# set-soft/ComfyUI-FLOAT_Optimized

Hardware: AMD Instinct MI355X
Metric: 512x512 frames/sec end-to-end audio->video @50 ODE steps (higher is better)
Workload: dtype fp16; 1 GPU; configs[1]: 10 s audio + 512x512 portrait in HBM -> 250 frames in pinned host memory; appearance encoder + wav2vec2 audio encoder + FMT sampling (50 Euler evaluations/window, CFG a=2.0 e=1.0) + decode + D2H, through InferenceAgent.infer_device (the product call); nfe=51, frames_per_clip=250, fmt_dtype=fp16, dec_dtype=fp16, decode_batch=32, hip_graph=True, parallelism=replicas x1 (one clip per GPU), stage_overlap=off

## Files before the change

### comfyui-float_optimized_amd/csrc/fmt_api.hip

```cpp
#include <math.h>
#include <stdlib.h>

#include "fmt_gemm.hpp"
#include "fmt_kernels.hpp"
#include "fmt_rb_kernels.hpp"
#include "fmt_big_kernels.hpp"

namespace {

typedef FmtLin Lin;

struct Blk {
  Lin qkv, proj, fc1, fc2;
};

constexpr int kMaxTok = 80;
constexpr int kMaxSteps = 1024;

}

struct float_fmt {
  float_fmt_cfg_t cfg;
  DevicePool pool;
  int D, ntok, Mpad, Kc, Ntot, Kx;
  int Bmax = 1;
  Lin x_embed, t0, t2, c_embed, adaln_all, final_lin;
  std::vector<Blk> blk;
  float* pos = nullptr;
  float* freqs = nullptr;
  u16 *cond16, *sc16, *h16, *hfin16, *qkv16, *att16, *hid16, *xin16, *tsin16, *th16;
  float *ccond, *xres, *xcur, *temb, *vout;
  unsigned long long* sat = nullptr;
  float* slab = nullptr;
  float *wa_c, *we_c, *prev_x, *prev_wa, *prev_we, *x0_c;
  int method = 0;
  FmtTune tune;
  int n_cu = 0;
  struct MegaPlan {
    MegaStage* dev = nullptr;
    int nstage = 0, bc = 0, tried = 0;
    MegaCtx ctx{};
  } mega[5];
  unsigned* mega_sync = nullptr;
  unsigned* mega_err_host = nullptr;
  u16* mega_ws = nullptr;
  float* kbuf = nullptr;
  float* modall = nullptr;
  int Mmod = 0;
  size_t mod_zs = 0;
  struct GraphKey {
    int nfe, bc, we_len, method, nclip;
    int prio;
    float a, r, e;
    bool operator==(const GraphKey& o) const { return memcmp(this, &o, sizeof(GraphKey)) == 0; }
  };
  struct GraphEntry {
    GraphKey key;
    hipGraphExec_t exec;
    uint64_t used;
  };
  std::vector<GraphEntry> graphs;
  uint64_t graph_clock = 0;
  hipStream_t cap_stream = nullptr;
  int cap_prio = 0;
  struct {
    const float *wr, *wa, *we, *noise;
    float* r_d;
    int T, we_len, nfe, include_r, next, n_chunks, B;
    int first = 0, total = 0;
    const float *hist_x = nullptr, *hist_wa = nullptr, *hist_we = nullptr;
    float a, r, e;
    std::vector<float> ts;
    bool active = false;
  } job;
};

namespace {

int round_up(int x, int m) { return (x + m - 1) / m * m; }

int dev_copy2d(float* dst, size_t dpitch, const float* src, size_t spitch, int width, int rows, hipStream_t s) {
  if (width <= 0 || rows <= 0) return FLOAT_OK;
  hipLaunchKernelGGL(fmt_copy_kernel, dim3((unsigned)(((size_t)rows * width + 255) / 256)), dim3(256), 0, s, dst, dpitch, src, spitch, width, rows);
  FH_CHECK_HIP(hipGetLastError());
  return FLOAT_OK;
}
int dev_copy(float* dst, const float* src, size_t n, hipStream_t s) { return dev_copy2d(dst, n, src, n, (int)n, 1, s); }
int dev_zero(float* dst, size_t n, hipStream_t s) { return dev_copy2d(dst, n, nullptr, n, (int)n, 1, s); }


template <class T>
__global__ __launch_bounds__(256) void fmt_pack_w_kernel(typename T::elem* __restrict__ out, const float* __restrict__ w, int N_each,
                                                         int K, int KB, int n0) {
  const size_t idx = (size_t)blockIdx.x * 256 + threadIdx.x;
  const int gpr = KB * 4;
  const int n = (int)(idx / gpr), k0 = (int)(idx % gpr) * 8;
  if (n >= N_each) return;
  typename T::pack8 p;
#pragma unroll
  for (int i = 0; i < 8; ++i) T::set(p, i, k0 + i < K ? w[(size_t)n * K + k0 + i] : 0.f);
  T::store8(out + fmt_pack_off(n0 + n, k0, KB), p);
}

template <class T>
int pack_linear_pool(const FmtTune& tn, DevicePool* pool, const TensorTable& tt, const std::vector<std::string>& names, int N_each,
                     int K, Lin* out) {
  typedef typename T::elem E;
  constexpr size_t esz = sizeof(E) / sizeof(u16);
  const int Kp = round_up(K, 128);
  const int N = N_each * (int)names.size();
  const bool on_host = tn.pack_host;
  std::vector<E> hw;
  if (on_host) hw.assign((size_t)N * Kp, (E)0);
  std::vector<float> hb(N, 0.f);
  int rc;
  if ((rc = pool->alloc(&out->W, (size_t)N * Kp * esz, false))) return rc;
  if ((rc = pool->alloc(&out->b, hb.size(), false))) return rc;
  float* stage = nullptr;
  if (!on_host) FH_CHECK_HIP(hipMalloc(&stage, (size_t)N_each * K * sizeof(float)));
  struct Free {
    float* p;
    ~Free() {
      if (p) (void)hipFree(p);
    }
  } free_stage{stage};
  int n0 = 0;
  for (const std::string& nm : names) {
    const float_tensor_t* w = tt.find(nm + ".weight");
    const float_tensor_t* b = tt.find(nm + ".bias");
    if (!w || !b) {
      fh_set_error("missing checkpoint tensor '%s.weight/.bias'", nm.c_str());
      return FLOAT_E_MISSING;
    }
    if (w->ndim != 2 || w->shape[0] != N_each || w->shape[1] != K || TensorTable::numel(b) != N_each) {
      fh_set_error("tensor '%s.weight' has shape (%lld,%lld), expected (%d,%d)", nm.c_str(), (long long)w->shape[0],
                   (long long)(w->ndim > 1 ? w->shape[1] : 0), N_each, K);
      return FLOAT_E_INVALID;
    }
    if (on_host) {
      for (int n = 0; n < N_each; ++n) {
        const float* src = w->data + (size_t)n * K;
        for (int k = 0; k < K; ++k) hw[fmt_pack_off(n0 + n, k, Kp / 32)] = T::host_from_float(src[k]);
      }
    } else {
      FH_CHECK_HIP(hipMemcpy(stage, w->data, (size_t)N_each * K * sizeof(float), hipMemcpyHostToDevice));
      const size_t packs = (size_t)N_each * (Kp / 8);
      hipLaunchKernelGGL((fmt_pack_w_kernel<T>), dim3((unsigned)((packs + 255) / 256)), dim3(256), 0, nullptr,
                         reinterpret_cast<E*>(out->W), stage, N_each, K, Kp / 32, n0);
      FH_CHECK_HIP(hipGetLastError());
    }
    for (int n = 0; n < N_each; ++n) hb[n0 + n] = b->data[n];
    n0 += N_each;
  }
  if (on_host) FH_CHECK_HIP(hipMemcpy(out->W, hw.data(), hw.size() * sizeof(E), hipMemcpyHostToDevice));
  FH_CHECK_HIP(hipMemcpy(out->b, hb.data(), hb.size() * sizeof(float), hipMemcpyHostToDevice));
  if (!on_host) FH_CHECK_HIP(hipDeviceSynchronize());
  out->N = N;
  out->K = Kp;
  return FLOAT_OK;
}

template <class T>
int pack_linear(float_fmt* h, const TensorTable& tt, const std::vector<std::string>& names, int N_each, int K, Lin* out) {
  return pack_linear_pool<T>(h->tune, &h->pool, tt, names, N_each, K, out);
}

constexpr int kWtRows = 256;
template <class T, int MTW, int KCH, int NWV = 4>
int launch_wide_t(GemmArgs g, bool prime, hipStream_t s) {
  constexpr int smem = 2 * MTW * KCH * 1024;
  auto kern = fmt_gemm_wide_kernel<T, MTW, KCH, NWV>;
  if (prime) {
    if (hipFuncSetAttribute(reinterpret_cast<const void*>(kern), hipFuncAttributeMaxDynamicSharedMemorySize, smem) != hipSuccess)
      (void)hipGetLastError();
    return FLOAT_OK;
  }
  const int mt_total = (g.M + 15) / 16;
  g.mblk = (mt_total + MTW - 1) / MTW;
  g.ksplit = 1;
  const dim3 grid((g.N / 128) * g.mblk * (g.zcount > 1 ? g.zcount : 1));
  fh_launch_prof(2, kern, grid, dim3(NWV * 64), smem, s, g);
  FH_CHECK_HIP(hipGetLastError());
  return FLOAT_OK;
}
template <class T, int NWC, int NS, int STG>
int launch_dma_t(GemmArgs g, bool prime, hipStream_t s) {
  constexpr int smem = NS * (12 + 5 * NWC) * 1024, BN = 80 * NWC;
  auto kern = fmt_gemm_dma_kernel<T, NWC, NS, STG>;
  if (prime) {
    if (hipFuncSetAttribute(reinterpret_cast<const void*>(kern), hipFuncAttributeMaxDynamicSharedMemorySize, smem) != hipSuccess)
      (void)hipGetLastError();
    return FLOAT_OK;
  }
  g.mblk = ((g.M + 15) / 16 + 11) / 12;
  const dim3 grid((g.N / BN) * g.mblk * (g.zcount > 1 ? g.zcount : 1));
  fh_launch_prof(2, kern, grid, dim3(NWC * 128), smem, s, g);
  FH_CHECK_HIP(hipGetLastError());
  return FLOAT_OK;
}
bool dma_shape_ok(const GemmArgs& g, int bn) { return g.N % bn == 0 && g.K % 64 == 0 && g.K >= 128; }

constexpr int kBigMinRows = 1536;
// ... 210 lines not shown
  }
}

struct Tiling {
  int mtw, nt, nw;
};
int pick_nw(int K, int forced) {
  const int KB = K / 32;
  if (forced && KB % forced == 0) return forced;
  if (KB >= 128 && KB % 16 == 0) return 16;
  if (KB >= 32 && KB % 8 == 0) return 8;
  return 4;
}
Tiling pick_tiling(const FmtTune& tn, int M, int N, int K, bool need_full_rows) {
  const int mt = (M + 15) / 16;
  if (need_full_rows) {
    if (mt <= 4) return {4, 1, pick_nw(K, 0)};
    return {mt <= 12 ? 12 : 15, 1, (tn.full_nw == 8 && (K / 32) % 8 == 0) ? 8 : 4};
  }
  int split = mt <= 4 ? 4 : (mt <= 12 ? 3 : 5);
  if (mt <= 2) split = mt;
  const int blocks = (mt + split - 1) / split;
  const bool wide = N >= 16384;
  if (mt >= 12) {
    const int* o = tn.plan + (wide ? 3 : 0);
    if (o[0]) {
      int nw = o[0] >= 12 ? 4 : pick_nw(K, o[2]);
      while (nw > 4 && nw * o[0] * 16 * o[1] * 16 * 4 > 160 * 1024) nw >>= 1;
      return {o[0], o[1], nw};
    }
  }
  if (wide) return {mt <= 4 ? 4 : 6, 2, std::min(8, pick_nw(K, 0))};
  if (mt > 15 && N % 64 == 0) return {3, 4, 4};
  int nt = 1;
  if (mt >= 5) {
    if ((N / 64) * blocks >= 192 && N % 64 == 0) nt = 4;
    else if ((N / 32) * blocks >= 192 && N % 32 == 0) nt = 2;
  } else if ((N / 16) * blocks > 512) {
    nt = 2;
  }
  return {split, nt, pick_nw(K, 0)};
}

GemmArgs base_args(const u16* A, const Lin& L, int M) {
  GemmArgs g;
  memset(&g, 0, sizeof(g));
  g.A = A;
  g.W = L.W;
  g.bias = L.b;
  g.K = L.K;
  g.N = L.N;
  g.M = M;
  return g;
}

Tiling pick_tiling32(int M) {
  const int mt = (M + 15) / 16;
  return {mt <= 5 ? mt : (mt <= 12 ? 3 : 5), 1, 4};
}

template <class T, int EPI>
int run_gemm(const FmtTune& tn, const GemmArgs& g, hipStream_t s, bool need_full_rows = false, const LayerPlan* plan = nullptr) {
  if constexpr (T::is32) {
    FH_REQUIRE(!need_full_rows, "the fp32 mode has no all-rows CFG epilogue tiling (token-blocked head only)");
    const Tiling t = pick_tiling32(g.M);
    GemmArgs g2 = g;
    g2.touch.W = nullptr;
    return launch_gemm<T, EPI>(g2, t.mtw, t.nt, t.nw, false, s);
  }
  if (plan && plan->on() && (g.M + 15) / 16 <= 15) {
    GemmArgs g2 = g;
    g2.touch.W = nullptr;
    return launch_gemm<T, EPI>(g2, plan->v[0], plan->v[1], plan->v[2], false, s);
  }
  const Tiling t = pick_tiling(tn, g.M, g.N, g.K, need_full_rows);
  return launch_gemm<T, EPI>(g, t.mtw, t.nt, t.nw, false, s);
}

struct PendingRed {
  int ks = 0;
  LnRed red{};
};

template <class T>
int run_gemm_partial(float_fmt* h, GemmArgs g, int ksplit, hipStream_t s, const LayerPlan* plan = nullptr) {
  g.ksplit = ksplit;
  g.out_f32 = h->slab;
  g.ldo = g.N;
  g.slab_stride = (size_t)h->Mpad * g.N;
  if (plan && plan->on() && !T::is32 && (g.M + 15) / 16 <= 15) {
    g.touch.W = nullptr;
    return launch_gemm<T, EPI_PARTIAL>(g, plan->v[0], plan->v[1], plan->v[2], false, s);
  }
  Tiling t = T::is32 ? pick_tiling32(g.M) : pick_tiling(h->tune, g.M, g.N * ksplit, g.K / ksplit, false);
  while (t.nt > 1 && g.N % (t.nt * 16)) t.nt >>= 1;
  if (T::is32) g.touch.W = nullptr;
  return launch_gemm<T, EPI_PARTIAL>(g, t.mtw, t.nt, t.nw, false, s);
}

TouchSpec make_touch(const FmtTune& tn, const Lin& L, int M, int ksplit, unsigned lanes, unsigned per_lane, int force_nt = 0) {
  TouchSpec t{};
  Tiling tl = ksplit ? pick_tiling(tn, M, L.N * ksplit, L.K / ksplit, false) : pick_tiling(tn, M, L.N, L.K, false);
  if (force_nt) tl.nt = force_nt;
  if (ksplit)
    while (tl.nt > 1 && L.N % (tl.nt * 16)) tl.nt >>= 1;
  const int ks = ksplit ? ksplit : 1;
  if (L.N % (tl.nt * 16) || L.K % (32 * ks) || 8 % ks) return t;
  const int nbn = L.N / (tl.nt * 16);
  if ((nbn * ks) % 8) return t;
  auto lg = [](unsigned v) {
    int n = 0;
    while ((1u << n) < v) ++n;
    return (1u << n) == v ? n : -1;
  };
  const unsigned P = 8 / ks, run_lines = (unsigned)(L.K / 32 / ks) * 8u;
  if (lg(run_lines) < 0 || lg((unsigned)tl.nt) < 0) return t;
  t.run_shift = (unsigned)lg(run_lines);
  t.nt_shift = (unsigned)lg((unsigned)tl.nt);
  t.p_shift = (unsigned)lg(P);
  t.tile_bytes = (unsigned)(L.K / 32) * 1024u;
  t.total = ((unsigned)nbn / P) * (unsigned)tl.nt * run_lines;
  if ((size_t)t.total > (size_t)lanes * per_lane) return t;
  t.W = reinterpret_cast<const char*>(L.W);
  return t;
}

TouchSpec make_touch_rb(const Lin& L, int shape, int kb, unsigned lanes, unsigned per_lane) {
  TouchSpec t{};
  const int ct = shape == 0 ? 4 : 8;
  if (kb <= 0 || (kb & (kb - 1)) || L.N % (ct * 16) || (L.N / (ct * 16)) % 8 || L.K / 32 < kb) return t;
  const unsigned run_lines = (unsigned)kb * 8u;
  auto lg = [](unsigned v) {
    int n = 0;
    while ((1u << n) < v) ++n;
    return n;
  };
  t.run_shift = (unsigned)lg(run_lines);
  t.nt_shift = (unsigned)lg((unsigned)ct);
  t.p_shift = 3;
  t.tile_bytes = (unsigned)(L.K / 32) * 1024u;
  t.total = (unsigned)(L.N / (ct * 16) / 8) * (unsigned)ct * run_lines;
  if ((size_t)t.total > (size_t)lanes * per_lane) return t;
  t.W = reinterpret_cast<const char*>(L.W);
  return t;
}

unsigned gemm_lanes_per_xcd(const FmtTune& tn, int M, int N, int K) {
  const Tiling t = pick_tiling(tn, M, N, K, false);
  const int mblk = ((M + 15) / 16 + t.mtw - 1) / t.mtw;
  return (unsigned)((N / (t.nt * 16)) * mblk / 8) * (unsigned)(t.nw * 64);
}

template <class T>
int launch_lnmod(float_fmt* h, int M, const float* shift, const float* scale, hipStream_t s, PendingRed* pend = nullptr,
                 const Lin* next = nullptr, u16* out = nullptr, int perm = 0, int touch_bit = 1, int rb_shape = -1) {
  const int nv = h->D / 256;
  const int rpw = h->tune.ln_rows;
  dim3 grid(rpw == 1 ? ((M + 63) / 64) * 64 : (M + rpw - 1) / rpw), block(64 * rpw);
  const int ks = pend ? pend->ks : 0;
  const bool wt = M <= kWtRows;
  LnRed red{};
  if (ks) red = pend->red;
  TouchSpec pf{};
  if (next && (h->tune.touch & (1 | touch_bit)) && rpw == 1 && !T::is32)
    pf = rb_shape >= 0 ? make_touch_rb(*next, rb_shape, h->tune.rb_touch, (grid.x / 8) * 64, 6)
                       : make_touch(h->tune, *next, M, 0, (grid.x / 8) * 64, 6);
#define LN_LAUNCH(NV, KS)                                                                                                          \
  do {                                                                                                                             \
    if (pf.W && wt) hipLaunchKernelGGL((fmt_lnmod_kernel<T, NV, KS, true, true>), grid, block, 0, s, h->xres, M, shift, scale, h->Ntot, out ? out : h->h16, red, pf, h->ntok, perm, h->sat); \
    else if (pf.W) hipLaunchKernelGGL((fmt_lnmod_kernel<T, NV, KS, true, false>), grid, block, 0, s, h->xres, M, shift, scale, h->Ntot, out ? out : h->h16, red, pf, h->ntok, perm, h->sat); \
    else if (wt) hipLaunchKernelGGL((fmt_lnmod_kernel<T, NV, KS, false, true>), grid, block, 0, s, h->xres, M, shift, scale, h->Ntot, out ? out : h->h16, red, pf, h->ntok, perm, h->sat); \
    else hipLaunchKernelGGL((fmt_lnmod_kernel<T, NV, KS, false, false>), grid, block, 0, s, h->xres, M, shift, scale, h->Ntot, out ? out : h->h16, red, pf, h->ntok, perm, h->sat);   \
  } while (0)
#define LN_CASE(NV)                     \
  case NV:                              \
    if (ks == 0) LN_LAUNCH(NV, 0);      \
    else if (ks == 1) LN_LAUNCH(NV, 1); \
    else if (ks == 2) LN_LAUNCH(NV, 2); \
    else if (ks == 4) LN_LAUNCH(NV, 4); \
    else LN_LAUNCH(NV, 8);              \
    break;
  switch (nv) {
    LN_CASE(1) LN_CASE(2) LN_CASE(4) LN_CASE(8)
    default:
      fh_set_error("dim_h %d unsupported (must be 256*{1,2,4,8})", h->D);
      return FLOAT_E_INVALID;
  }
#undef LN_CASE
#undef LN_LAUNCH
  if (pend) pend->ks = 0;
  FH_CHECK_HIP(hipGetLastError());
  return FLOAT_OK;
}

template <class T>
void launch_attn(float_fmt* h, int M, const Lin* pull, hipStream_t s) {
  const float_fmt_cfg_t& c = h->cfg;
  const int D = h->D, ntok = h->ntok;
  const int qpw = h->tune.attn_qpw, lpq = h->tune.attn_lpq;
  dim3 grid(c.heads, (M + qpw - 1) / qpw), block(qpw * lpq);
  TouchSpec pf{};
  if (pull && !T::is32) pf = make_touch(h->tune, *pull, M, 0, (grid.x * grid.y / 8) * block.x, 2);
#define ATTN_LAUNCH(LPQ, TCH)                                                                                                  \
  do {                                                                                                                         \
    if (M <= kWtRows) hipLaunchKernelGGL((fmt_attn_kernel<T, LPQ, TCH, true>), grid, block, 0, s, h->qkv16, 3 * D, h->att16, ntok, M, D, c.attn_window, pf, h->sat); \
    else hipLaunchKernelGGL((fmt_attn_kernel<T, LPQ, TCH, false>), grid, block, 0, s, h->qkv16, 3 * D, h->att16, ntok, M, D, c.attn_window, pf, h->sat);             \
  } while (0)
  if (lpq == 16) {
    if (pf.W) ATTN_LAUNCH(16, true);
    else ATTN_LAUNCH(16, false);
  } else {
    if (pf.W) ATTN_LAUNCH(8, true);
    else ATTN_LAUNCH(8, false);
  }
#undef ATTN_LAUNCH
}

int attnproj_hpw(const float_fmt* h) {
  const int hd = h->cfg.heads, hpw = h->tune.attnproj;
  if (hpw <= 0 || h->D != hd * 128 || hd % hpw) return 0;
  const int ks = hd / hpw;
  return (ks == 1 || ks == 2 || ks == 4 || ks == 8) && (hpw == 1 || hpw == 2) ? hpw : 0;
}
template <class T>
int launch_attnproj(float_fmt* h, int M, const Lin& proj, hipStream_t s) {
  const float_fmt_cfg_t& c = h->cfg;
  const int hpw = attnproj_hpw(h);
  GemmArgs g = base_args(nullptr, proj, M);
  g.sat = h->sat;
  g.out_f32 = h->slab;
  g.ldo = g.N;
  g.slab_stride = (size_t)h->Mpad * g.N;
  g.ksplit = c.heads / hpw;
  g.mblk = ((M + 15) / 16 + 2) / 3;
  const dim3 grid((unsigned)(g.ksplit * (g.N / (128 / hpw)) * g.mblk));
  fh_launch_prof(0, hpw == 2 ? fmt_attnproj_kernel<T, 3, 2> : fmt_attnproj_kernel<T, 3, 1>, grid, dim3(512), 0, s, h->qkv16, 3 * h->D, g,
                 h->ntok, h->D, c.attn_window);
  FH_CHECK_HIP(hipGetLastError());
  return FLOAT_OK;
}

constexpr int kScSteps = 64;

static int stream_priority(hipStream_t s) {
  int prio = 0;
  if (hipStreamGetPriority(s, &prio) != hipSuccess) {
    (void)hipGetLastError();
    prio = 0;
  }
  return prio;
}

template <class T>
int run_mod_all(float_fmt* h, int M, int e0, int n, hipStream_t s) {
  const int D = h->D;
  const FmtTune& tn = h->tune;
  FH_REQUIRE(n >= 1 && n <= kScSteps, "modulation batch of %d evaluations (max %d)", n, kScSteps);
  const int prio = (s == h->cap_stream && s) ? h->cap_prio : stream_priority(s);
  const bool big = !T::is32 && tn.wide && prio == 0 && big_shape_ok(tn, n * M, h->adaln_all.N, h->adaln_all.K, h->n_cu);
  hipLaunchKernelGGL((fmt_silu_c_kernel<T>), dim3((M * D / 8 + 255) / 256, n), dim3(256), 0, s, h->sc16, h->temb + (size_t)e0 * D,
                     h->ccond, M, D, (size_t)h->Mpad * D, big ? M : 0, h->sat);
  h->mod_zs = big ? (size_t)M * h->Ntot : (size_t)h->Mmod * h->Ntot;
  if constexpr (!T::is32) {
    if (big) return launch_big4<T>(h->sc16, h->adaln_all, h->modall, n * M, h->Ntot, h->n_cu, false, s);
  }
  GemmArgs g = base_args(h->sc16, h->adaln_all, M);
  g.sat = h->sat;
  g.out_f32 = h->modall;
  g.ldo = h->Ntot;
  g.zcount = n;
  const bool dma = (tn.wide_variant == 6 || tn.wide_variant == 7) && (M + 15) / 16 > 4 && dma_shape_ok(g, 320);
  g.zgroup = tn.zgroup > 0 ? tn.zgroup : (dma ? 2 : 4);
  g.a_zstride = (size_t)h->Mpad * D;
  g.o_zstride = (size_t)h->Mmod * h->Ntot;
  if constexpr (!T::is32) {
    if (tn.wide && g.N % 128 == 0 && g.K % 128 == 0) return launch_wide<T>(g, tn.wide_variant, false, s);
  }
  for (int z = 0; z < n; ++z) {
    GemmArgs gz = g;
    gz.A = g.A + (size_t)z * g.a_zstride * (sizeof(typename T::elem) / sizeof(u16));
    gz.out_f32 = g.out_f32 + (size_t)z * g.o_zstride;
    gz.zcount = 0;
    int rc = run_gemm<T, EPI_F32>(tn, gz, s);
    if (rc) return rc;
  }
  return FLOAT_OK;
}

constexpr int kMegaWgs = 256, kMegaSmem = 8 * 48 * 64 * 4;
MegaSync mega_sync_of(const float_fmt* h) {
  unsigned* m = h->mega_sync;
  return MegaSync{m, m + 8 * 32, m + 9 * 32, m + 17 * 32, m + 18 * 32, h->mega_err_host, reinterpret_cast<unsigned long long*>(m + 20 * 32), (unsigned)h->tune.mega_stamp_wg};
}
int mega_poll(float_fmt* h) {
  if (!h->mega_err_host || *reinterpret_cast<volatile unsigned*>(h->mega_err_host) == 0u) return FLOAT_OK;
  FH_CHECK_HIP(hipDeviceSynchronize());
  for (auto& gr : h->graphs) (void)hipGraphExecDestroy(gr.exec);
  h->graphs.clear();
  if (h->mega_sync) FH_CHECK_HIP(hipMemset(h->mega_sync, 0, (size_t)(32 * 20) * sizeof(unsigned)));
  *reinterpret_cast<volatile unsigned*>(h->mega_err_host) = 0u;
  h->tune.mega = 0;
  h->job.active = false;
  fh_set_error("fmt_mega_kernel: a grid barrier timed out in an earlier call (not all %d workgroups were resident) - the results of "
               "that call are invalid; the handle falls back to the launch chain (FLOAT_FMT_MEGA=0 selects it from the start)", 256);
  return FLOAT_E_HIP;
}
template <class T>
bool mega_shape_ok(const float_fmt* h, int nclip, int bc) {
  const FmtTune& tn = h->tune;
  if (T::is32 || !tn.mega || nclip != 1 || bc != 3 || h->D != 1024 || h->cfg.heads != 8 || h->n_cu < kMegaWgs) return false;
  if (attnproj_hpw(h) || tn.fc2_split != 4 || tn.proj_split != 0) return false;
  const int M = bc * h->ntok;
  auto is = [](Tiling t, int a, int b, int c) { return t.mtw == a && t.nt == b && t.nw == c; };
  const Blk& B = h->blk[0];
  return (M + 15) / 16 == 12 && (h->ntok + 15) / 16 == 4 && h->x_embed.K % 256 == 0 && h->final_lin.K % 256 == 0 &&
         is(pick_tiling(tn, M, B.qkv.N, B.qkv.K, false), 3, 4, 8) && is(pick_tiling(tn, M, B.proj.N, B.proj.K, false), 3, 1, 8) &&
         is(pick_tiling(tn, M, B.fc1.N, B.fc1.K, false), 3, 4, 8) && is(pick_tiling(tn, M, B.fc2.N * 4, B.fc2.K / 4, false), 3, 4, 8) &&
         B.fc2.K % 512 == 0;
}

template <class T>
int build_mega(float_fmt* h, int bc) {
  float_fmt::MegaPlan& P = h->mega[bc];
  P.tried = 1;
  {
    int per_cu = 0;
    if (hipOccupancyMaxActiveBlocksPerMultiprocessor(&per_cu, reinterpret_cast<const void*>(fmt_mega_kernel<T>), 512, kMegaSmem) != hipSuccess) {
      (void)hipGetLastError();
      per_cu = 0;
    }
    if (per_cu * h->n_cu < kMegaWgs) {
      h->tune.mega = 0;
      return FLOAT_OK;
    }
  }
  const float_fmt_cfg_t& c = h->cfg;
  const FmtTune& tn = h->tune;
  const int D = h->D, ntok = h->ntok, M = bc * ntok;
  std::vector<MegaStage> st;
  const size_t esz = sizeof(typename T::elem) / sizeof(u16);
  const size_t n_h = (size_t)h->Mpad * D * esz, n_hid = (size_t)h->Mpad * c.mlp_hidden * esz;
  if (!h->mega_ws) {
    int rc0 = h->pool.alloc(&h->mega_ws, (size_t)c.depth * (3 * n_h + n_hid), true);
    if (rc0) return rc0;
  }
  auto ws_h1 = [&](int b) { return h->mega_ws + (size_t)b * (3 * n_h + n_hid); };
  auto ws_h2 = [&](int b) { return ws_h1(b) + n_h; };
  auto ws_att = [&](int b) { return ws_h1(b) + 2 * n_h; };
  auto ws_hid = [&](int b) { return ws_h1(b) + 3 * n_h; };
  auto gemm_stage = [&](int kind, GemmArgs g, int mtw, int nt) {
    MegaStage m;
    memset(&m, 0, sizeof(m));
    m.kind = kind;
    g.sat = h->sat;
    g.mblk = ((g.M + 15) / 16 + mtw - 1) / mtw;
    if (g.ksplit < 1) g.ksplit = 1;
    m.g = g;
    m.nblk = (unsigned)((g.N / (nt * 16)) * g.mblk * g.ksplit);
    return m;
  };
  auto ln_stage = [&](int b_mod, int which, int ks, const float* bias, int gate_col, const Lin* next, int touch_bit, u16* out, int perm) {
    MegaStage m;
    memset(&m, 0, sizeof(m));
    m.kind = MS_LN;
    m.nblk = (unsigned)(((M + 63) / 64) * 64);
    m.shift_off = (long long)b_mod * 6 * D + (long long)which * D;
    m.scale_off = m.shift_off + D;
    m.ks = ks;
    m.red_bias = bias;
    m.red_gate_off = (long long)b_mod * 6 * D + (long long)gate_col * D;
    m.ln_out = out ? out : h->h16;
    m.perm = perm;
    if (next && (tn.touch & (1 | touch_bit))) m.pf = make_touch(tn, *next, M, 0, (m.nblk / 8) * 64, 6);
    return m;
  };
  {
    GemmArgs g = base_args(h->xin16, h->x_embed, ntok);
    g.out_f32 = h->xres;
    g.ldo = D;
    g.pos = h->pos;
    g.bc = bc;
    g.ntok = ntok;
    st.push_back(gemm_stage(MS_XEMBED, g, 4, 1));
  }
  for (int b = 0; b < c.depth; ++b) {
    const Blk& B = h->blk[b];
    if (b == 0) st.push_back(ln_stage(b, 0, 0, nullptr, 0, &B.qkv, 128, ws_h1(b), 0));
    else {
      MegaStage m = ln_stage(b, 0, 4, h->blk[b - 1].fc2.b, 0, &B.qkv, 128, ws_h1(b), 0);
      m.red_gate_off = (long long)(b - 1) * 6 * D + 5LL * D;
      st.push_back(m);
    }
    {
      GemmArgs g = base_args(ws_h1(b), B.qkv, M);
      g.out16 = h->qkv16;
      g.ldo16 = 3 * D;
      if (tn.touch & 8) g.touch = make_touch(tn, B.proj, M, 0, gemm_lanes_per_xcd(tn, M, g.N, g.K), 2);
      st.push_back(gemm_stage(MS_QKV, g, 3, 4));
    }
    {
      MegaStage m;
      memset(&m, 0, sizeof(m));
      m.kind = MS_ATTN;
      m.nblk = (unsigned)(c.heads * ((M + 7) / 8));
      if (tn.touch & 2) m.pf = make_touch(tn, B.proj, M, 0, (m.nblk / 8) * 128, 2);
      m.att_out = ws_att(b);
      st.push_back(m);
    }
    {
      GemmArgs g = base_args(ws_att(b), B.proj, M);
      g.out_f32 = h->xres;
      g.ldo = D;
      g.ldg = h->Ntot;
      if (tn.touch & 16) g.touch = make_touch(tn, B.fc1, M, 0, gemm_lanes_per_xcd(tn, M, g.N, g.K), 2);
      MegaStage m = gemm_stage(MS_PROJ, g, 3, 1);
      m.gate_off = (long long)b * 6 * D + 2LL * D;
      st.push_back(m);
    }
    st.push_back(ln_stage(b, 3, 0, nullptr, 0, &B.fc1, 64, ws_h2(b), 0));
    {
      GemmArgs g = base_args(ws_h2(b), B.fc1, M);
      g.out16 = ws_hid(b);
      g.ldo16 = B.fc2.K / 32;
      if (tn.touch & 4) g.touch = make_touch(tn, B.fc2, M, 4, gemm_lanes_per_xcd(tn, M, g.N, g.K), 2);
      st.push_back(gemm_stage(MS_FC1, g, 3, 4));
    }
    {
      GemmArgs g = base_args(ws_hid(b), B.fc2, M);
      g.ksplit = 4;
      g.out_f32 = h->slab;
      g.ldo = g.N;
      g.slab_stride = (size_t)h->Mpad * g.N;
      if (tn.touch & 32) {
        const unsigned lanes = gemm_lanes_per_xcd(tn, M, g.N * 4, g.K / 4);
        if (b + 1 < c.depth) g.touch = make_touch(tn, h->blk[b + 1].qkv, M, 0, lanes, 2);
        else g.touch = make_touch(tn, h->final_lin, M, 0, lanes, 2, 1);
      }
      st.push_back(gemm_stage(MS_FC2, g, 3, 4));
    }
  }
  {
    const int nblk = (ntok + 15) / 16, seqs = bc;
    MegaStage m = ln_stage(c.depth, 0, 4, h->blk[c.depth - 1].fc2.b, 0, nullptr, 0, h->hfin16, seqs * 16);
    m.red_gate_off = (long long)(c.depth - 1) * 6 * D + 5LL * D;
    st.push_back(m);
    GemmArgs g = base_args(h->hfin16, h->final_lin, nblk * seqs * 16);
    g.tokblk = 1;
    g.nclip = 1;
    g.bc = bc;
    g.ntok = ntok;
    g.n_prev = c.n_prev;
    g.xcur = h->xcur;
    g.xin16 = h->xin16;
    g.ldx = h->Kx / 32;
    st.push_back(gemm_stage(MS_HEAD, g, bc, 1));
  }
  for (const MegaStage& m : st) FH_REQUIRE(m.nblk <= (unsigned)kMegaWgs, "persistent kernel: a stage needs %u workgroups", m.nblk);
  int rc;
  if (!h->mega_sync && (rc = h->pool.alloc(&h->mega_sync, 32 * 20 + 2 * 3 * 64, true))) return rc;
  if (!h->mega_err_host) {
    FH_CHECK_HIP(hipHostMalloc(reinterpret_cast<void**>(&h->mega_err_host), 64, hipHostMallocMapped));
    memset(h->mega_err_host, 0, 64);
  }
  if ((rc = h->pool.alloc(&P.dev, st.size(), false))) return rc;
  FH_CHECK_HIP(hipMemcpy(P.dev, st.data(), st.size() * sizeof(MegaStage), hipMemcpyHostToDevice));
  P.nstage = (int)st.size();
  P.bc = bc;
  P.ctx = MegaCtx{h->xres, h->qkv16, h->slab, (size_t)h->Mpad * D, M, D, ntok, h->Ntot, c.attn_window, c.heads, h->sat};
  return FLOAT_OK;
}

template <class T>
int run_mega(float_fmt* h, int bc, const float* modbuf, bool euler, float dt, float a, float r, float e, hipStream_t s, float* vout_to) {
  float_fmt::MegaPlan& P = h->mega[bc];
  MegaDyn d{modbuf, dt, a, r, e, euler ? 1 : 0, vout_to ? vout_to : h->vout};
  fh_launch_prof(0, (fmt_mega_kernel<T>), dim3(kMegaWgs), dim3(512), kMegaSmem, s, P.dev, P.nstage, d, P.ctx, mega_sync_of(h));
  FH_CHECK_HIP(hipGetLastError());
  return FLOAT_OK;
}

template <class T>
int run_blocks(float_fmt* h, int nclip, int bc, const float* modbuf, bool euler, float dt, float a, float r, float e, hipStream_t s,
               float* vout_to = nullptr) {
  const float_fmt_cfg_t& c = h->cfg;
  const FmtTune& tn = h->tune;
  const int D = h->D, ntok = h->ntok, M = nclip * bc * ntok;
  int rc;
  if constexpr (!T::is32) {
    if (bc <= 4 && mega_shape_ok<T>(h, nclip, bc)) {
      if (h->mega[bc].dev) return run_mega<T>(h, bc, modbuf, euler, dt, a, r, e, s, vout_to);
    }
  }
  {
    GemmArgs g = base_args(h->xin16, h->x_embed, nclip * ntok);
    g.sat = h->sat;
    g.out_f32 = h->xres;
    g.ldo = D;
    g.pos = h->pos;
    g.bc = bc;
    g.ntok = ntok;
    if ((rc = run_gemm<T, EPI_XEMBED>(tn, g, s))) return rc;
  }
  PendingRed pend;
  RbPlan rb_qkv, rb_proj, rb_fc1, rb_fc2;
  if constexpr (!T::is32) {
    rb_qkv = pick_rb(tn, RB_QKV, M), rb_proj = pick_rb(tn, RB_PROJ, M), rb_fc1 = pick_rb(tn, RB_FC1, M), rb_fc2 = pick_rb(tn, RB_FC2, M);
  }
  auto split_ok = [&](int ks, const Lin& L) { return (ks == 1 || ks == 2 || ks == 4) && L.K % (128 * ks) == 0; };
  for (int b = 0; b < c.depth; ++b) {
    const float* mod = modbuf + (size_t)b * 6 * D;
    const Blk& B = h->blk[b];
    if ((rc = launch_lnmod<T>(h, M, mod, mod + D, s, &pend, &B.qkv, nullptr, 0, 128, rb_qkv.shape))) return rc;
    {
      GemmArgs g = base_args(h->h16, B.qkv, M);
      g.sat = h->sat;
      g.out16 = h->qkv16;
      g.ldo16 = 3 * D;
      if ((tn.touch & 8) && attnproj_hpw(h)) g.touch = make_touch(tn, B.proj, M, c.heads / attnproj_hpw(h), gemm_lanes_per_xcd(tn, M, g.N, g.K), 2, 8 / attnproj_hpw(h));
      else if ((tn.touch & 8) && !split_ok(tn.proj_split, B.proj)) g.touch = make_touch(tn, B.proj, M, 0, gemm_lanes_per_xcd(tn, M, g.N, g.K), 2);
      if (rb_qkv.shape >= 0) rc = launch_rbs<T, EPI_T16>(g, rb_qkv.shape, false, s);
      else rc = run_gemm<T, EPI_T16>(tn, g, s, false, &tn.plan_layer[RB_QKV]);
      if (rc) return rc;
    }
    if (rb_proj.shape >= 0) {
      launch_attn<T>(h, M, nullptr, s);
      GemmArgs gp = base_args(h->att16, B.proj, M);
      gp.ksplit = rb_proj.ksplit;
      gp.out_f32 = h->slab;
      gp.ldo = gp.N;
      gp.slab_stride = (size_t)h->Mpad * gp.N;
      if ((rc = launch_rbs<T, EPI_PARTIAL>(gp, rb_proj.shape, false, s))) return rc;
      pend.ks = rb_proj.ksplit;
      pend.red = LnRed{h->slab, (size_t)h->Mpad * D, B.proj.b, mod + 2 * D};
    } else if (attnproj_hpw(h)) {
      if ((rc = launch_attnproj<T>(h, M, B.proj, s))) return rc;
      pend.ks = c.heads / attnproj_hpw(h);
      pend.red = LnRed{h->slab, (size_t)h->Mpad * D, B.proj.b, mod + 2 * D};
    } else if (split_ok(tn.proj_split, B.proj)) {
      launch_attn<T>(h, M, nullptr, s);
      GemmArgs gp = base_args(h->att16, B.proj, M);
      if ((rc = run_gemm_partial<T>(h, gp, tn.proj_split, s))) return rc;
      pend.ks = tn.proj_split;
      pend.red = LnRed{h->slab, (size_t)h->Mpad * D, B.proj.b, mod + 2 * D};
    } else {
      launch_attn<T>(h, M, (tn.touch & 2) ? &B.proj : nullptr, s);
      GemmArgs g = base_args(h->att16, B.proj, M);
      g.sat = h->sat;
      g.out_f32 = h->xres;
      g.ldo = D;
      g.gate = mod + 2 * D;
      g.ldg = h->Ntot;
      if (tn.touch & 16) g.touch = make_touch(tn, B.fc1, M, 0, gemm_lanes_per_xcd(tn, M, g.N, g.K), 2);
      if ((rc = run_gemm<T, EPI_GATE_RES>(tn, g, s, false, &tn.plan_layer[RB_PROJ]))) return rc;
    }
    if ((rc = launch_lnmod<T>(h, M, mod + 3 * D, mod + 4 * D, s, &pend, &B.fc1, nullptr, 0, 64, rb_fc1.shape))) return rc;
    {
      GemmArgs g = base_args(h->h16, B.fc1, M);
      g.sat = h->sat;
      g.out16 = h->hid16;
      g.ldo16 = B.fc2.K / 32;
      if ((tn.touch & 4) && rb_fc2.shape < 0)
        g.touch = make_touch(tn, B.fc2, M, split_ok(tn.fc2_split, B.fc2) ? tn.fc2_split : 0, gemm_lanes_per_xcd(tn, M, g.N, g.K), 2);
      if (rb_fc1.shape >= 0) rc = launch_rbs<T, EPI_GELU_P16>(g, rb_fc1.shape, false, s);
      else rc = run_gemm<T, EPI_GELU_P16>(tn, g, s, false, &tn.plan_layer[RB_FC1]);
      if (rc) return rc;
    }
    if (rb_fc2.shape >= 0) {
      GemmArgs g = base_args(h->hid16, B.fc2, M);
      g.ksplit = rb_fc2.ksplit;
      g.out_f32 = h->slab;
      g.ldo = g.N;
      g.slab_stride = (size_t)h->Mpad * g.N;
      if ((rc = launch_rbs<T, EPI_PARTIAL>(g, rb_fc2.shape, false, s))) return rc;
      pend.ks = rb_fc2.ksplit;
      pend.red = LnRed{h->slab, (size_t)h->Mpad * D, B.fc2.b, mod + 5 * D};
    } else if (split_ok(tn.fc2_split, B.fc2)) {
      GemmArgs g = base_args(h->hid16, B.fc2, M);
      g.sat = h->sat;
      if (tn.touch & 32) {
        const unsigned lanes = gemm_lanes_per_xcd(tn, M, g.N * tn.fc2_split, g.K / tn.fc2_split);
        if (b + 1 < c.depth) g.touch = make_touch(tn, h->blk[b + 1].qkv, M, 0, lanes, 2);
        else g.touch = make_touch(tn, h->final_lin, M, 0, lanes, 2, 1);
      }
      if ((rc = run_gemm_partial<T>(h, g, tn.fc2_split, s, &tn.plan_layer[RB_FC2]))) return rc;
      pend.ks = tn.fc2_split;
      pend.red = LnRed{h->slab, (size_t)h->Mpad * D, B.fc2.b, mod + 5 * D};
    } else {
      GemmArgs g = base_args(h->hid16, B.fc2, M);
      g.sat = h->sat;
      g.out_f32 = h->xres;
      g.ldo = D;
      g.gate = mod + 5 * D;
      g.ldg = h->Ntot;
      if ((rc = run_gemm<T, EPI_GATE_RES>(tn, g, s))) return rc;
    }
  }
  {
    const float* mod = modbuf + (size_t)c.depth * 6 * D;
    const bool tokblk = (!tn.no_tokblk || nclip > 1) && (bc == 1 || bc == 3 || bc == 4) && h->final_lin.K % 256 == 0;
    FH_REQUIRE(tokblk || nclip == 1, "batched sampling needs the token-blocked head GEMM");
    const int nblk = (ntok + 15) / 16, seqs = nclip * bc;
    if ((rc = launch_lnmod<T>(h, M, mod, mod + D, s, &pend, nullptr, tokblk ? h->hfin16 : nullptr, tokblk ? seqs * 16 : 0))) return rc;
    GemmArgs g = base_args(tokblk ? h->hfin16 : h->h16, h->final_lin, tokblk ? nblk * seqs * 16 : M);
    g.sat = h->sat;
    g.tokblk = tokblk ? 1 : 0;
    g.nclip = nclip;
    g.bc = bc;
    g.ntok = ntok;
    g.n_prev = c.n_prev;
    g.a_cfg = a;
    g.r_cfg = r;
    g.e_cfg = e;
    g.dt = dt;
    if (euler) {
      g.xcur = h->xcur;
      g.xin16 = h->xin16;
      g.ldx = h->Kx / 32;
    } else {
      g.vout = vout_to ? vout_to : h->vout;
    }
    if (tokblk) rc = launch_gemm<T, EPI_CFG>(g, bc, 1, 8, false, s);
    else rc = run_gemm<T, EPI_CFG>(tn, g, s, true);
    if (rc) return rc;
  }
  FH_CHECK_HIP(hipGetLastError());
  return FLOAT_OK;
}

void linspace01(int n, std::vector<float>* ts) {
  ts->resize(n);
  if (n == 1) {
    (*ts)[0] = 0.f;
    return;
  }
  const float step = 1.0f / (float)(n - 1);
  const int half = n / 2;
  for (int i = 0; i < n; ++i) (*ts)[i] = (i < half) ? (0.f + step * (float)i) : (1.0f - step * (float)(n - 1 - i));
}

struct TimeSpec {
  float t;
  int nfe, stages;
  float c[4];
};
template <class T>
int prepare_time(float_fmt* h, const TimeSpec& ts, int n, hipStream_t s) {
  int rc;
  hipLaunchKernelGGL((fmt_tsin_kernel<T>), dim3(n), dim3(256), 0, s, h->tsin16, h->freqs, n, ts.t, ts.nfe, ts.stages, ts.c[0],
                     ts.c[1], ts.c[2], ts.c[3]);
  GemmArgs g = base_args(h->tsin16, h->t0, n);
  g.sat = h->sat;
  g.out16 = h->th16;
  g.ldo16 = h->t2.K / 32;
  if ((rc = launch_gemm<T, EPI_SILU_P16>(g, 4, 1, T::is32 ? 4 : pick_nw(g.K, 0), false, s))) return rc;
  GemmArgs g2 = base_args(h->th16, h->t2, n);
  g2.sat = h->sat;
  g2.out_f32 = h->temb;
  g2.ldo = h->D;
  if ((rc = launch_gemm<T, EPI_F32>(g2, 4, 1, T::is32 ? 4 : pick_nw(g2.K, 0), false, s))) return rc;
  return FLOAT_OK;
}

struct CfgMode {
  int bc;
  unsigned wr_mask, wa_mask, we_mask;
  int nclip = 1;
};

CfgMode cfg_mode(float a, float r, float e, int include_r) {
  if (a == 1.0f && r == 1.0f && e == 1.0f) return {1, 1u, 1u, 1u, 1};
  if (!include_r) return {3, 0b111u, 0b110u, 0b010u, 1};
  return {4, 0b1110u, 0b1100u, 0b0100u, 1};
}

template <class T>
int stage_window(float_fmt* h, const CfgMode& m, const float* x0, const float* wa, const float* wr, const float* we,
                 int we_len, const float* prev_x, const float* prev_wa, const float* prev_we, hipStream_t s) {
  const float_fmt_cfg_t& c = h->cfg;
  const int M = m.nclip * m.bc * h->ntok;
  hipLaunchKernelGGL((fmt_build_cond_kernel<T>), dim3(M), dim3(256), 0, s, h->cond16, h->Kc, m.bc, h->ntok, c.n_prev,
                     c.dim_w, c.dim_a, c.dim_e, wr, wa, prev_wa, we, we_len, prev_we, m.wr_mask, m.wa_mask, m.we_mask, h->sat);
  GemmArgs g = base_args(h->cond16, h->c_embed, M);
  g.sat = h->sat;
  g.out_f32 = h->ccond;
  g.ldo = h->D;
  int rc;
  if ((rc = run_gemm<T, EPI_F32>(h->tune, g, s))) return rc;
  const int n = m.nclip * h->ntok * c.dim_w;
  hipLaunchKernelGGL((fmt_init_x_kernel<T>), dim3((n + 255) / 256), dim3(256), 0, s, h->xcur, h->xin16, h->Kx / 32, x0, prev_x,
                     c.n_prev, c.n_cur, c.dim_w, m.nclip, h->sat);
  FH_CHECK_HIP(hipGetLastError());
  return FLOAT_OK;
}

int check_common(float_fmt* h, const void* we, int we_len, const void* prev_we) {
  FH_REQUIRE(h != nullptr, "null FMT handle");
  FH_REQUIRE(we_len == 1 || we_len == h->cfg.n_cur,
             "Dynamic emotion latent `we` time dimension (%d) does not match audio latent `wa` time dimension (%d).",
             we_len, h->cfg.n_cur);
  FH_REQUIRE(!(we_len > 1 && prev_we == nullptr),
             "`we` is dynamic (T>1), but prev_we was not provided with prev_x/prev_wa.");
  (void)we;
  return FLOAT_OK;
}

struct Tableau {
  int s;
  float c[4], a[4][3], b[4];
};
const Tableau& tableau(int method) {
  static const Tableau T[5] = {
      {1, {0.f}, {{0.f}}, {1.f}},
      {2, {0.f, 0.5f}, {{0.f}, {0.5f}}, {0.f, 1.f}},
      {4, {0.f, 1.f / 3, 2.f / 3, 1.f}, {{0.f}, {1.f / 3}, {-1.f / 3, 1.f}, {1.f, -1.f, 1.f}}, {0.125f, 0.375f, 0.375f, 0.125f}},
      {2, {0.f, 1.f}, {{0.f}, {1.f}}, {0.5f, 0.5f}},
      {3, {0.f, 1.f / 3, 2.f / 3}, {{0.f}, {1.f / 3}, {0.f, 2.f / 3}}, {0.25f, 0.f, 0.75f}},
  };
  return T[method];
}

TimeSpec time_spec(int method, int nfe) {
  const Tableau& tb = tableau(method);
  TimeSpec ts{};
  ts.nfe = nfe;
  ts.stages = tb.s;
  for (int j = 0; j < 4; ++j) ts.c[j] = tb.c[j];
  return ts;
}
int n_evals(int method, int nfe) { return (nfe - 1) * tableau(method).s; }

template <class T>
int run_window_steps(float_fmt* h, const CfgMode& m, int nfe, const std::vector<float>& ts, float a, float r, float e,
                     hipStream_t s) {
  const Tableau& tb = tableau(h->method);
  const float_fmt_cfg_t& c = h->cfg;
  const size_t kstride = (size_t)h->Bmax * kMaxTok * c.dim_w;
  const int n = m.nclip * c.n_cur * c.dim_w, rows = m.nclip * m.bc * h->ntok;
  const int nev = n_evals(h->method, nfe), batch = h->tune.hoist ? kScSteps : 1;
  const bool euler = h->method == FLOAT_ODE_EULER;
  int rc;
  for (int ev = 0; ev < nev; ++ev) {
    const int i = ev / tb.s, j = ev - i * tb.s, z = ev % batch;
    const float dt = ts[i + 1] - ts[i];
    if (z == 0 && (rc = run_mod_all<T>(h, rows, ev, std::min(batch, nev - ev), s))) return rc;
    const float* mod = h->modall + (size_t)z * h->mod_zs;
    if (euler) {
      if ((rc = run_blocks<T>(h, m.nclip, m.bc, mod, true, dt, a, r, e, s))) return rc;
      continue;
    }
    if (j > 0) {
      hipLaunchKernelGGL((fmt_rk_combine_kernel<T>), dim3((n + 255) / 256), dim3(256), 0, s, h->xcur, h->kbuf, kstride, j,
                         dt * tb.a[j][0], dt * tb.a[j][1], dt * tb.a[j][2], 0.f, 0, h->xin16, h->Kx / 32, c.n_prev, c.n_cur,
                         c.dim_w, m.nclip, h->sat);
    }
    if ((rc = run_blocks<T>(h, m.nclip, m.bc, mod, false, 0.f, a, r, e, s, h->kbuf + (size_t)j * kstride))) return rc;
    if (j == tb.s - 1) {
      hipLaunchKernelGGL((fmt_rk_combine_kernel<T>), dim3((n + 255) / 256), dim3(256), 0, s, h->xcur, h->kbuf, kstride, tb.s,
                         dt * tb.b[0], dt * tb.b[1], dt * tb.b[2], dt * tb.b[3], 1, h->xin16, h->Kx / 32, c.n_prev, c.n_cur,
                         c.dim_w, m.nclip, h->sat);
    }
  }
  FH_CHECK_HIP(hipGetLastError());
  return FLOAT_OK;
}

constexpr size_t kMaxGraphs = 8;
template <class T>
int run_window_steps_graph(float_fmt* h, const CfgMode& m, int we_len, int nfe, const std::vector<float>& ts, float a,
                           float r, float e, hipStream_t s) {
  float_fmt::GraphKey key;
  memset(&key, 0, sizeof(key));
  key.nfe = nfe;
  key.method = h->method;
  key.bc = m.bc;
  key.nclip = m.nclip;
  key.we_len = we_len;
  key.a = a;
  key.r = r;
  key.e = e;
  key.prio = stream_priority(s);
  float_fmt::GraphEntry* hit = nullptr;
  for (auto& g : h->graphs)
    if (g.key == key) hit = &g;
  if (!hit) {
    if (!h->cap_stream) FH_CHECK_HIP(hipStreamCreateWithFlags(&h->cap_stream, hipStreamNonBlocking));
    hipGraph_t graph = nullptr;
    h->cap_prio = key.prio;
    FH_CHECK_HIP(hipStreamBeginCapture(h->cap_stream, hipStreamCaptureModeThreadLocal));
    int rc = run_window_steps<T>(h, m, nfe, ts, a, r, e, h->cap_stream);
    hipError_t ce = hipStreamEndCapture(h->cap_stream, &graph);
    if (rc) {
      if (graph) (void)hipGraphDestroy(graph);
      return rc;
    }
    FH_CHECK_HIP(ce);
    hipGraphExec_t exec = nullptr;
    FH_CHECK_HIP(hipGraphInstantiate(&exec, graph, nullptr, nullptr, 0));
    (void)hipGraphDestroy(graph);
    if (h->graphs.size() >= kMaxGraphs) {
      size_t lru = 0;
      for (size_t i = 1; i < h->graphs.size(); ++i)
        if (h->graphs[i].used < h->graphs[lru].used) lru = i;
      FH_CHECK_HIP(hipDeviceSynchronize());
      (void)hipGraphExecDestroy(h->graphs[lru].exec);
      h->graphs.erase(h->graphs.begin() + lru);
    }
    h->graphs.push_back({key, exec, 0});
    hit = &h->graphs.back();
  }
  hit->used = ++h->graph_clock;
  FH_CHECK_HIP(hipGraphLaunch(hit->exec, s));
  return FLOAT_OK;
}

template <class T>
int window_impl(float_fmt* h, const float* x0, const float* wa, const float* wr, const float* we, int we_len,
                const float* prev_x, const float* prev_wa, const float* prev_we, int nfe, const std::vector<float>& ts,
                float a, float r, float e, int include_r, hipStream_t s, int nclip = 1) {
  CfgMode m = cfg_mode(a, r, e, include_r);
  m.nclip = nclip;
  FH_REQUIRE(!h->tune.no_tokblk || m.bc * h->ntok <= 240,
             "%d-way CFG of %d tokens is %d rows; the all-rows CFG epilogue GEMM holds at most 240 (15 row tiles)", m.bc, h->ntok,
             m.bc * h->ntok);
  int rc = stage_window<T>(h, m, x0, wa, wr, we, we_len, prev_x, prev_wa, prev_we, s);
  if (rc) return rc;
  if (nfe <= 1) return FLOAT_OK;
  hipStreamCaptureStatus cs = hipStreamCaptureStatusNone;
  if (hipStreamIsCapturing(s, &cs) != hipSuccess) {
    (void)hipGetLastError();
    cs = hipStreamCaptureStatusNone;
  }
  if (h->cfg.use_graph && !g_fh_profiling && cs == hipStreamCaptureStatusNone)
    return run_window_steps_graph<T>(h, m, we_len, nfe, ts, a, r, e, s);
  return run_window_steps<T>(h, m, nfe, ts, a, r, e, s);
}

template <class T>
int eval_impl(float_fmt* h, float t, const float* x, const float* wa, const float* wr, const float* we, int we_len,
              const float* prev_x, const float* prev_wa, const float* prev_we, float a, float r, float e, int include_r,
              float* out, hipStream_t s) {
  TimeSpec tsp{};
  tsp.t = t;
  int rc = prepare_time<T>(h, tsp, 1, s);
  if (rc) return rc;
  const CfgMode m = cfg_mode(a, r, e, include_r);
  FH_REQUIRE(!h->tune.no_tokblk || m.bc * h->ntok <= 240,
             "%d-way CFG of %d tokens is %d rows; the all-rows CFG epilogue GEMM holds at most 240 (15 row tiles)", m.bc, h->ntok,
             m.bc * h->ntok);
  if ((rc = stage_window<T>(h, m, x, wa, wr, we, we_len, prev_x, prev_wa, prev_we, s))) return rc;
  if ((rc = run_mod_all<T>(h, m.bc * h->ntok, 0, 1, s))) return rc;
  if ((rc = run_blocks<T>(h, 1, m.bc, h->modall, false, 0.f, a, r, e, s))) return rc;
  return dev_copy(out, h->vout, (size_t)h->ntok * h->cfg.dim_w, s);
}

template <class T>
int sample_window(float_fmt* h, int k, hipStream_t s) {
  const float_fmt_cfg_t& c = h->cfg;
  auto& J = h->job;
  const int L = c.n_cur, P = c.n_prev, Tn = J.T, B = J.B;
  const bool dynamic = J.we_len > 1;
  int rc;
  auto blocks = [](int n) { return dim3((n + 255) / 256); };
  if (k == J.first) {
    if ((rc = prepare_time<T>(h, time_spec(h->method, J.nfe), std::max(1, n_evals(h->method, J.nfe)), s))) return rc;
    if (J.hist_x) rc = dev_copy(h->prev_x, J.hist_x, (size_t)B * P * c.dim_w, s);
    else rc = dev_zero(h->prev_x, (size_t)B * P * c.dim_w, s);
    if (rc) return rc;
    if (J.hist_wa) rc = dev_copy(h->prev_wa, J.hist_wa, (size_t)B * P * c.dim_a, s);
    else rc = dev_zero(h->prev_wa, (size_t)B * P * c.dim_a, s);
    if (rc) return rc;
    if (J.hist_we) rc = dev_copy(h->prev_we, J.hist_we, (size_t)B * P * c.dim_e, s);
    else rc = dev_zero(h->prev_we, (size_t)B * P * c.dim_e, s);
    if (rc) return rc;
  } else if (P > 0) {
    hipLaunchKernelGGL(fmt_tail_kernel, blocks(B * P * c.dim_w), dim3(256), 0, s, h->prev_x, h->xcur, P, L, c.dim_w, B);
    hipLaunchKernelGGL(fmt_tail_kernel, blocks(B * P * c.dim_a), dim3(256), 0, s, h->prev_wa, h->wa_c, P, L, c.dim_a, B);
    if (dynamic) hipLaunchKernelGGL(fmt_tail_kernel, blocks(B * P * c.dim_e), dim3(256), 0, s, h->prev_we, h->we_c, P, L, c.dim_e, B);
  }
  hipLaunchKernelGGL(fmt_slice_pad_kernel, blocks(B * L * c.dim_a), dim3(256), 0, s, h->wa_c, J.wa, k * L, Tn, L, c.dim_a, B);
  if (dynamic) hipLaunchKernelGGL(fmt_slice_pad_kernel, blocks(B * L * c.dim_e), dim3(256), 0, s, h->we_c, J.we, k * L, Tn, L, c.dim_e, B);
  if ((rc = dev_copy(h->x0_c, J.noise + (size_t)k * B * L * c.dim_w, (size_t)B * L * c.dim_w, s))) return rc;
  rc = window_impl<T>(h, h->x0_c, h->wa_c, J.wr, dynamic ? h->we_c : J.we, dynamic ? L : 1, h->prev_x, h->prev_wa,
                      dynamic ? h->prev_we : nullptr, J.nfe, J.ts, J.a, J.r, J.e, J.include_r, s, B);
  if (rc) return rc;
  const int rows = (k == J.total - 1) ? (Tn - k * L) : L;
  return dev_copy2d(J.r_d + (size_t)k * L * c.dim_w, (size_t)Tn * c.dim_w, h->xcur, (size_t)L * c.dim_w, rows * c.dim_w, B, s);
}

template <class T>
int create_impl(float_fmt* h, const TensorTable& tt) {
  const float_fmt_cfg_t& c = h->cfg;
  const int D = c.dim_h;
  int rc;
  prime_kernels<T>();
  if ((rc = pack_linear<T>(h, tt, {"x_embedder.proj"}, D, c.dim_w, &h->x_embed))) return rc;
  if ((rc = pack_linear<T>(h, tt, {"t_embedder.mlp.0"}, D, 256, &h->t0))) return rc;
  if ((rc = pack_linear<T>(h, tt, {"t_embedder.mlp.2"}, D, D, &h->t2))) return rc;
  if ((rc = pack_linear<T>(h, tt, {"c_embedder"}, D, c.dim_w + c.dim_a + c.dim_e, &h->c_embed))) return rc;
  h->blk.resize(c.depth);
  std::vector<std::string> ada;
  for (int b = 0; b < c.depth; ++b) {
    const std::string p = "blocks." + std::to_string(b) + ".";
    if ((rc = pack_linear<T>(h, tt, {p + "attn.qkv"}, 3 * D, D, &h->blk[b].qkv))) return rc;
    if ((rc = pack_linear<T>(h, tt, {p + "attn.proj"}, D, D, &h->blk[b].proj))) return rc;
    if ((rc = pack_linear<T>(h, tt, {p + "mlp.fc1"}, c.mlp_hidden, D, &h->blk[b].fc1))) return rc;
    if ((rc = pack_linear<T>(h, tt, {p + "mlp.fc2"}, D, c.mlp_hidden, &h->blk[b].fc2))) return rc;
    ada.push_back(p + "adaLN_modulation.1");
  }
  if ((rc = pack_linear<T>(h, tt, ada, 6 * D, D, &h->adaln_all))) return rc;
  {
    Lin tail;
    if ((rc = pack_linear<T>(h, tt, {"decoder.adaLN_modulation.1"}, 2 * D, D, &tail))) return rc;
    Lin fused;
    fused.N = h->adaln_all.N + tail.N;
    fused.K = h->adaln_all.K;
    constexpr size_t esz = sizeof(typename T::elem) / sizeof(u16);
    if ((rc = h->pool.alloc(&fused.W, (size_t)fused.N * fused.K * esz, false))) return rc;
    if ((rc = h->pool.alloc(&fused.b, (size_t)fused.N, false))) return rc;
    FH_CHECK_HIP(hipMemcpy(fused.W, h->adaln_all.W, (size_t)h->adaln_all.N * fused.K * esz * sizeof(u16), hipMemcpyDeviceToDevice));
    FH_CHECK_HIP(hipMemcpy(fused.W + (size_t)h->adaln_all.N * fused.K * esz, tail.W, (size_t)tail.N * fused.K * esz * sizeof(u16),
                           hipMemcpyDeviceToDevice));
    FH_CHECK_HIP(hipMemcpy(fused.b, h->adaln_all.b, (size_t)h->adaln_all.N * sizeof(float), hipMemcpyDeviceToDevice));
    FH_CHECK_HIP(hipMemcpy(fused.b + h->adaln_all.N, tail.b, (size_t)tail.N * sizeof(float), hipMemcpyDeviceToDevice));
    h->adaln_all = fused;
  }
  if ((rc = pack_linear<T>(h, tt, {"decoder.linear"}, c.dim_w, D, &h->final_lin))) return rc;
  return FLOAT_OK;
}

}


int fmt_pack_linear(const FmtTune& tn, DevicePool* pool, int dtype, const TensorTable& tt, const std::vector<std::string>& names,
                    int N_each, int K, FmtLin* out) {
  FH_REQUIRE(dtype == FLOAT_DT_BF16 || dtype == FLOAT_DT_FP16 || dtype == FLOAT_DT_FP32, "the GEMM service: unknown dtype %d", dtype);
  if (dtype == FLOAT_DT_FP32) return pack_linear_pool<FP32>(tn, pool, tt, names, N_each, K, out);
  return dtype == FLOAT_DT_BF16 ? pack_linear_pool<BF16>(tn, pool, tt, names, N_each, K, out)
                                : pack_linear_pool<FP16>(tn, pool, tt, names, N_each, K, out);
}

int fmt_pack_linear_raw(const FmtTune& tn, DevicePool* pool, int dtype, const float* w, const float* b, int N, int K, FmtLin* out) {
  std::vector<float> zeros;
  if (!b) {
    zeros.assign(N, 0.f);
    b = zeros.data();
  }
  float_tensor_t t[2];
  memset(t, 0, sizeof(t));
  t[0].name = "raw.weight";
  t[0].data = w;
  t[0].ndim = 2;
  t[0].shape[0] = N;
  t[0].shape[1] = K;
  t[1].name = "raw.bias";
  t[1].data = b;
  t[1].ndim = 1;
  t[1].shape[0] = N;
  TensorTable tt(t, 2);
  return fmt_pack_linear(tn, pool, dtype, tt, {"raw"}, N, K, out);
}

GemmArgs fmt_gemm_args(const u16* A, const FmtLin& L, int M) { return base_args(A, L, M); }

void fmt_gemm_prime(int dtype) {
  if (dtype == FLOAT_DT_BF16) prime_kernels<BF16>();
  else if (dtype == FLOAT_DT_FP32) prime_kernels<FP32>();
  else prime_kernels<FP16>();
}

template <class T>
static int gemm_run_t(const FmtTune& tn, int epi, const GemmArgs& g, hipStream_t s) {
  switch (epi) {
    case EPI_F32: return run_gemm<T, EPI_F32>(tn, g, s);
    case EPI_T16: return run_gemm<T, EPI_T16>(tn, g, s);
    case EPI_SILU_P16: return run_gemm<T, EPI_SILU_P16>(tn, g, s);
    case EPI_GELU_P16: return run_gemm<T, EPI_GELU_P16>(tn, g, s);
    case EPI_GELUERF_P16: return run_gemm<T, EPI_GELUERF_P16>(tn, g, s);
    default: fh_set_error("fmt_gemm_run: epilogue %d is not exported", epi); return FLOAT_E_INVALID;
  }
}

int fmt_gemm_run(const FmtTune& tn, int dtype, int epi, GemmArgs g, hipStream_t s) {
  if (dtype == FLOAT_DT_FP32) return gemm_run_t<FP32>(tn, epi, g, s);
  return dtype == FLOAT_DT_BF16 ? gemm_run_t<BF16>(tn, epi, g, s) : gemm_run_t<FP16>(tn, epi, g, s);
}

template <class T>
static int debug_impl(float_fmt* h, int what, const float* in, float* out, hipStream_t s) {
  const int D = h->D, ntok = h->ntok;
  if (what == 0) {
    return dev_copy(out, h->pos, (size_t)ntok * D, s);
  }
  if (what == 2) {
    FH_REQUIRE(h->mega_sync && h->mega[3].nstage > 0 && h->mega[3].nstage <= 64, "no persistent-kernel plan");
    FH_CHECK_HIP(hipStreamSynchronize(s));
    const int n = h->mega[3].nstage * 3;
    std::vector<unsigned long long> st(n);
    FH_CHECK_HIP(hipMemcpy(st.data(), h->mega_sync + 20 * 32, n * 8, hipMemcpyDeviceToHost));
    std::vector<float> us(n);
    for (int i = 0; i < n; ++i) us[i] = st[i] ? (float)((double)(st[i] - st[0]) * 0.01) : -1.f;
    FH_CHECK_HIP(hipMemcpy(out, us.data(), n * 4, hipMemcpyHostToDevice));
    return FLOAT_OK;
  }
  FH_REQUIRE(what == 1 && in != nullptr, "float_fmt_debug: unknown request %d (or null input)", what);
  const int n = ntok * 3 * D;
  hipLaunchKernelGGL((fmt_dbg_to16_kernel<T>), dim3((n + 255) / 256), dim3(256), 0, s, h->qkv16, in, n);
  launch_attn<T>(h, ntok, nullptr, s);
  hipLaunchKernelGGL((fmt_dbg_unpack_kernel<T>), dim3((ntok * D + 255) / 256), dim3(256), 0, s, out, h->att16, ntok, D);
  FH_CHECK_HIP(hipGetLastError());
  return FLOAT_OK;
}

extern "C" {

int float_fmt_create(const float_fmt_cfg_t* cfg, const float_tensor_t* tensors, int32_t n_tensors, float_fmt_t** out) {
  FH_REQUIRE(cfg && tensors && out, "null argument to float_fmt_create");
  FH_REQUIRE(cfg->dim_h % 256 == 0 && cfg->dim_h / 256 <= 8 && ((cfg->dim_h / 256) & (cfg->dim_h / 256 - 1)) == 0,
             "dim_h=%d unsupported", cfg->dim_h);
  FH_REQUIRE(cfg->dim_h / cfg->heads == 128, "head_dim must be 128 (dim_h=%d heads=%d)", cfg->dim_h, cfg->heads);
  FH_REQUIRE(cfg->dim_w % 128 == 0 && cfg->mlp_hidden % 128 == 0, "dim_w / mlp_hidden must be multiples of 128");
  FH_REQUIRE(cfg->n_prev + cfg->n_cur <= kMaxTok, "at most %d tokens per window (got %d)", kMaxTok, cfg->n_prev + cfg->n_cur);
  FH_REQUIRE(cfg->n_prev >= 0 && cfg->n_prev <= cfg->n_cur, "n_prev must be in [0, n_cur]");
  FH_REQUIRE(cfg->dtype == FLOAT_DT_BF16 || cfg->dtype == FLOAT_DT_FP16 || cfg->dtype == FLOAT_DT_FP32, "unknown dtype %d", cfg->dtype);
  FH_REQUIRE(cfg->max_batch >= 0 && cfg->max_batch <= 16, "max_batch must be in [0, 16] (got %d)", cfg->max_batch);
  float_fmt* h = new float_fmt();
  h->tune = FmtTune::from_env();
  h->cfg = *cfg;
  h->D = cfg->dim_h;
  h->ntok = cfg->n_prev + cfg->n_cur;
  h->Bmax = cfg->max_batch > 0 ? cfg->max_batch : 1;
  h->Mpad = 16 * ((h->Bmax * 4 * h->ntok + 15) / 16 + 12);
  h->Kc = round_up(cfg->dim_w + cfg->dim_a + cfg->dim_e, 128);
  h->Kx = round_up(cfg->dim_w, 128);
  {
    int dev = 0, ncu = 0;
    if (hipGetDevice(&dev) == hipSuccess && hipDeviceGetAttribute(&ncu, hipDeviceAttributeMultiprocessorCount, dev) == hipSuccess) h->n_cu = ncu;
    else (void)hipGetLastError();
  }
  h->Ntot = cfg->depth * 6 * h->D + 2 * h->D;
  TensorTable tt(tensors, n_tensors);
  int rc = (cfg->dtype == FLOAT_DT_BF16) ? create_impl<BF16>(h, tt)
           : (cfg->dtype == FLOAT_DT_FP16) ? create_impl<FP16>(h, tt) : create_impl<FP32>(h, tt);
  const int D = h->D, Mp = h->Mpad;
  const size_t esz = cfg->dtype == FLOAT_DT_FP32 ? 2 : 1;
  auto A = [&](auto** p, size_t n) {
    if (!rc) rc = h->pool.alloc(p, std::is_same<std::remove_reference_t<decltype(**p)>, u16>::value ? n * esz : n, true);
  };
  A(&h->pos, (size_t)kMaxTok * D);
  A(&h->freqs, 128);
  A(&h->cond16, (size_t)Mp * h->Kc);
  A(&h->sc16, (size_t)kScSteps * Mp * D + (size_t)12 * 16 * D);
  A(&h->h16, (size_t)Mp * D);
  A(&h->hfin16, (size_t)h->Bmax * 64 * ((kMaxTok + 15) / 16) * D);
  A(&h->qkv16, (size_t)Mp * 3 * D);
  A(&h->att16, (size_t)Mp * D);
  A(&h->hid16, (size_t)Mp * cfg->mlp_hidden);
  A(&h->xin16, (size_t)(h->Bmax * kMaxTok + 6 * 16) * h->Kx);
  A(&h->tsin16, (size_t)kMaxSteps * 256);
  A(&h->th16, (size_t)kMaxSteps * D);
  A(&h->ccond, (size_t)Mp * D);
  h->Mmod = 16 * ((h->Bmax * 4 * h->ntok + 15) / 16);
  if (!rc) rc = h->pool.alloc(&h->modall, (size_t)kScSteps * h->Mmod * h->Ntot, false);
  A(&h->kbuf, (size_t)4 * h->Bmax * kMaxTok * cfg->dim_w);
  A(&h->xres, (size_t)Mp * D);
  A(&h->slab, (size_t)8 * Mp * D);
  A(&h->sat, 1);
  A(&h->xcur, (size_t)h->Bmax * cfg->n_cur * cfg->dim_w);
  A(&h->temb, (size_t)kMaxSteps * D);
  A(&h->vout, (size_t)h->Bmax * kMaxTok * cfg->dim_w);
  A(&h->wa_c, (size_t)h->Bmax * cfg->n_cur * cfg->dim_a);
  A(&h->we_c, (size_t)h->Bmax * cfg->n_cur * cfg->dim_e);
  A(&h->x0_c, (size_t)h->Bmax * cfg->n_cur * cfg->dim_w);
  A(&h->prev_x, (size_t)h->Bmax * cfg->n_cur * cfg->dim_w);
  A(&h->prev_wa, (size_t)h->Bmax * cfg->n_cur * cfg->dim_a);
  A(&h->prev_we, (size_t)h->Bmax * cfg->n_cur * cfg->dim_e);
  if (!rc) {
    std::vector<float> pos((size_t)h->ntok * D);
    const float_tensor_t* pe = tt.find("pos_embed");
    if (pe && TensorTable::numel(pe) == (int64_t)h->ntok * D) {
      memcpy(pos.data(), pe->data, pos.size() * sizeof(float));
    } else {
      for (int p = 0; p < h->ntok; ++p)
        for (int j = 0; j < D; ++j) {
          const float ang = (float)((double)p / pow(10000.0, 2.0 * (double)(j / 2) / (double)D));
          pos[(size_t)p * D + j] = (j & 1) ? cosf(ang) : sinf(ang);
        }
    }
    std::vector<float> fr(128);
    for (int k = 0; k < 128; ++k) fr[k] = expf(-logf(10000.0f) * (float)k / 128.0f);
    if (hipMemcpy(h->pos, pos.data(), pos.size() * sizeof(float), hipMemcpyHostToDevice) != hipSuccess ||
        hipMemcpy(h->freqs, fr.data(), fr.size() * sizeof(float), hipMemcpyHostToDevice) != hipSuccess) {
      fh_set_error("hipMemcpy of FMT tables failed");
      rc = FLOAT_E_HIP;
    }
  }
  if (!rc && cfg->dtype != FLOAT_DT_FP32) {
    const bool ok = cfg->dtype == FLOAT_DT_BF16 ? mega_shape_ok<BF16>(h, 1, 3) : mega_shape_ok<FP16>(h, 1, 3);
    if (ok) rc = cfg->dtype == FLOAT_DT_BF16 ? build_mega<BF16>(h, 3) : build_mega<FP16>(h, 3);
  }
  if (rc) {
    float_fmt_destroy(h);
    return rc;
  }
  *out = h;
  return FLOAT_OK;
}

void float_fmt_destroy(float_fmt_t* h) {
  if (!h) return;
  for (auto& g : h->graphs) (void)hipGraphExecDestroy(g.exec);
  if (h->cap_stream) (void)hipStreamDestroy(h->cap_stream);
  if (h->mega_err_host) (void)hipHostFree(h->mega_err_host);
  h->pool.release();
  delete h;
}

int float_fmt_eval(float_fmt_t* h, float t, const float* x, const float* wa, const float* wr, const float* we,
                   int32_t we_len, const float* prev_x, const float* prev_wa, const float* prev_we, float a_cfg,
                   float r_cfg, float e_cfg, int32_t include_r_cfg, float* out, void* stream) {
  int rc = check_common(h, we, we_len, prev_we);
  if (rc) return rc;
  if ((rc = mega_poll(h))) return rc;
  FH_REQUIRE(x && wa && wr && we && prev_x && prev_wa && out, "null tensor argument to float_fmt_eval");
  hipStream_t s = (hipStream_t)stream;
  return h->cfg.dtype == FLOAT_DT_BF16
             ? eval_impl<BF16>(h, t, x, wa, wr, we, we_len, prev_x, prev_wa, prev_we, a_cfg, r_cfg, e_cfg, include_r_cfg, out, s)
         : h->cfg.dtype == FLOAT_DT_FP16
             ? eval_impl<FP16>(h, t, x, wa, wr, we, we_len, prev_x, prev_wa, prev_we, a_cfg, r_cfg, e_cfg, include_r_cfg, out, s)
             : eval_impl<FP32>(h, t, x, wa, wr, we, we_len, prev_x, prev_wa, prev_we, a_cfg, r_cfg, e_cfg, include_r_cfg, out, s);
}

int float_fmt_sample_chunk(float_fmt_t* h, const float* x0, const float* wa, const float* wr, const float* we,
                           int32_t we_len, const float* prev_x, const float* prev_wa, const float* prev_we, int32_t nfe,
                           float a_cfg, float r_cfg, float e_cfg, int32_t include_r_cfg, float* out, void* stream) {
  int rc = check_common(h, we, we_len, prev_we);
  if (rc) return rc;
  if ((rc = mega_poll(h))) return rc;
  FH_REQUIRE(x0 && wa && wr && we && prev_x && prev_wa && out, "null tensor argument to float_fmt_sample_chunk");
  FH_REQUIRE(nfe >= 1 && n_evals(h->method, nfe) < kMaxSteps, "nfe=%d: too many evaluations (max %d)", nfe, kMaxSteps);
  hipStream_t s = (hipStream_t)stream;
  std::vector<float> ts;
  linspace01(nfe, &ts);
  const float_fmt_cfg_t& c = h->cfg;
  if ((rc = dev_copy(h->x0_c, x0, (size_t)c.n_cur * c.dim_w, s))) return rc;
  if ((rc = dev_copy(h->wa_c, wa, (size_t)c.n_cur * c.dim_a, s))) return rc;
  if ((rc = dev_copy(h->prev_x, prev_x, (size_t)c.n_prev * c.dim_w, s))) return rc;
  if ((rc = dev_copy(h->prev_wa, prev_wa, (size_t)c.n_prev * c.dim_a, s))) return rc;
  if (we_len > 1) {
    if ((rc = dev_copy(h->we_c, we, (size_t)c.n_cur * c.dim_e, s))) return rc;
    if ((rc = dev_copy(h->prev_we, prev_we, (size_t)c.n_prev * c.dim_e, s))) return rc;
  }
  const float* we_p = we_len > 1 ? h->we_c : we;
  const float* pwe_p = we_len > 1 ? h->prev_we : nullptr;
  const TimeSpec tsp = time_spec(h->method, nfe);
  const int nev = std::max(1, n_evals(h->method, nfe));
#define FMT_CHUNK(TT)                                                                                                          \
  do {                                                                                                                           \
    if ((rc = prepare_time<TT>(h, tsp, nev, s))) return rc;                                                                      \
    rc = window_impl<TT>(h, h->x0_c, h->wa_c, wr, we_p, we_len, h->prev_x, h->prev_wa, pwe_p, nfe, ts, a_cfg, r_cfg, e_cfg,      \
                         include_r_cfg, s);                                                                                      \
  } while (0)
  if (c.dtype == FLOAT_DT_BF16) FMT_CHUNK(BF16);
  else if (c.dtype == FLOAT_DT_FP16) FMT_CHUNK(FP16);
  else FMT_CHUNK(FP32);
#undef FMT_CHUNK
  if (rc) return rc;
  return dev_copy(out, h->xcur, (size_t)c.n_cur * c.dim_w, s);
}

int float_fmt_debug(float_fmt_t* h, int32_t what, const float* in, float* out, void* stream) {
  FH_REQUIRE(h != nullptr && out != nullptr, "null argument to float_fmt_debug");
  return h->cfg.dtype == FLOAT_DT_BF16   ? debug_impl<BF16>(h, what, in, out, (hipStream_t)stream)
         : h->cfg.dtype == FLOAT_DT_FP16 ? debug_impl<FP16>(h, what, in, out, (hipStream_t)stream)
                                         : debug_impl<FP32>(h, what, in, out, (hipStream_t)stream);
}

int float_fmt_saturation(float_fmt_t* h, uint64_t* total, int32_t reset, void* stream) {
  FH_REQUIRE(h && total, "null argument to float_fmt_saturation");
  FH_CHECK_HIP(hipStreamSynchronize((hipStream_t)stream));
  unsigned long long v = 0;
  FH_CHECK_HIP(hipMemcpy(&v, h->sat, sizeof(v), hipMemcpyDeviceToHost));
  *total = v;
  if (reset) {
    FH_CHECK_HIP(hipMemsetAsync(h->sat, 0, sizeof(v), (hipStream_t)stream));
    FH_CHECK_HIP(hipStreamSynchronize((hipStream_t)stream));
  }
  if (int rc = mega_poll(h)) return rc;
  return FLOAT_OK;
}

int float_fmt_set_method(float_fmt_t* h, int32_t method) {
  FH_REQUIRE(h != nullptr, "null FMT handle");
  FH_REQUIRE(method >= FLOAT_ODE_EULER && method <= FLOAT_ODE_HEUN3, "unknown ODE method %d", method);
  h->method = method;
  return FLOAT_OK;
}

int float_fmt_sample_begin(float_fmt_t* h, const float* wr, const float* wa, int32_t T, const float* we, int32_t we_len,
                           const float* noise, int32_t nfe, float a_cfg, float r_cfg, float e_cfg, int32_t include_r_cfg,
                           float* r_d) {
  FH_REQUIRE(h != nullptr, "null FMT handle");
  FH_REQUIRE(wr && wa && we && noise && r_d, "null tensor argument to float_fmt_sample");
  FH_REQUIRE(T >= 1, "T must be >= 1 (got %d)", T);
  FH_REQUIRE(we_len == 1 || we_len == T,
             "Dynamic emotion latent `we` time dimension (%d) does not match audio latent `wa` time dimension (%d).",
             we_len, T);
  FH_REQUIRE(nfe >= 1 && n_evals(h->method, nfe) < kMaxSteps, "nfe=%d: too many evaluations (max %d)", nfe, kMaxSteps);
  auto& J = h->job;
  J.wr = wr;
  J.wa = wa;
  J.we = we;
  J.noise = noise;
  J.r_d = r_d;
  J.T = T;
  J.we_len = we_len;
  J.nfe = nfe;
  J.include_r = include_r_cfg;
  J.a = a_cfg;
  J.r = r_cfg;
  J.e = e_cfg;
  J.B = 1;
  J.next = 0;
  J.n_chunks = (T + h->cfg.n_cur - 1) / h->cfg.n_cur;
  J.first = 0;
  J.total = J.n_chunks;
  J.hist_x = J.hist_wa = J.hist_we = nullptr;
  linspace01(nfe, &J.ts);
  J.active = true;
  return FLOAT_OK;
}

int float_fmt_sample_begin_range(float_fmt_t* h, const float* wr, const float* wa, int32_t T, const float* we, int32_t we_len,
                                 const float* noise, int32_t nfe, float a_cfg, float r_cfg, float e_cfg, int32_t include_r_cfg,
                                 float* r_d, int32_t first_window, int32_t end_window, const float* hist_x, const float* hist_wa,
                                 const float* hist_we) {
  int rc = float_fmt_sample_begin(h, wr, wa, T, we, we_len, noise, nfe, a_cfg, r_cfg, e_cfg, include_r_cfg, r_d);
  if (rc) return rc;
  auto& J = h->job;
  J.active = false;
  FH_REQUIRE(first_window >= 0 && first_window < end_window && end_window <= J.total,
             "window range [%d, %d) outside the clip's %d windows", first_window, end_window, J.total);
  FH_REQUIRE(we_len == 1 || hist_we != nullptr || hist_x == nullptr,
             "a dynamic-emotion job that starts from a history needs hist_we too");
  J.first = J.next = first_window;
  J.n_chunks = end_window;
  J.hist_x = hist_x;
  J.hist_wa = hist_wa;
  J.hist_we = we_len > 1 ? hist_we : nullptr;
  J.active = true;
  return FLOAT_OK;
}

int float_fmt_sample_next(float_fmt_t* h, void* stream, int32_t* window_done, int32_t* windows_left) {
  FH_REQUIRE(h != nullptr && h->job.active, "float_fmt_sample_next without float_fmt_sample_begin");
  if (int prc = mega_poll(h)) return prc;
  auto& J = h->job;
  hipStream_t s = (hipStream_t)stream;
  const int k = J.next;
  int rc = h->cfg.dtype == FLOAT_DT_BF16   ? sample_window<BF16>(h, k, s)
           : h->cfg.dtype == FLOAT_DT_FP16 ? sample_window<FP16>(h, k, s)
                                           : sample_window<FP32>(h, k, s);
  if (rc) {
    J.active = false;
    return rc;
  }
  J.next = k + 1;
  if (window_done) *window_done = k;
  if (windows_left) *windows_left = J.n_chunks - J.next;
  if (J.next >= J.n_chunks) J.active = false;
  return FLOAT_OK;
}

int float_fmt_sample_batch(float_fmt_t* h, int32_t n_clips, const float* wr, const float* wa, int32_t T, const float* we,
                           int32_t we_len, const float* noise, int32_t nfe, float a_cfg, float r_cfg, float e_cfg,
                           int32_t include_r_cfg, float* r_d, void* stream) {
  FH_REQUIRE(h != nullptr, "null FMT handle");
  FH_REQUIRE(n_clips >= 1 && n_clips <= h->Bmax, "batch of %d clips, the handle was created with max_batch = %d", n_clips, h->Bmax);
  int rc = float_fmt_sample_begin(h, wr, wa, T, we, we_len, noise, nfe, a_cfg, r_cfg, e_cfg, include_r_cfg, r_d);
  if (rc) return rc;
  h->job.B = n_clips;
  int32_t left = 1;
  while (left > 0)
    if ((rc = float_fmt_sample_next(h, stream, nullptr, &left))) return rc;
  return FLOAT_OK;
}

int float_fmt_sample(float_fmt_t* h, const float* wr, const float* wa, int32_t T, const float* we, int32_t we_len,
                     const float* noise, int32_t nfe, float a_cfg, float r_cfg, float e_cfg, int32_t include_r_cfg,
                     float* r_d, void* stream) {
  int rc = float_fmt_sample_begin(h, wr, wa, T, we, we_len, noise, nfe, a_cfg, r_cfg, e_cfg, include_r_cfg, r_d);
  if (rc) return rc;
  int32_t left = 1;
  while (left > 0)
    if ((rc = float_fmt_sample_next(h, stream, nullptr, &left))) return rc;
  return FLOAT_OK;
}

}
```

### comfyui-float_optimized_amd/csrc/fmt_kernels.hpp

```cpp
#pragma once
#include "common.hpp"
#include "fmt_pack.hpp"

template <class T, int MTW, int NT, int NW, int EPI, bool COH>
__device__ __forceinline__ void fmt_gemm_body(const GemmArgs& g, const unsigned bid, const unsigned nblk) {
  constexpr int BN = NT * 16;
  constexpr int ROWS = MTW * 16;
  constexpr bool WT = NW >= 8 || COH;
  auto ldA = [](const typename T::elem* p) -> typename T::pack8 { return T::load8(p); };
  constexpr int NTHR = NW * 64;
  constexpr int PF = T::is32 ? 1 : ((MTW + NT <= 7) ? 4 : ((MTW + NT <= 8) ? 3 : 2));
  typedef typename T::elem E;
  typedef typename T::pack8 P8;
  extern __shared__ __attribute__((aligned(16))) float red[];
  const int lane = threadIdx.x & 63;
  const int w = threadIdx.x >> 6;
  const int r16 = lane & 15, q = lane >> 4;
  int bx, by, ks = 0;
  {
    const int nbn = g.N / BN, id = (int)bid;
    const int nbx = (EPI == EPI_PARTIAL) ? nbn * g.ksplit : nbn;
    if ((nbx & 7) == 0) {
      const int slot = id >> 3;
      by = slot % g.mblk;
      bx = (slot / g.mblk) * 8 + (id & 7);
    } else {
      bx = id % nbx;
      by = id / nbx;
    }
    if constexpr (EPI == EPI_PARTIAL) {
      if ((nbx & 7) == 0 && (8 % g.ksplit) == 0) {
        const int P = 8 / g.ksplit, x = bx & 7;
        ks = x / P;
        bx = (bx >> 3) * P + (x % P);
      } else {
        ks = bx / nbn;
        bx = bx % nbn;
      }
    }
  }
  const int nb0 = bx * NT;
  const int mt0 = by * MTW;
  const int n0 = nb0 * 16, m0 = mt0 * 16;

  f32x4 acc[MTW][NT];
#pragma unroll
  for (int i = 0; i < MTW; ++i)
#pragma unroll
    for (int j = 0; j < NT; ++j) acc[i][j] = f32x4{0.f, 0.f, 0.f, 0.f};

  const int KB = g.K >> 5;
  const int KBs = (EPI == EPI_PARTIAL) ? KB / g.ksplit : KB;
  const int KBw = KBs / NW;
  const E* Ap = reinterpret_cast<const E*>(g.A) + ((size_t)mt0 * KB + ks * KBs + w * KBw) * 512 + lane * 8;
  const E* Wp = reinterpret_cast<const E*>(g.W) + ((size_t)nb0 * KB + ks * KBs + w * KBw) * 512 + lane * 8;
  const size_t tstride = (size_t)KB * 512;
  constexpr bool kEarlyRes = (EPI == EPI_GATE_RES) && (MTW * 16 * (NT * 2) <= NW * 64);
  float4 res_pf[2], gate_pf[2];
  if constexpr (kEarlyRes) {
    const int r = threadIdx.x / (NT * 2), cg = threadIdx.x % (NT * 2);
    const int row = m0 + r, nb = n0 + cg * 8;
    if (r < ROWS && row < g.M) {
      const float* o = g.out_f32 + (size_t)row * g.ldo + nb;
      const float* gt = g.gate + (size_t)row * g.ldg + nb;
      res_pf[0] = fh_load_f4<COH>(o);
      res_pf[1] = fh_load_f4<COH>(o + 4);
      gate_pf[0] = fh_load_f4_stream(gt);
      gate_pf[1] = fh_load_f4_stream(gt + 4);
    }
  }

  P8 a[PF][MTW], b[PF][NT];
#pragma unroll
  for (int p = 0; p < PF; ++p) {
    if (p < KBw) {
#pragma unroll
      for (int j = 0; j < NT; ++j) b[p][j] = T::load8_nt(Wp + j * tstride + (size_t)p * 512);
#pragma unroll
      for (int i = 0; i < MTW; ++i) a[p][i] = ldA(Ap + i * tstride + (size_t)p * 512);
    }
  }
  constexpr bool kTouch = (EPI == EPI_GELU_P16 || EPI == EPI_T16 || EPI == EPI_GATE_RES || EPI == EPI_PARTIAL);
  unsigned touched[2] = {0u, 0u};
  if constexpr (kTouch) {
    if (g.touch.W) fmt_touch(g.touch, bid & 7, (bid >> 3) * NTHR + threadIdx.x, (nblk >> 3) * NTHR, touched);
  }
  for (int kb0 = 0; kb0 < KBw; kb0 += PF) {
#pragma unroll
    for (int p = 0; p < PF; ++p) {
      const int kb = kb0 + p;
      if (kb < KBw) {
#pragma unroll
        for (int i = 0; i < MTW; ++i)
#pragma unroll
          for (int j = 0; j < NT; ++j) acc[i][j] = T::mfma(a[p][i], b[p][j], acc[i][j]);
        if (kb + PF < KBw) {
#pragma unroll
          for (int j = 0; j < NT; ++j)
            b[p][j] = T::load8_nt(Wp + j * tstride + (size_t)(kb + PF) * 512);
#pragma unroll
          for (int i = 0; i < MTW; ++i) a[p][i] = ldA(Ap + i * tstride + (size_t)(kb + PF) * 512);
        }
      }
    }
  }

  if constexpr (kTouch) {
    if (g.touch.W) fmt_touch_retire(touched);
  }
  float* my = red + w * (ROWS * BN);
#pragma unroll
  for (int i = 0; i < MTW; ++i)
#pragma unroll
    for (int j = 0; j < NT; ++j)
#pragma unroll
      for (int r = 0; r < 4; ++r) my[(i * 16 + q * 4 + r) * BN + j * 16 + r16] = acc[i][j][r];
  __syncthreads();

  constexpr int S = ROWS * BN;
  constexpr int CG = BN / 8;
  unsigned rm = 0u;
  auto slab_sum = [&](int o) {
    float a = red[o];
#pragma unroll
    for (int ww = 1; ww < NW; ++ww) a += red[ww * S + o];
    return a;
  };
  if constexpr (EPI == EPI_CFG) {
    const int nclip = g.nclip > 1 ? g.nclip : 1;
    const int tb = g.tokblk ? by / nclip : 0, q = g.tokblk ? by - tb * nclip : 0;
    const int ni = g.tokblk ? 16 : g.ntok, i0 = tb * 16, rstride = g.tokblk ? 16 : g.ntok;
    float* const vout_q = g.vout ? g.vout + (size_t)q * g.ntok * g.N : nullptr;
    float* const xcur_q = g.xcur ? g.xcur + (size_t)q * (g.ntok - g.n_prev) * g.N : nullptr;
    for (int idx = threadIdx.x; idx < ni * BN; idx += NTHR) {
      const int il = idx / BN, i = i0 + il, c = idx % BN, n = n0 + c;
      if (i >= g.ntok) break;
      const float bias = g.bias[n];
      float v[4];
#pragma unroll
      for (int b2 = 0; b2 < 4; ++b2) {
        if (b2 < g.bc) {
          const int o = (b2 * rstride + il) * BN + c;
          v[b2] = slab_sum(o) + bias;
        } else {
          v[b2] = 0.f;
        }
      }
      float out;
      if (g.bc == 1) {
        out = v[0];
      } else if (g.bc == 3) {
        out = v[0] + g.a_cfg * (v[2] - v[0]) + g.e_cfg * (v[1] - v[2]);
      } else {
        out = v[0] + g.r_cfg * (v[1] - v[0]) + g.a_cfg * (v[3] - v[1]) + g.e_cfg * (v[2] - v[3]);
      }
      if (vout_q) vout_q[(size_t)i * g.N + n] = out;
      if (xcur_q && i >= g.n_prev) {
        const size_t xo = (size_t)(i - g.n_prev) * g.N + n;
        const float xn = xcur_q[xo] + g.dt * out;
        xcur_q[xo] = xn;
        reinterpret_cast<E*>(g.xin16)[fmt_pack_off(q * g.ntok + i, n, g.ldx)] = fh_cvt<T>(xn, rm);
      }
    }
  } else {
    for (int idx = threadIdx.x; idx < ROWS * CG; idx += NTHR) {
      const int r = idx / CG, cg = idx % CG;
      const int row = m0 + r, nb = n0 + cg * 8;
      if (row >= g.M) continue;
      float v[8];
      {
        const float* p0 = red + r * BN + cg * 8;
#pragma unroll
        for (int e = 0; e < 8; e += 4) {
          float4 a4 = *reinterpret_cast<const float4*>(p0 + e);
#pragma unroll
          for (int ww = 1; ww < NW; ++ww) {
            const float4 t4 = *reinterpret_cast<const float4*>(p0 + ww * S + e);
            a4.x += t4.x;
            a4.y += t4.y;
            a4.z += t4.z;
            a4.w += t4.w;
          }
          float4 bb = float4{0.f, 0.f, 0.f, 0.f};
          if constexpr (EPI != EPI_PARTIAL) bb = *reinterpret_cast<const float4*>(g.bias + nb + e);
          v[e + 0] = a4.x + bb.x;
          v[e + 1] = a4.y + bb.y;
          v[e + 2] = a4.z + bb.z;
          v[e + 3] = a4.w + bb.w;
        }
      }
      if constexpr (EPI == EPI_F32 || EPI == EPI_PARTIAL) {
        float* o = g.out_f32 + (size_t)ks * g.slab_stride + (size_t)row * g.ldo + nb;
        fh_store_f4_wt<fh_site<COH>(4), WT>(o, float4{v[0], v[1], v[2], v[3]});
        fh_store_f4_wt<fh_site<COH>(4), WT>(o + 4, float4{v[4], v[5], v[6], v[7]});
      } else if constexpr (EPI == EPI_T16 || EPI == EPI_SILU_P16 || EPI == EPI_GELU_P16 || EPI == EPI_GELUERF_P16) {
        P8 u;
#pragma unroll
        for (int i = 0; i < 8; ++i) {
          float x = v[i];
          if constexpr (EPI == EPI_SILU_P16) x = fh_silu(x);
          if constexpr (EPI == EPI_GELU_P16) x = fh_gelu_tanh(x);
          if constexpr (EPI == EPI_GELUERF_P16) x = fh_gelu_erf(x);
          T::set(u, i, x);
        }
        fh_track_pack<T>(rm, u);
        E* const o16 = reinterpret_cast<E*>(g.out16);
        if constexpr (EPI == EPI_T16) T::template store8_wt<fh_site<COH>(8), WT>(o16 + (size_t)row * g.ldo16 + nb, u);
        else T::template store8_wt<fh_site<COH>(8), WT>(o16 + fmt_pack_off(row, nb, g.ldo16), u);
      } else if constexpr (EPI == EPI_GATE_RES) {
        float* o = g.out_f32 + (size_t)row * g.ldo + nb;
        const float* gt = g.gate + (size_t)row * g.ldg + nb;
#pragma unroll
        for (int e = 0; e < 8; e += 4) {
          float4 x, gg;
          if constexpr (kEarlyRes) {
            x = res_pf[e / 4];
            gg = gate_pf[e / 4];
          } else {
            x = fh_load_f4<COH>(o + e);
            gg = fh_load_f4_stream(gt + e);
          }
          x.x += gg.x * v[e + 0];
          x.y += gg.y * v[e + 1];
          x.z += gg.z * v[e + 2];
          x.w += gg.w * v[e + 3];
          fh_store_f4_wt<fh_site<COH>(16), WT>(o + e, x);
        }
      } else if constexpr (EPI == EPI_XEMBED) {
        const int q = row / g.ntok, tok = row - q * g.ntok;
        const float* ps = g.pos + (size_t)tok * g.N + nb;
#pragma unroll
        for (int i = 0; i < 8; ++i) v[i] += ps[i];
        for (int b2 = 0; b2 < g.bc; ++b2) {
          float* o = g.out_f32 + (size_t)((q * g.bc + b2) * g.ntok + tok) * g.ldo + nb;
          fh_store_f4_wt<fh_site<COH>(32), WT>(o, float4{v[0], v[1], v[2], v[3]});
          fh_store_f4_wt<fh_site<COH>(32), WT>(o + 4, float4{v[4], v[5], v[6], v[7]});
        }
      }
    }
  }
  if constexpr (EPI == EPI_CFG || EPI == EPI_T16 || EPI == EPI_SILU_P16 || EPI == EPI_GELU_P16 || EPI == EPI_GELUERF_P16) fh_range_flush<T>(g.sat, rm);
}

template <class T, int MTW, int NT, int NW, int EPI>
__global__ __launch_bounds__(NW * 64) void fmt_gemm_kernel(GemmArgs g) {
  fmt_gemm_body<T, MTW, NT, NW, EPI, false>(g, blockIdx.x, gridDim.x);
}

template <class T, int MTW, int KCH , int NWV = 4>
__global__ __launch_bounds__(NWV * 64) void fmt_gemm_wide_kernel(GemmArgs g) {
  constexpr int EPI = EPI_F32;
  constexpr int NF = MTW * KCH;
  constexpr int NFW = (NF + NWV - 1) / NWV;
  constexpr int WR = NWV / 4, MTR = MTW / WR;
  static_assert(MTW % WR == 0, "row tiles must split evenly over the wave rows");
  extern __shared__ __attribute__((aligned(16))) unsigned char sA[];
  const int lane = threadIdx.x & 63, w = threadIdx.x >> 6, wc = w & 3, wr = w >> 2;
  const int r16 = lane & 15, q = lane >> 4;
  const int nbn = g.N >> 7;
  const int nbx = (EPI == EPI_PARTIAL) ? nbn * g.ksplit : nbn;
  int bx, by, bz = 0, ks = 0;
  {
    const int id = blockIdx.x;
    const int nz = g.zcount > 1 ? g.zcount : 1;
    if (nz > 1 && (nbx & 7) == 0 && g.zgroup > 1) {
      const int slot = id >> 3, G = g.zgroup, ncx = nbx >> 3, rows = g.mblk * nz;
      const int full = ncx / G, per_grp = G * rows;
      int grp = slot / per_grp, rem = slot - grp * per_grp, gw = G;
      if (grp >= full) {
        grp = full;
        rem = slot - full * per_grp;
        gw = ncx - full * G;
      }
      const int zy = rem / gw;
      bz = zy / g.mblk;
      by = zy - bz * g.mblk;
      bx = (grp * G + (rem - zy * gw)) * 8 + (id & 7);
    } else if ((nbx & 7) == 0) {
      const int slot = id >> 3, zy = slot % (g.mblk * nz);
      bz = zy / g.mblk;
      by = zy - bz * g.mblk;
      bx = (slot / (g.mblk * nz)) * 8 + (id & 7);
    } else {
      bx = id % nbx;
      const int zy = id / nbx;
      bz = zy / g.mblk;
      by = zy - bz * g.mblk;
    }
    if constexpr (EPI == EPI_PARTIAL) {
      if ((nbx & 7) == 0 && (8 % g.ksplit) == 0) {
        const int P = 8 / g.ksplit, x = bx & 7;
        ks = x / P;
        bx = (bx >> 3) * P + (x % P);
      } else {
        ks = bx / nbn;
        bx = bx % nbn;
      }
    }
  }
  const int mt0 = by * MTW;
  const int nb0 = bx * 8 + wc * 2;
  const int KB = g.K >> 5;
  const int KBs = (EPI == EPI_PARTIAL) ? KB / g.ksplit : KB;
  const int nchunk = KBs / KCH;
  const size_t tstride = (size_t)KB * 512;
  const u16* Wp = g.W + (size_t)nb0 * tstride + (size_t)ks * KBs * 512 + lane * 8;
  const u16* Ag = g.A + (size_t)bz * g.a_zstride + (size_t)mt0 * tstride + (size_t)ks * KBs * 512 + lane * 8;
  float* const outz = g.out_f32 + (size_t)bz * g.o_zstride + (size_t)ks * g.slab_stride;

  f32x4 acc[MTR][2];
#pragma unroll
  for (int i = 0; i < MTR; ++i) acc[i][0] = acc[i][1] = f32x4{0.f, 0.f, 0.f, 0.f};

  u32x4 an[NFW], bn[KCH][2], bc[KCH][2];
  auto issue = [&](int c) {
    const int kc = c * KCH;
#pragma unroll
    for (int f = 0; f < NFW; ++f) {
      const int fi = f * NWV + w;
      if (fi < NF) {
        const int i = fi / KCH, kk = fi % KCH;
        an[f] = *reinterpret_cast<const u32x4*>(Ag + i * tstride + (size_t)(kc + kk) * 512);
      }
    }
#pragma unroll
    for (int kk = 0; kk < KCH; ++kk) {
      bn[kk][0] = __builtin_nontemporal_load(reinterpret_cast<const u32x4*>(Wp + (size_t)(kc + kk) * 512));
      bn[kk][1] = __builtin_nontemporal_load(reinterpret_cast<const u32x4*>(Wp + tstride + (size_t)(kc + kk) * 512));
    }
  };
  auto commit = [&](int buf) {
#pragma unroll
    for (int f = 0; f < NFW; ++f) {
      const int fi = f * NWV + w;
      if (fi < NF) *reinterpret_cast<u32x4*>(sA + (buf * NF + fi) * 1024 + lane * 16) = an[f];
    }
#pragma unroll
    for (int kk = 0; kk < KCH; ++kk) {
      bc[kk][0] = bn[kk][0];
      bc[kk][1] = bn[kk][1];
    }
  };
  issue(0);
  commit(0);
  __syncthreads();
  for (int c = 0; c < nchunk; ++c) {
    const int buf = c & 1;
    if (c + 1 < nchunk) issue(c + 1);
#pragma unroll
    for (int kk = 0; kk < KCH; ++kk) {
#pragma unroll
      for (int i = 0; i < MTR; ++i) {
        const u32x4 a = *reinterpret_cast<const u32x4*>(sA + (buf * NF + (wr * MTR + i) * KCH + kk) * 1024 + lane * 16);
        acc[i][0] = T::mfma(bc[kk][0], a, acc[i][0]);
        acc[i][1] = T::mfma(bc[kk][1], a, acc[i][1]);
      }
    }
    if (c + 1 < nchunk) {
      commit(buf ^ 1);
      __syncthreads();
    }
  }
#pragma unroll
  for (int i = 0; i < MTR; ++i) {
// ... 86 lines not shown
#define DMA_WAIT(K)                                   \
  do {                                                \
    if (NHI == 0 || w < NHI) fh_wait_vmcnt<(K)*IMAX>(); \
    else fh_wait_vmcnt<(K)*ILO>();                    \
  } while (0)
  const unsigned abase = (unsigned)(lane * 16 + wr * 6 * 1024), bbase = (unsigned)(lane * 16 + (RT + wc * 5) * 1024);

  f32x4 acc[6][5];
#pragma unroll
  for (int i = 0; i < 6; ++i)
#pragma unroll
    for (int j = 0; j < 5; ++j) acc[i][j] = f32x4{0.f, 0.f, 0.f, 0.f};
  u32x4 a0[6], b0[5], a1[6], b1[5];

#define DMA_READ(S, AR, BR)                                        \
  do {                                                             \
    const unsigned so = (unsigned)(((S) % NS) * STAGE);            \
    AR[0] = fh_ds_read128<0>(abase + so);                          \
    AR[1] = fh_ds_read128<1024>(abase + so);                       \
    AR[2] = fh_ds_read128<2048>(abase + so);                       \
    AR[3] = fh_ds_read128<3072>(abase + so);                       \
    AR[4] = fh_ds_read128<4096>(abase + so);                       \
    AR[5] = fh_ds_read128<5120>(abase + so);                       \
    BR[0] = fh_ds_read128<0>(bbase + so);                          \
    BR[1] = fh_ds_read128<1024>(bbase + so);                       \
    BR[2] = fh_ds_read128<2048>(bbase + so);                       \
    BR[3] = fh_ds_read128<3072>(bbase + so);                       \
    BR[4] = fh_ds_read128<4096>(bbase + so);                       \
  } while (0)
#define DMA_STEP(S, AC, BC, AN, BN)                                                            \
  do {                                                                                         \
    const int s_ = (S);                                                                        \
    if (s_ + 1 < KB) {                                                                         \
      const int rem = KB - 2 - s_;                               \
      if (NS == 4 && rem >= 2) DMA_WAIT(2);                                                    \
      else if (rem >= 1) DMA_WAIT(1);                                                          \
      else DMA_WAIT(0);                                                                        \
    }                                                                                          \
    __builtin_amdgcn_s_barrier();                                                              \
    if (s_ + NS < KB) issue(s_ + NS);                                                          \
    if (s_ + 1 < KB) DMA_READ(s_ + 1, AN, BN);                                                 \
    __builtin_amdgcn_sched_barrier(0);                                                         \
    _Pragma("unroll") for (int i = 0; i < 6; ++i)                                              \
      _Pragma("unroll") for (int j = 0; j < 5; ++j) acc[i][j] = T::mfma(BC[j], AC[i], acc[i][j]); \
    __builtin_amdgcn_sched_barrier(0);                                                         \
    asm volatile("s_waitcnt lgkmcnt(0)" ::: "memory");                                         \
    __builtin_amdgcn_sched_barrier(0);                                                         \
  } while (0)

#define DMA_WAIT_UPTO(K)                      \
  do {                                        \
    const int k_ = (K);                       \
    if (NS == 4 && k_ >= 2) DMA_WAIT(2);      \
    else if (k_ >= 1) DMA_WAIT(1);            \
    else DMA_WAIT(0);                         \
  } while (0)
#define DMA_STEP_STG(S, AC, BC, AN, BN)                                                        \
  do {                                                                                         \
    const int s_ = (S);                                                                        \
    if (!g1 && s_ + 1 < KB) DMA_WAIT_UPTO(KB - 2 - s_);                                        \
    __builtin_amdgcn_s_barrier();                                                              \
    if (s_ + NS < KB) issue(s_ + NS);                                                          \
    if (s_ + 1 < KB) DMA_READ(s_ + 1, AN, BN);                                                 \
    asm volatile("s_waitcnt lgkmcnt(0)" ::: "memory");                                         \
    __builtin_amdgcn_sched_barrier(0);                                                         \
    if (g1 && s_ + 2 < KB) {                                                                   \
      DMA_WAIT_UPTO(KB - 3 - s_);                                                              \
    }                                                                                          \
    __builtin_amdgcn_s_barrier();                                                              \
    __builtin_amdgcn_sched_barrier(0);                                                         \
    _Pragma("unroll") for (int i = 0; i < 6; ++i)                                              \
      _Pragma("unroll") for (int j = 0; j < 5; ++j) acc[i][j] = T::mfma(BC[j], AC[i], acc[i][j]); \
    __builtin_amdgcn_sched_barrier(0);                                                         \
  } while (0)

  const bool g1 = wr == 1;
#ifdef DMA_CLK
  const unsigned long long c0 = clock64(), w0 = wall_clock64();
#endif
#pragma unroll
  for (int s = 0; s < NS; ++s) issue(s);
  if constexpr (STG) DMA_WAIT(NS - 2);
  else DMA_WAIT(NS - 1);
  __builtin_amdgcn_s_barrier();
  DMA_READ(0, a0, b0);
  asm volatile("s_waitcnt lgkmcnt(0)" ::: "memory");
  __builtin_amdgcn_sched_barrier(0);
  if constexpr (STG) {
    if (g1) __builtin_amdgcn_s_barrier();
    for (int s = 0; s < KB; s += 2) {
      DMA_STEP_STG(s, a0, b0, a1, b1);
      DMA_STEP_STG(s + 1, a1, b1, a0, b0);
    }
    if (!g1) __builtin_amdgcn_s_barrier();
  } else {
    for (int s = 0; s < KB; s += 2) {
      DMA_STEP(s, a0, b0, a1, b1);
      DMA_STEP(s + 1, a1, b1, a0, b0);
    }
  }
#ifdef DMA_CLK
  if ((blockIdx.x == 3000 || blockIdx.x == 6001) && threadIdx.x == 0) {
    const unsigned long long c1 = clock64(), w1 = wall_clock64();
    printf("tile loop: %llu core clocks, %llu wall ticks\n", c1 - c0, w1 - w0);
  }
#endif
#undef DMA_STEP_STG
#undef DMA_WAIT_UPTO
#undef DMA_STEP
#undef DMA_READ
#undef DMA_WAIT
  float* const outz = g.out_f32 + (size_t)bz * g.o_zstride;
  constexpr int OW = CT * 16, OSTR = OW + 4, C4 = OW / 4, NTHR = NW * 64;
  static_assert(96 * OSTR * 4 <= NS * STAGE, "output staging does not fit the ring");
  float* const so = reinterpret_cast<float*>(ring);
  float4 bb[5];
#pragma unroll
  for (int j = 0; j < 5; ++j) bb[j] = *reinterpret_cast<const float4*>(g.bias + (bx * CT + wc * 5 + j) * 16 + q * 4);
#pragma unroll
  for (int p = 0; p < 2; ++p) {
    if (wr == p) {
#pragma unroll
      for (int i = 0; i < 6; ++i)
#pragma unroll
        for (int j = 0; j < 5; ++j)
          *reinterpret_cast<float4*>(so + (i * 16 + r16) * OSTR + (wc * 5 + j) * 16 + q * 4) =
              float4{acc[i][j][0] + bb[j].x, acc[i][j][1] + bb[j].y, acc[i][j][2] + bb[j].z, acc[i][j][3] + bb[j].w};
    }
    __syncthreads();
    {
#pragma unroll
      for (int k = 0; k < (96 * C4) / NTHR; ++k) {
        const int idx = k * NTHR + threadIdx.x, rl = idx / C4, c4 = idx - rl * C4;
        const int row = by * (RT * 16) + p * 96 + rl;
        if (row < g.M)
          *reinterpret_cast<float4*>(outz + (size_t)row * g.ldo + bx * OW + c4 * 4) = *reinterpret_cast<const float4*>(so + rl * OSTR + c4 * 4);
      }
    }
    if (p == 0) __syncthreads();
  }
}

struct LnRed {
  const float* slab;
  size_t slab_stride;
  const float* bias;
  const float* gate;
};

constexpr int kLnTouch = 6;

template <class T, int NV, int KS, bool TOUCH, bool WT_, bool COH>
__device__ __forceinline__ void fmt_lnmod_body(float* __restrict__ x, int M, const float* __restrict__ shift,
                                               const float* __restrict__ scale, int ldm, u16* __restrict__ out, const LnRed& red,
                                               const TouchSpec& pf, int ntok, int perm, unsigned long long* sat, const unsigned bid,
                                               const unsigned nblk, const int wpb) {
  constexpr int D = NV * 256;
  constexpr bool WT = WT_ || COH;
  const int lane = threadIdx.x & 63;
  int row = bid * wpb + (threadIdx.x >> 6);
  unsigned touched[kLnTouch] = {};
  const unsigned tfirst = (bid >> 3) * 64 + lane, tstride = (nblk >> 3) * 64;
  const bool touch = TOUCH && wpb == 1;
  if (wpb == 1) {
    const int x = bid & 7, j = bid >> 3;
    row = (((j >> 3) * 8 + x) << 3) + (j & 7);
  }
  if (row >= M) {
    if (touch) {
      fmt_touch(pf, bid & 7, tfirst, tstride, touched);
      fmt_touch_retire(touched);
    }
    return;
  }
  float* xr = x + (size_t)row * D;
#ifdef FMT_DIAG_HOTMOD
  const size_t mrow = 0;
#else
  const size_t mrow = (size_t)row;
#endif
  const float* sh = shift + mrow * ldm;
  const float* sc = scale + mrow * ldm;
  float4 v[NV], a[NV], b[NV];
  float s = 0.f;
#pragma unroll
  for (int i = 0; i < NV; ++i) {
    const int c = i * 256 + lane * 4;
    v[i] = fh_load_f4<COH>(xr + c);
    a[i] = fh_load_f4_stream(sh + c);
    b[i] = fh_load_f4_stream(sc + c);
  }
  if (KS == 0 && touch) fmt_touch(pf, bid & 7, tfirst, tstride, touched);
  if constexpr (KS > 0) {
    float4 p[KS][NV], gt[NV], bi[NV];
#pragma unroll
    for (int i = 0; i < NV; ++i) {
      const int c = i * 256 + lane * 4;
#pragma unroll
      for (int k = 0; k < KS; ++k) {
        const float* ps = red.slab + k * red.slab_stride + (size_t)row * D + c;
        if constexpr (COH) p[k][i] = fh_load_f4<true>(ps);
        else p[k][i] = fh_load_f4_stream(ps);
      }
      gt[i] = fh_load_f4_stream(red.gate + mrow * ldm + c);
      bi[i] = *reinterpret_cast<const float4*>(red.bias + c);
    }
    if (touch) fmt_touch(pf, bid & 7, tfirst, tstride, touched);
#pragma unroll
    for (int i = 0; i < NV; ++i) {
      float4 t = p[0][i];
#pragma unroll
      for (int k = 1; k < KS; ++k) {
        t.x += p[k][i].x;
        t.y += p[k][i].y;
        t.z += p[k][i].z;
        t.w += p[k][i].w;
      }
      v[i].x += gt[i].x * (t.x + bi[i].x);
      v[i].y += gt[i].y * (t.y + bi[i].y);
      v[i].z += gt[i].z * (t.z + bi[i].z);
      v[i].w += gt[i].w * (t.w + bi[i].w);
      fh_store_f4_wt<fh_site<COH>(1), WT>(xr + i * 256 + lane * 4, v[i]);
    }
  }
#pragma unroll
  for (int i = 0; i < NV; ++i) s += (v[i].x + v[i].y) + (v[i].z + v[i].w);
  const float mu = wave_sum(s) * (1.f / D);
  float s2 = 0.f;
#pragma unroll
  for (int i = 0; i < NV; ++i) {
    const float d0 = v[i].x - mu, d1 = v[i].y - mu, d2 = v[i].z - mu, d3 = v[i].w - mu;
    s2 += (d0 * d0 + d1 * d1) + (d2 * d2 + d3 * d3);
  }
  const float rstd = rsqrtf(wave_sum(s2) * (1.f / D) + 1e-6f);
  unsigned rm = 0u;
  int orow = row;
  if (perm) {
    const int b = row / ntok, i = row - b * ntok;
    orow = (i >> 4) * perm + b * 16 + (i & 15);
  }
#pragma unroll
  for (int i = 0; i < NV; ++i) {
    const int c = i * 256 + lane * 4;
    fh_store4_wt<T, fh_site<COH>(1), WT>(reinterpret_cast<typename T::elem*>(out) + fmt_pack_off(orow, c, D / 32),
              (v[i].x - mu) * rstd * (1.f + b[i].x) + a[i].x, (v[i].y - mu) * rstd * (1.f + b[i].y) + a[i].y,
              (v[i].z - mu) * rstd * (1.f + b[i].z) + a[i].z, (v[i].w - mu) * rstd * (1.f + b[i].w) + a[i].w, rm);
  }
  fh_range_flush<T>(sat, rm);
  if (touch) fmt_touch_retire(touched);
}

template <class T, int NV, int KS, bool TOUCH, bool WT>
__global__ __launch_bounds__(256) void fmt_lnmod_kernel(float* __restrict__ x, int M, const float* __restrict__ shift,
                                                        const float* __restrict__ scale, int ldm, u16* __restrict__ out,
                                                        LnRed red, TouchSpec pf, int ntok, int perm, unsigned long long* sat) {
  fmt_lnmod_body<T, NV, KS, TOUCH, WT, false>(x, M, shift, scale, ldm, out, red, pf, ntok, perm, sat, blockIdx.x, gridDim.x,
                                              (int)(blockDim.x >> 6));
}

template <class T, int LPQ, bool TOUCH, bool WT_, bool COH>
__device__ __forceinline__ void fmt_attn_body(const u16* __restrict__ qkv, int ld, u16* __restrict__ out, int ntok, int M, int D,
                                              int window, const TouchSpec& pf, unsigned long long* sat, const int h, const int run,
                                              const int nthr, const unsigned lin, const unsigned nwg) {
  constexpr int HD = 128, PD = HD / LPQ, NU = PD / 8;
  constexpr bool WT = WT_ || COH;
  auto ld8 = [](const typename T::elem* p) -> typename T::pack8 {
    if constexpr (COH && !T::is32) return fh_load16<true>(p);
    else return T::load8(p);
  };
  const int row_ = run * (nthr / LPQ) + threadIdx.x / LPQ, part = threadIdx.x % LPQ;
  unsigned touched[2] = {0u, 0u};
  auto touch = [&]() {
    if constexpr (TOUCH) {
      fmt_touch(pf, lin & 7, (lin >> 3) * nthr + threadIdx.x, (nwg >> 3) * nthr, touched);
    }
  };
  if (row_ >= M) {
    touch();
    if constexpr (TOUCH) fmt_touch_retire(touched);
    return;
  }
  const int b = row_ / ntok, qi = row_ - b * ntok;
  const int d0 = h * HD + part * PD;
  const float scale = rsqrtf((float)HD);
  typedef typename T::elem E;
  typedef typename T::pack8 P8;
  const E* base = reinterpret_cast<const E*>(qkv) + (size_t)(b * ntok) * ld + d0;
  float qf[PD], o[PD];
#pragma unroll
  for (int u = 0; u < NU; ++u) {
    const P8 uu = ld8(base + (size_t)qi * ld + u * 8);
#pragma unroll
    for (int j = 0; j < 8; ++j) qf[u * 8 + j] = T::get(uu, j) * scale;
  }
#pragma unroll
  for (int i = 0; i < PD; ++i) o[i] = 0.f;
  float m = -INFINITY, l = 0.f;
  auto fold = [&](const P8* k, const P8* v, bool valid) {
    float dot = 0.f;
#pragma unroll
    for (int u = 0; u < NU; ++u) {
#pragma unroll
      for (int j = 0; j < 8; ++j) dot += qf[u * 8 + j] * T::get(k[u], j);
    }
#pragma unroll
    for (int d = 1; d < LPQ; d <<= 1) dot += __shfl_xor(dot, d, 64);
    if (!valid) return;
    const float mn = fmaxf(m, dot);
    const float alpha = __expf(m - mn), p = __expf(dot - mn);
    l = l * alpha + p;
    m = mn;
#pragma unroll
    for (int u = 0; u < NU; ++u) {
#pragma unroll
      for (int j = 0; j < 8; ++j) o[u * 8 + j] = o[u * 8 + j] * alpha + p * T::get(v[u], j);
    }
  };
  if (window <= 2) {
    P8 kk[5][NU], vv[5][NU];
#pragma unroll
    for (int t = 0; t < 5; ++t) {
      const int kj = min(max(qi + t - 2, 0), ntok - 1);
      const E* kp = base + (size_t)kj * ld + D;
#pragma unroll
      for (int u = 0; u < NU; ++u) {
        kk[t][u] = ld8(kp + u * 8);
        vv[t][u] = ld8(kp + D + u * 8);
      }
    }
    touch();
#pragma unroll
    for (int t = 0; t < 5; ++t) {
      const int kj = qi + t - 2;
      const bool valid = kj >= 0 && kj < ntok && (t - 2 >= -window) && (t - 2 <= window);
      fold(kk[t], vv[t], valid);
    }
  } else {
    touch();
    for (int kj = qi - window; kj <= qi + window; ++kj) {
      const int kc = min(max(kj, 0), ntok - 1);
      const E* kp = base + (size_t)kc * ld + D;
      P8 k[NU], v[NU];
#pragma unroll
      for (int u = 0; u < NU; ++u) {
        k[u] = ld8(kp + u * 8);
        v[u] = ld8(kp + D + u * 8);
      }
      fold(k, v, kj >= 0 && kj < ntok);
    }
  }
  const float inv = 1.f / l;
  const int row = b * ntok + qi;
  unsigned rm = 0u;
#pragma unroll
  for (int u = 0; u < NU; ++u) {
    P8 uo;
#pragma unroll
    for (int j = 0; j < 8; ++j) T::set(uo, j, o[u * 8 + j] * inv);
    fh_track_pack<T>(rm, uo);
    T::template store8_wt<fh_site<COH>(2), WT>(reinterpret_cast<E*>(out) + fmt_pack_off(row, d0 + u * 8, D / 32), uo);
  }
  fh_range_flush<T>(sat, rm);
  if constexpr (TOUCH) fmt_touch_retire(touched);
}

template <class T, int LPQ, bool TOUCH, bool WT>
__global__ __launch_bounds__(512) void fmt_attn_kernel(const u16* __restrict__ qkv, int ld, u16* __restrict__ out, int ntok,
                                                       int M, int D, int window, TouchSpec pf, unsigned long long* sat) {
  fmt_attn_body<T, LPQ, TOUCH, WT, false>(qkv, ld, out, ntok, M, D, window, pf, sat, blockIdx.x, blockIdx.y, blockDim.x,
                                          blockIdx.x + gridDim.x * blockIdx.y, gridDim.x * gridDim.y);
}

__device__ __forceinline__ float fh_sum8_dpp(float v) {
  v += __builtin_bit_cast(float, __builtin_amdgcn_mov_dpp(__builtin_bit_cast(int, v), 0xB1, 0xF, 0xF, true));
  v += __builtin_bit_cast(float, __builtin_amdgcn_mov_dpp(__builtin_bit_cast(int, v), 0x4E, 0xF, 0xF, true));
  v += __builtin_bit_cast(float, __builtin_amdgcn_mov_dpp(__builtin_bit_cast(int, v), 0x141, 0xF, 0xF, true));
  return v;
}

template <class T, int MTW, int HPW >
__global__ __launch_bounds__(512) void fmt_attnproj_kernel(const u16* __restrict__ qkv, int ld, GemmArgs g, int ntok, int D, int window) {
  constexpr int HD = 128, LPQ = 8, NU = HD / (LPQ * 8), KBH = HD / 32, NWV = 8, ROWS = MTW * 16;
  constexpr int NCT = NWV / HPW;
  constexpr int NPAIR = ROWS * HPW, NPASS = (NPAIR * LPQ + NWV * 64 - 1) / (NWV * 64);
  typedef typename T::elem E;
  typedef typename T::pack8 P8;
  __shared__ __attribute__((aligned(16))) E sO[HPW * MTW * KBH * 512];
  __shared__ __attribute__((aligned(16))) float sR[(HPW > 1 ? (HPW - 1) : 1) * NCT * MTW * 256];
  const int lane = threadIdx.x & 63, w = threadIdx.x >> 6, r16 = lane & 15, q4 = lane >> 4;
  const int ct = w % NCT, hh = w / NCT;
  int ks, bx, by;
  {
    const int id = blockIdx.x, nbn = g.N / (NCT * 16), nbx = nbn * g.ksplit;
    if ((nbx & 7) == 0 && (8 % g.ksplit) == 0) {
      const int slot = id >> 3, P = 8 / g.ksplit, x = id & 7;
      by = slot % g.mblk;
      ks = x / P;
      bx = (slot / g.mblk) * P + (x % P);
    } else {
      const int bxl = id % nbx;
      by = id / nbx;
      ks = bxl / nbn;
      bx = bxl - ks * nbn;
    }
  }
  const int KB = g.K >> 5;
  const int h0 = ks * HPW;
  const int nt = bx * NCT + ct;
  const E* Wp = reinterpret_cast<const E*>(g.W) + ((size_t)nt * KB + (h0 + hh) * KBH) * 512 + lane * 8;
// ... 15 lines not shown
      if (row_ < g.M) {
        const int bq = row_ / ntok, qi = row_ - bq * ntok;
        const E* base = reinterpret_cast<const E*>(qkv) + (size_t)(bq * ntok) * ld + (h0 + ah) * HD + part * 8;
        float qf[NU * 8], o[NU * 8];
        P8 qq[NU];
#pragma unroll
        for (int u = 0; u < NU; ++u) qq[u] = T::load8(base + (size_t)qi * ld + u * 64);
#pragma unroll
        for (int i = 0; i < NU * 8; ++i) o[i] = 0.f;
        float l = 0.f;
        auto dotk = [&](const P8* k) {
          float dot = 0.f;
#pragma unroll
          for (int u = 0; u < NU; ++u) {
#pragma unroll
            for (int j = 0; j < 8; ++j) dot += qf[u * 8 + j] * T::get(k[u], j);
          }
          return fh_sum8_dpp(dot);
        };
        if (window <= 2) {
          P8 kk[5][NU], vv[5][NU];
#pragma unroll
          for (int t = 0; t < 5; ++t) {
            const int kj = min(max(qi + t - 2, 0), ntok - 1);
            const E* kp = base + (size_t)kj * ld + D;
#pragma unroll
            for (int u = 0; u < NU; ++u) {
              kk[t][u] = T::load8(kp + u * 64);
              vv[t][u] = T::load8(kp + D + u * 64);
            }
          }
#pragma unroll
          for (int u = 0; u < NU; ++u) {
#pragma unroll
            for (int j = 0; j < 8; ++j) qf[u * 8 + j] = T::get(qq[u], j) * scale;
          }
          float dot[5], m = -INFINITY;
#pragma unroll
          for (int t = 0; t < 5; ++t) {
            const int kj = qi + t - 2;
            const bool valid = kj >= 0 && kj < ntok && (t - 2 >= -window) && (t - 2 <= window);
            dot[t] = valid ? dotk(kk[t]) : -INFINITY;
            m = fmaxf(m, dot[t]);
          }
#pragma unroll
          for (int t = 0; t < 5; ++t) {
            const float p = __expf(dot[t] - m);
            l += p;
#pragma unroll
            for (int u = 0; u < NU; ++u) {
#pragma unroll
              for (int j = 0; j < 8; ++j) o[u * 8 + j] += p * T::get(vv[t][u], j);
            }
          }
        } else {
#pragma unroll
          for (int u = 0; u < NU; ++u) {
#pragma unroll
            for (int j = 0; j < 8; ++j) qf[u * 8 + j] = T::get(qq[u], j) * scale;
          }
          float m = -INFINITY;
          for (int kj = max(qi - window, 0); kj <= min(qi + window, ntok - 1); ++kj) {
            const E* kp = base + (size_t)kj * ld + D;
            P8 k[NU], v[NU];
#pragma unroll
            for (int u = 0; u < NU; ++u) {
              k[u] = T::load8(kp + u * 64);
              v[u] = T::load8(kp + D + u * 64);
            }
            const float dot = dotk(k);
            const float mn = fmaxf(m, dot);
            const float alpha = __expf(m - mn), p = __expf(dot - mn);
            l = l * alpha + p;
            m = mn;
#pragma unroll
            for (int u = 0; u < NU; ++u) {
#pragma unroll
              for (int j = 0; j < 8; ++j) o[u * 8 + j] = o[u * 8 + j] * alpha + p * T::get(v[u], j);
            }
          }
        }
        const float inv = 1.f / l;
#pragma unroll
        for (int u = 0; u < NU; ++u) {
#pragma unroll
          for (int j = 0; j < 8; ++j) T::set(uo[u], j, o[u * 8 + j] * inv);
          fh_track_pack<T>(rm, uo[u]);
        }
      }
#pragma unroll
      for (int u = 0; u < NU; ++u) T::store8(sO + ah * (MTW * KBH * 512) + fmt_pack_off(qslot, u * 64 + part * 8, KBH), uo[u]);
    }
  }
  fh_range_flush<T>(g.sat, rm);
  __syncthreads();

  f32x4 acc[MTW];
#pragma unroll
  for (int i = 0; i < MTW; ++i) acc[i] = f32x4{0.f, 0.f, 0.f, 0.f};
  const E* const sOh = sO + hh * (MTW * KBH * 512);
#pragma unroll
  for (int kk = 0; kk < KBH; ++kk) {
#pragma unroll
    for (int i = 0; i < MTW; ++i) acc[i] = T::mfma(b[kk], T::load8(sOh + (i * KBH + kk) * 512 + lane * 8), acc[i]);
  }
  if constexpr (HPW > 1) {
    if (hh > 0) {
#pragma unroll
      for (int i = 0; i < MTW; ++i) *reinterpret_cast<f32x4*>(sR + (((hh - 1) * NCT + ct) * MTW + i) * 256 + lane * 4) = acc[i];
    }
    __syncthreads();
    if (hh > 0) return;
#pragma unroll
    for (int o = 1; o < HPW; ++o) {
#pragma unroll
      for (int i = 0; i < MTW; ++i) {
        const f32x4 t = *reinterpret_cast<const f32x4*>(sR + (((o - 1) * NCT + ct) * MTW + i) * 256 + lane * 4);
        acc[i] += t;
      }
    }
  }
  float* const outp = g.out_f32 + (size_t)ks * g.slab_stride + nt * 16 + q4 * 4;
#pragma unroll
  for (int i = 0; i < MTW; ++i) {
    const int row = (by * MTW + i) * 16 + r16;
    if (row < g.M) __builtin_nontemporal_store(acc[i], reinterpret_cast<f32x4*>(outp + (size_t)row * g.ldo));
  }
}

enum { MS_XEMBED = 0, MS_LN, MS_QKV, MS_ATTN, MS_PROJ, MS_FC1, MS_FC2, MS_HEAD };
struct MegaStage {
  int kind;
  unsigned nblk;
  GemmArgs g;
  long long gate_off;
  long long shift_off, scale_off, red_gate_off;
  int ks;
  const float* red_bias;
  u16* ln_out;
  int perm;
  TouchSpec pf;
  u16* att_out;
};
struct MegaCtx {
  float* xres;
  const u16* qkv16;
  const float* slab;
  size_t slab_stride;
  int M, D, ntok, ldm, window, heads;
  unsigned long long* sat;
};
struct MegaDyn {
  const float* mod;
  float dt, a, r, e;
  int euler;
  float* vout;
};
struct MegaSync {
  unsigned* grp;
  unsigned* top;
  unsigned* rel;
  unsigned* seq;
  unsigned* err;
  unsigned* err_host;
  unsigned long long* stamps;
  unsigned stamp_wg;
};

__device__ __forceinline__ bool fmt_grid_barrier(const MegaSync& sy, unsigned gen, unsigned nwg) {
  typedef __attribute__((address_space(1))) unsigned int gu32;
  const unsigned g = blockIdx.x & 7u, per = nwg >> 3;
  const unsigned old = __hip_atomic_fetch_add((gu32*)(sy.grp + g * 32), 1u, __ATOMIC_RELAXED, __HIP_MEMORY_SCOPE_AGENT);
  if (old + 1u == gen * per) {
    const unsigned t = __hip_atomic_fetch_add((gu32*)sy.top, 1u, __ATOMIC_RELAXED, __HIP_MEMORY_SCOPE_AGENT);
    if (t + 1u == gen * 8u) {
#pragma unroll
      for (int i = 0; i < 8; ++i) __hip_atomic_store((gu32*)(sy.rel + i * 32), gen, __ATOMIC_RELAXED, __HIP_MEMORY_SCOPE_AGENT);
    }
  }
  unsigned spins = 0;
  while ((int)(__hip_atomic_load((gu32*)(sy.rel + g * 32), __ATOMIC_RELAXED, __HIP_MEMORY_SCOPE_AGENT) - gen) < 0) {
    if (++spins > (1u << 18) || ((spins & 63u) == 0u && __hip_atomic_load((gu32*)sy.err, __ATOMIC_RELAXED, __HIP_MEMORY_SCOPE_AGENT) != 0u)) {
      __hip_atomic_store((gu32*)sy.err, 1u, __ATOMIC_RELAXED, __HIP_MEMORY_SCOPE_AGENT);
      if (sy.err_host) __hip_atomic_store((gu32*)sy.err_host, 1u, __ATOMIC_RELAXED, __HIP_MEMORY_SCOPE_SYSTEM);
      return false;
    }
    __builtin_amdgcn_s_sleep(1);
  }
  return true;
}

template <class T>
__global__ __launch_bounds__(512) void fmt_mega_kernel(const MegaStage* __restrict__ tab, int nstage, MegaDyn d, MegaCtx c,
                                                       MegaSync sy) {
  typedef __attribute__((address_space(1))) unsigned int gu32;
  __shared__ unsigned s_flag[2];
  const unsigned bid = blockIdx.x, nwg = gridDim.x;
  if (threadIdx.x == 0) {
    s_flag[0] = __hip_atomic_load((gu32*)sy.seq, __ATOMIC_RELAXED, __HIP_MEMORY_SCOPE_AGENT);
    s_flag[1] = 1u;
  }
  __syncthreads();
  const unsigned seq0 = s_flag[0];
  const unsigned gen0 = seq0 * (unsigned)(nstage - 1);
#ifdef MEGA_STAMPS
#define MEGA_STAMP(k) do { if (sy.stamps && bid == sy.stamp_wg && threadIdx.x == 0) sy.stamps[s * 3 + (k)] = __builtin_amdgcn_s_memrealtime(); } while (0)
#else
#define MEGA_STAMP(k) do { } while (0)
#endif
  for (int s = 0; s < nstage; ++s) {
    const MegaStage& st = tab[s];
    MEGA_STAMP(0);
    if (bid < st.nblk) {
      switch (st.kind) {
        case MS_XEMBED:
          fmt_gemm_body<T, 4, 1, 8, EPI_XEMBED, true>(st.g, bid, st.nblk);
          break;
        case MS_LN:
          if (threadIdx.x < 64) {
            const LnRed red{c.slab, c.slab_stride, st.red_bias, d.mod + st.red_gate_off};
            if (st.ks == 0)
              fmt_lnmod_body<T, 4, 0, true, true, true>(c.xres, c.M, d.mod + st.shift_off, d.mod + st.scale_off, c.ldm, st.ln_out, red,
                                                        st.pf, c.ntok, st.perm, c.sat, bid, st.nblk, 1);
            else
              fmt_lnmod_body<T, 4, 4, true, true, true>(c.xres, c.M, d.mod + st.shift_off, d.mod + st.scale_off, c.ldm, st.ln_out, red,
                                                        st.pf, c.ntok, st.perm, c.sat, bid, st.nblk, 1);
          }
          break;
        case MS_QKV:
          fmt_gemm_body<T, 3, 4, 8, EPI_T16, true>(st.g, bid, st.nblk);
          break;
        case MS_ATTN:
          if (threadIdx.x < 128)
            fmt_attn_body<T, 16, true, true, true>(c.qkv16, 3 * c.D, st.att_out, c.ntok, c.M, c.D, c.window, st.pf, c.sat,
                                                   (int)(bid % (unsigned)c.heads), (int)(bid / (unsigned)c.heads), 128, bid, st.nblk);
          break;
        case MS_PROJ: {
          GemmArgs g = st.g;
          g.gate = d.mod + st.gate_off;
          fmt_gemm_body<T, 3, 1, 8, EPI_GATE_RES, true>(g, bid, st.nblk);
          break;
        }
        case MS_FC1:
          fmt_gemm_body<T, 3, 4, 8, EPI_GELU_P16, true>(st.g, bid, st.nblk);
          break;
        case MS_FC2:
          fmt_gemm_body<T, 3, 4, 8, EPI_PARTIAL, true>(st.g, bid, st.nblk);
          break;
        default: {
          GemmArgs g = st.g;
          g.a_cfg = d.a;
          g.r_cfg = d.r;
          g.e_cfg = d.e;
          g.dt = d.dt;
          if (!d.euler) {
            g.xcur = nullptr;
            g.xin16 = nullptr;
            g.vout = d.vout;
          }
          fmt_gemm_body<T, 3, 1, 8, EPI_CFG, true>(g, bid, st.nblk);
          break;
        }
      }
    }
    MEGA_STAMP(1);
    if (s + 1 < nstage) {
      asm volatile("s_waitcnt vmcnt(0)" ::: "memory");
      __syncthreads();
      MEGA_STAMP(2);
      if (threadIdx.x == 0) {
        int pre = 0;
#pragma unroll
        for (int i = 0; i < (int)(sizeof(MegaStage) + 63) / 64; ++i) pre ^= reinterpret_cast<const int*>(&tab[s + 1])[i * 16];
        asm volatile("" ::"s"(pre));
        if (!fmt_grid_barrier(sy, gen0 + (unsigned)s + 1u, nwg)) s_flag[1] = 0u;
      }
      __syncthreads();
      if (s_flag[1] == 0u) return;
    }
  }
  if (bid == 0 && threadIdx.x == 0) __hip_atomic_store((gu32*)sy.seq, seq0 + 1u, __ATOMIC_RELAXED, __HIP_MEMORY_SCOPE_AGENT);
}

template <class T>
__global__ void fmt_build_cond_kernel(u16* __restrict__ out, int ld, int bc, int ntok, int n_prev, int dim_w, int dim_a,
                                      int dim_e, const float* __restrict__ wr, const float* __restrict__ wa,
                                      const float* __restrict__ prev_wa, const float* __restrict__ we, int we_len,
                                      const float* __restrict__ prev_we, unsigned wr_mask, unsigned wa_mask,
                                      unsigned we_mask, unsigned long long* sat) {
  const int row = blockIdx.x;
  const int s = row / ntok, i = row % ntok, q = s / bc, b = s - q * bc, n_cur = ntok - n_prev;
  const bool on_r = (wr_mask >> b) & 1, on_a = (wa_mask >> b) & 1, on_e = (we_mask >> b) & 1;
  wr += (size_t)q * dim_w;
  wa += (size_t)q * n_cur * dim_a;
  prev_wa += (size_t)q * n_prev * dim_a;
  we += (size_t)q * we_len * dim_e;
  if (prev_we) prev_we += (size_t)q * n_prev * dim_e;
  unsigned rm = 0u;
  for (int c = threadIdx.x; c < ld; c += blockDim.x) {
    float v = 0.f;
    if (c < dim_w) {
      v = on_r ? wr[c] : 0.f;
    } else if (c < dim_w + dim_a) {
      const int k = c - dim_w;
      if (i < n_prev) v = prev_wa[i * dim_a + k];
      else if (on_a) v = wa[(i - n_prev) * dim_a + k];
    } else if (c < dim_w + dim_a + dim_e) {
      const int k = c - dim_w - dim_a;
      if (on_e) {
        if (we_len == 1) v = we[k];
        else v = (i < n_prev) ? prev_we[i * dim_e + k] : we[(i - n_prev) * dim_e + k];
      }
    }
    reinterpret_cast<typename T::elem*>(out)[fmt_pack_off(row, c, ld / 32)] = fh_cvt<T>(v, rm);
  }
  fh_range_flush<T>(sat, rm);
}

__device__ __forceinline__ float fmt_linspace01(int i, int n) {
  if (n <= 1) return 0.f;
  const float step = __fdiv_rn(1.0f, (float)(n - 1));
  return (i < n / 2) ? __fmul_rn(step, (float)i) : __fsub_rn(1.0f, __fmul_rn(step, (float)(n - 1 - i)));
}
template <class T>
__global__ void fmt_tsin_kernel(u16* __restrict__ out, const float* __restrict__ freqs, int n_steps, float t0, int nfe,
                                int stages, float c0, float c1, float c2, float c3) {
  const int s = blockIdx.x;
  if (s >= n_steps) return;
  float t = t0;
  if (nfe > 0) {
    const int i = s / stages, j = s - i * stages;
    const float gi = fmt_linspace01(i, nfe);
    t = gi;
    if (j > 0) {
      const float cj = j == 1 ? c1 : (j == 2 ? c2 : c3);
      t = __fadd_rn(gi, __fmul_rn(__fsub_rn(fmt_linspace01(i + 1, nfe), gi), cj));
    }
  }
  (void)c0;
  const int k = threadIdx.x;
  const float arg = t * freqs[k & 127];
  reinterpret_cast<typename T::elem*>(out)[fmt_pack_off(s, k, 8)] = T::from_float(k < 128 ? cosf(arg) : sinf(arg));
}

template <class T>
__global__ void fmt_silu_c_kernel(u16* __restrict__ out, const float* __restrict__ temb, const float* __restrict__ ccond,
                                  int M, int D, size_t step_stride, int dense_rows, unsigned long long* sat) {
  const int idx = (blockIdx.x * blockDim.x + threadIdx.x) * 8;
  if (idx >= M * D) return;
  const int c = idx % D, row = idx / D + (int)blockIdx.y * dense_rows;
  typename T::elem* const o = reinterpret_cast<typename T::elem*>(out) + (dense_rows ? (size_t)0 : (size_t)blockIdx.y * step_stride);
  temb += (size_t)blockIdx.y * D;
  typename T::pack8 u;
#pragma unroll
  for (int h = 0; h < 2; ++h) {
    const float4 a = *reinterpret_cast<const float4*>(ccond + idx + 4 * h);
    const float4 t = *reinterpret_cast<const float4*>(temb + c + 4 * h);
    T::set(u, 4 * h + 0, fh_silu(a.x + t.x));
    T::set(u, 4 * h + 1, fh_silu(a.y + t.y));
    T::set(u, 4 * h + 2, fh_silu(a.z + t.z));
    T::set(u, 4 * h + 3, fh_silu(a.w + t.w));
  }
  unsigned rm = 0u;
  fh_track_pack<T>(rm, u);
  fh_range_flush<T>(sat, rm);
  T::store8(o + fmt_pack_off(row, c, D / 32), u);
}

template <class T>
__global__ void fmt_init_x_kernel(float* __restrict__ xcur, u16* __restrict__ xin16, int ldx, const float* __restrict__ x0,
                                  const float* __restrict__ prev_x, int n_prev, int n_cur, int dim_w, int nclip,
                                  unsigned long long* sat) {
  const int idx = blockIdx.x * blockDim.x + threadIdx.x;
  const int ntok = n_prev + n_cur;
  if (idx >= nclip * ntok * dim_w) return;
  const int q = idx / (ntok * dim_w), r = idx - q * ntok * dim_w;
  const int i = r / dim_w, c = r % dim_w;
  float v;
  if (i < n_prev) {
    v = prev_x[((size_t)q * n_prev + i) * dim_w + c];
  } else {
    v = x0[((size_t)q * n_cur + (i - n_prev)) * dim_w + c];
    xcur[((size_t)q * n_cur + (i - n_prev)) * dim_w + c] = v;
  }
  unsigned rm = 0u;
  reinterpret_cast<typename T::elem*>(xin16)[fmt_pack_off(q * ntok + i, c, ldx)] = fh_cvt<T>(v, rm);
  fh_range_flush<T>(sat, rm);
}

template <class T>
__global__ void fmt_rk_combine_kernel(float* __restrict__ xcur, const float* __restrict__ kbuf, size_t kstride, int nk, float c0,
                                      float c1, float c2, float c3, int final, u16* __restrict__ xin16, int ldx, int n_prev,
                                      int n_cur, int W, int nclip, unsigned long long* sat) {
  const int idx = blockIdx.x * blockDim.x + threadIdx.x;
  if (idx >= nclip * n_cur * W) return;
  const int q = idx / (n_cur * W), r = idx - q * n_cur * W;
  const int i = r / W, c = r % W, ntok = n_prev + n_cur;
  const float cf[4] = {c0, c1, c2, c3};
  float y = xcur[idx];
  for (int m = 0; m < nk; ++m) y += cf[m] * kbuf[(size_t)m * kstride + ((size_t)q * ntok + n_prev + i) * W + c];
  if (final) xcur[idx] = y;
  unsigned rm = 0u;
  reinterpret_cast<typename T::elem*>(xin16)[fmt_pack_off(q * ntok + n_prev + i, c, ldx)] = fh_cvt<T>(y, rm);
  fh_range_flush<T>(sat, rm);
}

__global__ void fmt_slice_pad_kernel(float* __restrict__ dst, const float* __restrict__ src, int t0, int T, int n, int dim,
                                     int nclip) {
  const int idx = blockIdx.x * blockDim.x + threadIdx.x;
  if (idx >= nclip * n * dim) return;
  const int q = idx / (n * dim), r = idx - q * n * dim;
  const int i = r / dim, c = r % dim;
  const int t = min(t0 + i, T - 1);
  dst[idx] = src[((size_t)q * T + t) * dim + c];
}

__global__ void fmt_tail_kernel(float* __restrict__ dst, const float* __restrict__ src, int n_prev, int n_cur, int dim, int nclip) {
  const int idx = blockIdx.x * blockDim.x + threadIdx.x;
  if (idx >= nclip * n_prev * dim) return;
  const int q = idx / (n_prev * dim), r = idx - q * n_prev * dim;
  dst[idx] = src[((size_t)q * n_cur + (n_cur - n_prev)) * dim + r];
}

template <class T>
__global__ void fmt_dbg_to16_kernel(u16* __restrict__ dst, const float* __restrict__ src, int n) {
  const int i = blockIdx.x * blockDim.x + threadIdx.x;
  if (i < n) reinterpret_cast<typename T::elem*>(dst)[i] = T::from_float(src[i]);
}
template <class T>
__global__ void fmt_dbg_unpack_kernel(float* __restrict__ dst, const u16* __restrict__ src, int rows, int D) {
  const int i = blockIdx.x * blockDim.x + threadIdx.x;
  if (i >= rows * D) return;
  const int r = i / D, c = i - r * D;
  dst[i] = T::to_float(reinterpret_cast<const typename T::elem*>(src)[fmt_pack_off(r, c, D / 32)]);
}

__global__ void fmt_copy_kernel(float* __restrict__ dst, size_t dpitch, const float* __restrict__ src, size_t spitch, int width, int rows) {
  const int idx = blockIdx.x * blockDim.x + threadIdx.x;
  if (idx >= rows * width) return;
  const int r = idx / width, c = idx - r * width;
  dst[(size_t)r * dpitch + c] = src ? src[(size_t)r * spitch + c] : 0.f;
}
```

### comfyui-float_optimized_amd/csrc/fmt_pack.hpp

```cpp
#pragma once
#include "common.hpp"

enum {
  EPI_F32 = 0,
  EPI_T16 = 1,
  EPI_SILU_P16 = 2,
  EPI_GELU_P16 = 3,
  EPI_GATE_RES = 4,
  EPI_XEMBED = 5,
  EPI_CFG = 6,
  EPI_PARTIAL = 7,
  EPI_GELUERF_P16 = 8
};

__host__ __device__ __forceinline__ size_t fmt_pack_off(int row, int k, int KB) {
  return ((size_t)((row >> 4) * KB + (k >> 5)) * 64 + (row & 15) + 16 * ((k >> 3) & 3)) * 8 + (k & 7);
}

struct TouchSpec {
  const char* W;
  unsigned run_shift;
  unsigned nt_shift;
  unsigned p_shift;
  unsigned tile_bytes;
  unsigned total;
};

__device__ __forceinline__ unsigned fmt_touch_line(const TouchSpec& t, unsigned xcd, unsigned l) {
  if (l >= t.total) return 0u;
  const unsigned r = l >> t.run_shift, off = l & ((1u << t.run_shift) - 1u);
  const unsigned cb = r >> t.nt_shift, jn = r & ((1u << t.nt_shift) - 1u);
  const unsigned ks = xcd >> t.p_shift, bx = (cb << t.p_shift) + (xcd & ((1u << t.p_shift) - 1u));
  return *reinterpret_cast<const unsigned*>(t.W + (size_t)((bx << t.nt_shift) + jn) * t.tile_bytes +
                                            ((size_t)((ks << t.run_shift) + off) << 7));
}
template <int N>
__device__ __forceinline__ void fmt_touch(const TouchSpec& t, unsigned xcd, unsigned first, unsigned stride, unsigned (&v)[N]) {
#pragma unroll
  for (int i = 0; i < N; ++i) v[i] = fmt_touch_line(t, xcd, first + (unsigned)i * stride);
}
template <int N>
__device__ __forceinline__ void fmt_touch_retire(const unsigned (&v)[N]) {
  unsigned o = 0u;
#pragma unroll
  for (int i = 0; i < N; ++i) o |= v[i];
  asm volatile("" ::"v"(o));
}

struct GemmArgs {
  const u16* A;
  const u16* W;
  const float* bias;
  int K, M, N;
  int mblk;
  float* out_f32;
  int ldo;
  u16* out16;
  int ldo16;
  const float* gate;
  int ldg;
  const float* pos;
  int bc, ntok, n_prev;
  int nclip;
  float a_cfg, r_cfg, e_cfg, dt;
  float* vout;
  float* xcur;
  u16* xin16;
  int ldx;
  int ksplit;
  size_t slab_stride;
  TouchSpec touch;
  int zcount, zgroup;
  size_t a_zstride, o_zstride;
  int tokblk;
  unsigned long long* sat;
};
```

### comfyui-float_optimized_amd/csrc/tuning.hpp

```cpp
#pragma once
#include <stdio.h>
#include <stdlib.h>
#include <string.h>

#include <algorithm>
#include <string>

inline int env_int(const char* name, int dflt, int lo, int hi) {
  const char* v = getenv(name);
  if (!v || !*v) return dflt;
  char* end = nullptr;
  const long x = strtol(v, &end, 10);
  return (end && *end == 0 && x >= lo && x <= hi) ? (int)x : dflt;
}
inline int env_atoi(const char* name, int dflt) {
  const char* v = getenv(name);
  return v ? atoi(v) : dflt;
}
inline bool env_set(const char* name) { return getenv(name) != nullptr; }
inline int env_scan(const char* s, int* v) { int n = 0; return sscanf(s, "%d%n", v, &n) == 1 ? n : 0; }
inline int env_scan(const char* s, double* v) { int n = 0; return sscanf(s, "%lf%n", v, &n) == 1 ? n : 0; }
template <class V>
int env_list(const char* name, V* v, int n, char sep = ',') {
  const char* s = getenv(name);
  int got = 0;
  while (s && got < n) {
    const int used = env_scan(s, v + got);
    if (!used) break;
    ++got;
    s += used;
    if (sep == ',' && *s++ != ',') break;
  }
  return got;
}

struct LayerPlan {
  int v[3] = {0, 0, 0};
  bool on() const { return v[0] > 0; }
};

enum { RB_QKV = 0, RB_PROJ, RB_FC1, RB_FC2 };

struct FmtTune {
  bool wide = true;
  int wide_variant = 7;
  bool big = true;
  bool rb = true;
  int rb_touch = 16;
  struct Rb {
    int n = 0, shape = -1, ksplit = 1;
  } rb_layer[4];
  int full_nw = 8;
  int plan[6] = {0, 0, 0, 0, 0, 0};
  LayerPlan plan_layer[4];
  int fc2_split = 4;
  int proj_split = 0;
  int touch = 230;
  bool hoist = true;
  int zgroup = 0;
  int ln_rows = 1;
  int attn_qpw = 8, attn_lpq = 16;
  bool no_tokblk = false;
  int attnproj = 0;
  int mega = 0;
  int mega_stamp_wg = 0;
  bool pack_host = false;

  static FmtTune from_env() {
    FmtTune t;
    t.wide = env_atoi("FLOAT_FMT_WIDE", 1) != 0;
    t.wide_variant = env_atoi("FLOAT_FMT_WIDE_VARIANT", t.wide_variant);
    t.big = env_atoi("FLOAT_FMT_BIG", 1) != 0;
    t.rb = env_atoi("FLOAT_FMT_RB", 1) != 0;
    t.rb_touch = env_atoi("FLOAT_FMT_RB_TOUCH", t.rb_touch);
    static const char* const layers[4] = {"QKV", "PROJ", "FC1", "FC2"};
    for (int l = 0; l < 4; ++l) {
      const std::string s = layers[l];
      int rb[2] = {-1, 1};
      t.rb_layer[l].n = env_list(("FLOAT_FMT_RB_" + s).c_str(), rb, 2);
      t.rb_layer[l].shape = rb[0];
      t.rb_layer[l].ksplit = rb[1];
      env_list(("FLOAT_FMT_PLAN_" + s).c_str(), t.plan_layer[l].v, 3);
    }
    t.full_nw = env_atoi("FLOAT_FMT_FULL_NW", t.full_nw);
    env_list("FLOAT_FMT_PLAN", t.plan, 6);
    t.fc2_split = env_atoi("FLOAT_FMT_FC2_SPLIT", t.fc2_split);
    t.proj_split = env_atoi("FLOAT_FMT_PROJ_SPLIT", t.proj_split);
    t.touch = env_atoi("FLOAT_FMT_TOUCH", t.touch);
    t.hoist = env_atoi("FLOAT_FMT_HOIST", 1) != 0;
    t.zgroup = std::max(0, env_atoi("FLOAT_FMT_ZGROUP", 0));
    t.ln_rows = std::max(1, std::min(4, env_atoi("FLOAT_FMT_LN_ROWS", 1)));
    int attn[2] = {t.attn_qpw, t.attn_lpq};
    env_list("FLOAT_FMT_ATTN", attn, 2);
    t.attn_lpq = attn[1] == 16 ? 16 : 8;
    t.attn_qpw = std::max(1, std::min(512 / t.attn_lpq, attn[0]));
    t.no_tokblk = env_set("FLOAT_FMT_NO_TOKBLK");
    t.attnproj = env_atoi("FLOAT_FMT_ATTNPROJ", 0);
    t.mega = env_atoi("FLOAT_FMT_MEGA", 0);
    t.mega_stamp_wg = env_atoi("FLOAT_FMT_MEGA_STAMP_WG", 0);
    t.pack_host = env_atoi("FLOAT_PACK_HOST", 0) != 0;
    return t;
  }
};

struct DecTune {
  int lds_pad = 0;
  unsigned ride_wgs = 16;
  int ride_min_res = 64;
  unsigned ride_pace = 3;
  bool ride_equal = false;
  double ride_w[4][3] = {{170, 140, 50}, {170, 155, 100}, {220, 200, 180}, {300, 250, 120}};
  int ride_tail = 0;
#ifdef DEC_STAMPS
  int ride_test = 0;
#endif
  bool cb_order = true;
  int conv_bn = 64, conv_bn_lo = 32;
  int tpw = 0;
  int conv_db = 0;
  bool no_zfuse = false;
  int zblur_min = 64;
  int flow_pix = 0;
  int flow_wgs = 2048;
  bool flow_epi = true;
  bool write_pyr = false;
  bool copy_memcpy = false;
  bool short_first = true;
  bool style_norm = true;

  static DecTune from_env() {
    DecTune t;
    t.lds_pad = env_int("FLOAT_DEC_LDS_PAD", 0, 0, 160 * 1024);
    t.ride_wgs = (unsigned)env_int("FLOAT_DEC_RIDE_WGS", 16, 0, 64) / 8 * 8;
    t.ride_min_res = env_int("FLOAT_DEC_RIDE_MIN_RES", 64, 64, 512);
    t.ride_pace = (unsigned)env_int("FLOAT_DEC_RIDE_PACE", 3, 0, 64);
    t.ride_equal = env_set("FLOAT_DEC_RIDE_EQUAL");
    double w[12];
    if (env_list("FLOAT_DEC_RIDE_W", w, 12, ' ') == 12)
      for (int i = 0; i < 12; ++i)
        if (w[i] > 0.0 && w[i] < 1e6) t.ride_w[i / 3][i % 3] = w[i];
    t.ride_tail = env_atoi("FLOAT_DEC_RIDE_TAIL", 0);
#ifdef DEC_STAMPS
    t.ride_test = env_int("FLOAT_DEC_RIDE_TEST", 0, 0, 2);
#endif
    t.cb_order = env_atoi("FLOAT_DEC_CB_ORDER", 1) != 0;
    t.conv_bn = env_int("FLOAT_DEC_CONV_BN", 64, 32, 64);
    t.conv_bn_lo = env_int("FLOAT_DEC_CONV_BN_LO", 32, 32, 64);
    t.tpw = env_int("FLOAT_DEC_TPW", 0, 0, 4096);
    t.conv_db = env_int("FLOAT_DEC_CONV_DB", 0, 0, 3);
    t.no_zfuse = env_set("FLOAT_DEC_NO_ZFUSE");
    t.zblur_min = env_int("FLOAT_DEC_ZBLUR_MIN", 64, 16, 4096);
    t.flow_pix = env_int("FLOAT_DEC_FLOW_PIX", 0, 0, 4);
    t.flow_wgs = env_int("FLOAT_DEC_FLOW_WGS", 2048, 8, 1 << 20);
    t.flow_epi = env_int("FLOAT_DEC_FLOW_EPI", 1, 0, 1) != 0;
    t.write_pyr = env_set("FLOAT_DEC_WRITE_PYR");
    const char* copy = getenv("FLOAT_DEC_COPY");
    t.copy_memcpy = copy && !strcmp(copy, "memcpy");
    t.short_first = env_int("FLOAT_DEC_SHORT_FIRST", 1, 0, 1) != 0;
    t.style_norm = env_int("FLOAT_DEC_STYLE_NORM", 1, 0, 1) != 0;
    return t;
  }
};

struct EncTune {
  bool no_tiles = false;
  static EncTune from_env() { return EncTune{env_set("FLOAT_ENC_NO_TILES")}; }
};

struct AudTune {
  bool attn_mfma = true;
  static AudTune from_env() { return AudTune{env_atoi("FLOAT_AUD_ATTN_MFMA", 1) != 0}; }
};
```

### comfyui-float_optimized_amd/fmt.py

```python
import ctypes as C
import math

import torch

from . import native
from .config import FmtConfig


@native.rebuildable
class FlowMatchingTransformerHIP:

    def __init__(self, state_dict, cfg: FmtConfig = None, device="cuda:0", dtype="fp16", use_graph=2, max_batch=1):
        self.cfg = cfg or FmtConfig()
        self.device = torch.device(device)
        self.dtype = dtype = native.canon_dtype(dtype)
        self.max_batch = max(1, int(max_batch))
        L = native.lib()
        c = self.cfg
        ncfg = native.FmtCfg(c.dim_w, c.dim_a, c.dim_e, c.dim_h, c.fmt_depth, c.num_heads,
                             int(c.dim_h * c.mlp_ratio), c.num_prev_frames, c.num_frames_for_clip,
                             c.attention_window, native.DTYPES[dtype], int(use_graph), self.max_batch)
        sd = {k[4:] if k.startswith("fmt.") else k: v for k, v in state_dict.items()
              if k not in ("alignment_mask", "fmt.alignment_mask")}
        arr, keep = native.tensor_table(sd)
        h = C.c_void_p()
        with torch.cuda.device(self.device):
            native.check(L.float_fmt_create(C.byref(ncfg), arr, len(sd), C.byref(h)))
        self._h = h
        del keep

    def set_method(self, name):
        if name not in native.ODE_METHODS:
            raise ValueError("unknown fixed-step ODE method %r (known: %s)" % (name, ", ".join(native.ODE_METHODS)))
        native.check(native.lib().float_fmt_set_method(self._h, native.ODE_METHODS[name]))
        self.method = name

    @torch.no_grad()
    def pos_embed_in_use(self):
        out = torch.empty(self.cfg.n_tokens, self.cfg.dim_h, device=self.device, dtype=torch.float32)
        with torch.cuda.device(self.device):
            native.check(native.lib().float_fmt_debug(self._h, 0, None, native.dev_ptr(out), native.stream_ptr(self.device)))
        return out

    @torch.no_grad()
    def attention_probe(self, qkv):
        qkv = self._f(qkv)
        if qkv.shape != (self.cfg.n_tokens, 3 * self.cfg.dim_h):
            raise ValueError("qkv must be (%d,%d)" % (self.cfg.n_tokens, 3 * self.cfg.dim_h))
        out = torch.empty(self.cfg.n_tokens, self.cfg.dim_h, device=self.device, dtype=torch.float32)
        with torch.cuda.device(self.device):
            native.check(native.lib().float_fmt_debug(self._h, 1, native.dev_ptr(qkv), native.dev_ptr(out),
                                                      native.stream_ptr(self.device)))
        return out

    def saturation(self, reset=False):
        with torch.cuda.device(self.device):
            return native.saturation("float_fmt_saturation", self._h, self.device, reset)

    def close(self):
        if getattr(self, "_h", None) and native is not None:
            native.lib().float_fmt_destroy(self._h)
            self._h = None

    __del__ = close

    def _f(self, t):
        return None if t is None else t.to(self.device, torch.float32).contiguous()

    def _check_shapes(self, x, wa, wr, we, prev_x, prev_wa, prev_we):
        c = self.cfg
        B = x.shape[0]
        if x.shape != (B, c.num_frames_for_clip, c.dim_w):
            raise ValueError("x must be (B,%d,%d), got %s" % (c.num_frames_for_clip, c.dim_w, tuple(x.shape)))
        if wa.shape != (B, c.num_frames_for_clip, c.dim_a):
            raise ValueError("wa must be (B,%d,%d), got %s" % (c.num_frames_for_clip, c.dim_a, tuple(wa.shape)))
        if wr.shape != (B, c.dim_w):
            raise ValueError("wr must be (B,%d), got %s" % (c.dim_w, tuple(wr.shape)))
        if prev_x is None or prev_wa is None:
            raise ValueError("prev_x was provided, but prev_wa was not." if prev_x is not None
                             else "prev_x / prev_wa are required")
        if we.dim() != 3 or we.shape[2] != c.dim_e:
            raise ValueError("we must be (B,1|%d,%d)" % (c.num_frames_for_clip, c.dim_e))
        if we.shape[1] > 1 and prev_we is None:
            raise ValueError("`we` is dynamic (T>1), but prev_we was not provided with prev_x/prev_wa.")
        if we.shape[1] not in (1, c.num_frames_for_clip):
            raise ValueError("Dynamic emotion latent `we` time dimension (%d) does not match audio latent `wa` "
                             "time dimension (%d)." % (we.shape[1] + c.num_prev_frames,
                                                       c.num_frames_for_clip + c.num_prev_frames))

    @torch.no_grad()
    def forward_with_cfv(self, t, x, wa, wr, we, prev_x, prev_wa, prev_we=None, a_cfg_scale=1.0, r_cfg_scale=1.0,
                         e_cfg_scale=1.0, include_r_cfg=False, **kwargs):
        x, wa, wr, we, prev_x, prev_wa, prev_we = map(self._f, (x, wa, wr, we, prev_x, prev_wa, prev_we))
        self._check_shapes(x, wa, wr, we, prev_x, prev_wa, prev_we)
        c, L = self.cfg, native.lib()
        tval = float(torch.as_tensor(t).reshape(-1)[0])
        B = x.shape[0]
        out = torch.empty(B, c.n_tokens, c.dim_w, device=self.device, dtype=torch.float32)
        dynamic = we.shape[1] > 1
        with torch.cuda.device(self.device):
            s = native.stream_ptr(self.device)
            for b in range(B):
                native.check(L.float_fmt_eval(
                    self._h, tval, native.dev_ptr(x[b]), native.dev_ptr(wa[b]), native.dev_ptr(wr[b]),
                    native.dev_ptr(we[b]), we.shape[1], native.dev_ptr(prev_x[b]), native.dev_ptr(prev_wa[b]),
                    native.dev_ptr(prev_we[b]) if dynamic else None, a_cfg_scale, r_cfg_scale, e_cfg_scale,
                    1 if include_r_cfg else 0, native.dev_ptr(out[b]), s))
        return out

    @torch.no_grad()
    def sample_chunk(self, x0, wa, wr, we, prev_x, prev_wa, prev_we=None, nfe=10, a_cfg_scale=1.0, r_cfg_scale=1.0,
                     e_cfg_scale=1.0, include_r_cfg=False):
        x0, wa, wr, we, prev_x, prev_wa, prev_we = map(self._f, (x0, wa, wr, we, prev_x, prev_wa, prev_we))
        self._check_shapes(x0, wa, wr, we, prev_x, prev_wa, prev_we)
        c, L = self.cfg, native.lib()
        B = x0.shape[0]
        out = torch.empty(B, c.num_frames_for_clip, c.dim_w, device=self.device, dtype=torch.float32)
        dynamic = we.shape[1] > 1
        with torch.cuda.device(self.device):
            s = native.stream_ptr(self.device)
            for b in range(B):
                native.check(L.float_fmt_sample_chunk(
                    self._h, native.dev_ptr(x0[b]), native.dev_ptr(wa[b]), native.dev_ptr(wr[b]),
                    native.dev_ptr(we[b]), we.shape[1], native.dev_ptr(prev_x[b]), native.dev_ptr(prev_wa[b]),
                    native.dev_ptr(prev_we[b]) if dynamic else None, int(nfe), a_cfg_scale, r_cfg_scale, e_cfg_scale,
                    1 if include_r_cfg else 0, native.dev_ptr(out[b]), s))
        return out

    @torch.no_grad()
    def sample(self, r_s, wa, we, noise, nfe=10, a_cfg_scale=2.0, r_cfg_scale=1.0, e_cfg_scale=1.0,
               include_r_cfg=False):
        r_s, wa, we, noise = map(self._f, (r_s, wa, we, noise))
        c, L = self.cfg, native.lib()
        B, T = wa.shape[0], wa.shape[1]
        n_chunks = int(math.ceil(T / c.num_frames_for_clip))
        if noise.shape != (n_chunks, B, c.num_frames_for_clip, c.dim_w):
            raise ValueError("noise must be (%d,%d,%d,%d), got %s" % (n_chunks, B, c.num_frames_for_clip, c.dim_w,
                                                                      tuple(noise.shape)))
        if we.shape[1] not in (1, T):
            raise ValueError("Dynamic emotion latent `we` time dimension (%d) does not match audio latent `wa` "
                             "time dimension (%d)." % (we.shape[1], T))
        r_d = torch.empty(B, T, c.dim_w, device=self.device, dtype=torch.float32)
        with torch.cuda.device(self.device):
            s = native.stream_ptr(self.device)
            for b0 in range(0, B, self.max_batch):
                nb = min(self.max_batch, B - b0)
                nz = noise[:, b0:b0 + nb].contiguous()
                native.check(L.float_fmt_sample_batch(
                    self._h, nb, native.dev_ptr(r_s[b0:b0 + nb]), native.dev_ptr(wa[b0:b0 + nb]), T,
                    native.dev_ptr(we[b0:b0 + nb]), we.shape[1], native.dev_ptr(nz), int(nfe), a_cfg_scale, r_cfg_scale,
                    e_cfg_scale, 1 if include_r_cfg else 0, native.dev_ptr(r_d[b0:b0 + nb]), s))
        return r_d


class WindowSampler:

    def __init__(self, fmt, r_s, wa, we, noise, nfe, a_cfg_scale, r_cfg_scale, e_cfg_scale, include_r_cfg=False,
                 windows=None, hist=None, r_d=None):
        self.fmt = fmt
        c = fmt.cfg
        f = fmt._f
        self.r_s, self.wa, self.we = f(r_s).reshape(-1), f(wa).reshape(-1, c.dim_a), f(we).reshape(-1, c.dim_e)
        self.T = self.wa.shape[0]
        self.n_chunks = int(math.ceil(self.T / c.num_frames_for_clip))
        self.noise = f(noise).reshape(self.n_chunks, c.num_frames_for_clip, c.dim_w)
        self.r_d = torch.empty(1, self.T, c.dim_w, device=fmt.device, dtype=torch.float32) if r_d is None else r_d
        w0, w1 = windows if windows is not None else (0, self.n_chunks)
        self.left = w1 - w0
        args = (fmt._h, native.dev_ptr(self.r_s), native.dev_ptr(self.wa), self.T, native.dev_ptr(self.we),
                self.we.shape[0], native.dev_ptr(self.noise), int(nfe), a_cfg_scale, r_cfg_scale, e_cfg_scale,
                1 if include_r_cfg else 0, native.dev_ptr(self.r_d))
        with torch.cuda.device(fmt.device):
            if windows is None and hist is None:
                native.check(native.lib().float_fmt_sample_begin(*args))
            else:
                self._hist = [None if t is None else f(t).reshape(c.num_prev_frames, -1) for t in (hist or (None, None, None))]
                native.check(native.lib().float_fmt_sample_begin_range(
                    *args, int(w0), int(w1), *[native.dev_ptr(t) if t is not None else None for t in self._hist]))

    def next(self):
        k, left = C.c_int32(0), C.c_int32(0)
        with torch.cuda.device(self.fmt.device):
            native.check(native.lib().float_fmt_sample_next(self.fmt._h, native.stream_ptr(self.fmt.device),
                                                            C.byref(k), C.byref(left)))
        self.left = left.value
        L = self.fmt.cfg.num_frames_for_clip
        return k.value, (k.value * L, min(self.T, (k.value + 1) * L))


def draw_noise(n_chunks, batch, cfg, seed, device="cpu"):
    g = torch.Generator(device)
    g.manual_seed(int(seed))
    return torch.stack([torch.randn(batch, cfg.num_frames_for_clip, cfg.dim_w, generator=g, device=device)
                        for _ in range(n_chunks)])
```

### comfyui-float_optimized_amd/native.py

```python
import ctypes as C
import os

import torch

_HERE = os.path.dirname(os.path.abspath(__file__))
LIB_PATH = os.path.join(_HERE, "csrc", "libfloat_hip.so")

FLOAT_DT_BF16, FLOAT_DT_FP16, FLOAT_DT_FP32 = 0, 1, 2
ODE_METHODS = {"euler": 0, "midpoint": 1, "rk4": 2, "heun2": 3, "heun3": 4}
DTYPES = {"bf16": FLOAT_DT_BF16, "bfloat16": FLOAT_DT_BF16, "fp16": FLOAT_DT_FP16, "float16": FLOAT_DT_FP16,
          "fp32": FLOAT_DT_FP32, "float32": FLOAT_DT_FP32}
DTYPE_NAMES = {FLOAT_DT_BF16: "bf16", FLOAT_DT_FP16: "fp16", FLOAT_DT_FP32: "fp32"}
DEC_SAT_SITES = 40
ABI_VERSION = 6


def canon_dtype(dtype):
    try:
        return DTYPE_NAMES[DTYPES[str(dtype)]]
    except KeyError:
        raise ValueError("unknown dtype %r (one of %s)" % (dtype, ", ".join(sorted(DTYPES)))) from None


class NativeLibraryError(RuntimeError):
    pass


class FloatTensor(C.Structure):
    _fields_ = [("name", C.c_char_p), ("data", C.POINTER(C.c_float)), ("ndim", C.c_int32),
                ("shape", C.c_int64 * 6)]


class FmtCfg(C.Structure):
    _fields_ = [(n, C.c_int32) for n in ("dim_w", "dim_a", "dim_e", "dim_h", "depth", "heads", "mlp_hidden",
                                         "n_prev", "n_cur", "attn_window", "dtype", "use_graph", "max_batch")]


class DecCfg(C.Structure):
    _fields_ = [(n, C.c_int32) for n in ("size", "style_dim", "dtype", "max_frames")]


class DecUnit(C.Structure):
    _fields_ = [(n, C.c_int32) for n in ("dtype", "cin", "cout", "res", "upsample", "n_frames", "style_dim", "flags")]


class EncCfg(C.Structure):
    _fields_ = [(n, C.c_int32) for n in ("size", "dim", "dim_motion", "dtype")]


class AudCfg(C.Structure):
    _fields_ = [("n_conv", C.c_int32), ("conv_dim", C.c_int32 * 8), ("conv_kernel", C.c_int32 * 8), ("conv_stride", C.c_int32 * 8)] + \
               [(n, C.c_int32) for n in ("hidden", "layers", "heads", "intermediate", "pos_k", "pos_groups", "dim_w", "only_last",
                                         "dtype")] + [("ln_eps", C.c_float)] + \
               [(n, C.c_int32) for n in ("feat_norm_layer", "stable_ln", "conv_bias", "num_labels")]


_F = C.POINTER(C.c_float)
_SIGNATURES = {
    "float_hip_abi_version": (C.c_int, []),
    "float_last_error": (C.c_char_p, []),
    "float_set_profiling": (C.c_int, [C.c_int32]),
    "float_probe_peaks": (C.c_int, [C.POINTER(C.c_float)] * 4 + [C.POINTER(C.c_int32)]),
    "float_profile_ms": (C.c_double, [C.c_int32, C.POINTER(C.c_int64)]),
    "float_stream_create_cu_range": (C.c_int, [C.c_int32, C.c_int32, C.POINTER(C.c_void_p)]),
    "float_stream_destroy": (C.c_int, [C.c_void_p]),
    "float_fmt_create": (C.c_int, [C.POINTER(FmtCfg), C.POINTER(FloatTensor), C.c_int32, C.POINTER(C.c_void_p)]),
    "float_fmt_destroy": (None, [C.c_void_p]),
    "float_fmt_set_method": (C.c_int, [C.c_void_p, C.c_int32]),
    "float_fmt_debug": (C.c_int, [C.c_void_p, C.c_int32, C.c_void_p, C.c_void_p, C.c_void_p]),
    "float_fmt_eval": (C.c_int, [C.c_void_p, C.c_float] + [C.c_void_p] * 4 + [C.c_int32] + [C.c_void_p] * 3 +
                       [C.c_float] * 3 + [C.c_int32, C.c_void_p, C.c_void_p]),
    "float_fmt_sample_chunk": (C.c_int, [C.c_void_p] + [C.c_void_p] * 4 + [C.c_int32] + [C.c_void_p] * 3 +
                               [C.c_int32] + [C.c_float] * 3 + [C.c_int32, C.c_void_p, C.c_void_p]),
    "float_fmt_sample": (C.c_int, [C.c_void_p, C.c_void_p, C.c_void_p, C.c_int32, C.c_void_p, C.c_int32, C.c_void_p,
                                   C.c_int32] + [C.c_float] * 3 + [C.c_int32, C.c_void_p, C.c_void_p]),
    "float_fmt_sample_batch": (C.c_int, [C.c_void_p, C.c_int32, C.c_void_p, C.c_void_p, C.c_int32, C.c_void_p, C.c_int32,
                                         C.c_void_p, C.c_int32] + [C.c_float] * 3 + [C.c_int32, C.c_void_p, C.c_void_p]),
    "float_fmt_sample_begin": (C.c_int, [C.c_void_p, C.c_void_p, C.c_void_p, C.c_int32, C.c_void_p, C.c_int32, C.c_void_p,
                                         C.c_int32] + [C.c_float] * 3 + [C.c_int32, C.c_void_p]),
    "float_fmt_sample_next": (C.c_int, [C.c_void_p, C.c_void_p, C.POINTER(C.c_int32), C.POINTER(C.c_int32)]),
    "float_fmt_sample_begin_range": (C.c_int, [C.c_void_p, C.c_void_p, C.c_void_p, C.c_int32, C.c_void_p, C.c_int32, C.c_void_p,
                                               C.c_int32] + [C.c_float] * 3 + [C.c_int32, C.c_void_p, C.c_int32, C.c_int32] +
                                     [C.c_void_p] * 3),
    "float_dec_create": (C.c_int, [C.POINTER(DecCfg), C.POINTER(FloatTensor), C.c_int32, C.POINTER(C.c_void_p)]),
    "float_dec_destroy": (None, [C.c_void_p]),
    "float_dec_set_feats": (C.c_int, [C.c_void_p, C.POINTER(C.c_void_p), C.c_int32, C.c_void_p]),
    "float_dec_frames": (C.c_int, [C.c_void_p, C.c_void_p, C.c_void_p, C.c_int32, C.c_void_p, C.c_void_p]),
    "float_dec_frames_host": (C.c_int, [C.c_void_p, C.c_void_p, C.c_void_p, C.c_int32, C.c_void_p, C.c_void_p, C.c_void_p,
                                        C.c_void_p]),
    "float_dec_frames_u8": (C.c_int, [C.c_void_p, C.c_void_p, C.c_void_p, C.c_int32, C.c_void_p, C.c_void_p]),
    "float_dec_frames_host_u8": (C.c_int, [C.c_void_p, C.c_void_p, C.c_void_p, C.c_int32, C.c_void_p, C.c_void_p, C.c_void_p,
                                           C.c_void_p]),
    "float_dec_feat_shape": (C.c_int, [C.c_void_p, C.c_int32, C.POINTER(C.c_int32), C.POINTER(C.c_int32)]),
    "float_dec_frames_raw": (C.c_int, [C.c_void_p, C.c_void_p, C.c_void_p, C.c_int32, C.c_void_p, C.c_void_p]),
    "float_dec_direction": (C.c_int, [C.c_void_p, C.c_void_p, C.c_void_p, C.c_void_p]),
    "float_dec_saturation": (C.c_int, [C.c_void_p, C.POINTER(C.c_uint64), C.POINTER(C.c_uint64), C.c_int32, C.c_void_p]),
    "float_dec_debug_styled_conv": (C.c_int, [C.POINTER(DecUnit), C.POINTER(FloatTensor), C.c_int32, C.c_void_p, C.c_void_p,
                                              C.c_void_p, C.POINTER(C.c_uint64), C.c_void_p]),
    "float_dec_debug_flow_level": (C.c_int, [C.POINTER(DecUnit), C.POINTER(FloatTensor), C.c_int32] + [C.c_void_p] * 9),
    "float_dec_set_feats16": (C.c_int, [C.c_void_p, C.POINTER(C.c_void_p), C.c_int32, C.c_int32, C.c_void_p]),
    "float_enc_create": (C.c_int, [C.POINTER(EncCfg), C.POINTER(FloatTensor), C.c_int32, C.POINTER(C.c_void_p)]),
    "float_enc_destroy": (None, [C.c_void_p]),
    "float_enc_forward": (C.c_int, [C.c_void_p] * 5 + [C.POINTER(C.c_void_p), C.c_int32, C.c_void_p]),
    "float_aud_create": (C.c_int, [C.POINTER(AudCfg), C.POINTER(FloatTensor), C.c_int32, C.POINTER(C.c_void_p)]),
    "float_aud_destroy": (None, [C.c_void_p]),
    "float_aud_reserve": (C.c_int, [C.c_void_p, C.c_int32, C.c_int32, C.c_void_p]),
    "float_aud_classify": (C.c_int, [C.c_void_p, C.c_void_p, C.c_int32, C.c_void_p, C.c_void_p]),
    "float_aud_inference": (C.c_int, [C.c_void_p, C.c_void_p, C.c_int32, C.c_int32, C.c_void_p, C.c_void_p]),
    "float_enc_feats16": (C.c_int, [C.c_void_p, C.POINTER(C.c_void_p), C.POINTER(C.c_int32), C.c_int32, C.POINTER(C.c_int32)]),
    "float_enc_export_feats16": (C.c_int, [C.c_void_p, C.POINTER(C.c_void_p), C.c_int32, C.c_void_p]),
    "float_fmt_saturation": (C.c_int, [C.c_void_p, C.POINTER(C.c_uint64), C.c_int32, C.c_void_p]),
    "float_enc_saturation": (C.c_int, [C.c_void_p, C.POINTER(C.c_uint64), C.c_int32, C.c_void_p]),
    "float_aud_saturation": (C.c_int, [C.c_void_p, C.POINTER(C.c_uint64), C.c_int32, C.c_void_p]),
    "float_cmp_segments": (C.c_int, [C.c_void_p, C.c_void_p, C.c_int32, C.c_int64, C.c_float, C.c_void_p, C.c_void_p, C.c_size_t,
                                     C.c_void_p]),
    "float_cmp_work_bytes": (C.c_size_t, [C.c_int32, C.c_int64]),
}
EXPORTS = tuple(_SIGNATURES)

_lib = None


def lib():
    global _lib
    if _lib is not None:
        return _lib
    if not os.path.exists(LIB_PATH):
        raise NativeLibraryError(
            "libfloat_hip.so not built: run `python -c 'import __graft_entry__ as g; g.build()'` or "
            "`make -C comfyui-float_optimized_amd/csrc` (there is no CPU fallback)")
    try:
        L = C.CDLL(LIB_PATH)
    except OSError as e:
        raise NativeLibraryError("cannot load %s: %s" % (LIB_PATH, e)) from e
    for name, (res, args) in _SIGNATURES.items():
        try:
            fn = getattr(L, name)
        except AttributeError as e:
            raise NativeLibraryError("libfloat_hip.so does not export %s" % name) from e
        fn.restype = res
        fn.argtypes = args
    if L.float_hip_abi_version() != ABI_VERSION:
        raise NativeLibraryError("libfloat_hip.so ABI version mismatch")
    _lib = L
    return L


_ERR_TYPES = {1: ValueError, 2: KeyError, 3: RuntimeError, 4: MemoryError}


def check(rc):
    if rc != 0:
        msg = lib().float_last_error().decode("utf-8", "replace")
        raise _ERR_TYPES.get(rc, RuntimeError)(msg)


def tensor_table(state):
    keep = []
    arr = (FloatTensor * len(state))()
    for i, (k, v) in enumerate(state.items()):
        t = v.detach().to("cpu", torch.float32).contiguous()
        nm = k.encode()
        keep.append((t, nm))
        arr[i].name = nm
        arr[i].data = C.cast(t.data_ptr(), _F)
        arr[i].ndim = t.dim()
        for d in range(t.dim()):
            arr[i].shape[d] = t.shape[d]
    return arr, keep


def dev_ptr(t, name="tensor"):
    if t is None:
        return None
    if not t.is_cuda:
        raise ValueError("%s must live on the GPU" % name)
    if t.dtype != torch.float32 or not t.is_contiguous():
        raise TypeError("%s must be contiguous float32" % name)
    return C.c_void_p(t.data_ptr())


def stream_ptr(device=None):
    return C.c_void_p(torch.cuda.current_stream(device).cuda_stream)


def cu_range_stream(cu_begin, cu_end, device=None):
    p = C.c_void_p()
    check(lib().float_stream_create_cu_range(int(cu_begin), int(cu_end), C.byref(p)))
    return torch.cuda.ExternalStream(p.value, device=device)


def saturation(fn_name, handle, device=None, reset=False):
    tot = C.c_uint64(0)
    check(getattr(lib(), fn_name)(handle, C.byref(tot), 1 if reset else 0, stream_ptr(device)))
    return int(tot.value)


CMP_STATS = ("sum_sq_diff", "sum_sq_ref", "max_abs", "beyond_thr", "non_finite")
_cmp_work = {}


def cmp_segments(a, b, seg_len, thr=2.0 / 255):
    if not a.is_cuda or a.device != b.device or a.numel() != b.numel():
        raise ValueError("cmp_segments: a and b must hold the same number of elements on one GPU")
    seg_len = int(seg_len)
    if seg_len <= 0 or a.numel() == 0 or a.numel() % seg_len:
        raise ValueError("cmp_segments: %d elements are not whole segments of %d" % (a.numel(), seg_len))
    n_seg = a.numel() // seg_len
    L = lib()
    need = int(L.float_cmp_work_bytes(n_seg, seg_len))
    with torch.cuda.device(a.device):
        s = stream_ptr(a.device)
        key = (a.device.index, s.value)
        work = _cmp_work.get(key)
        if work is None or work.numel() * 8 < need:
            work = _cmp_work[key] = torch.empty((need + 7) // 8, dtype=torch.float64, device=a.device)
        stats = torch.empty(n_seg, len(CMP_STATS), dtype=torch.float64, device=a.device)
        check(L.float_cmp_segments(dev_ptr(a, "a"), dev_ptr(b, "b"), n_seg, seg_len, float(thr), C.c_void_p(stats.data_ptr()),
                                   C.c_void_p(work.data_ptr()), work.numel() * 8, s))
    return stats


def set_profiling(on):
    check(lib().float_set_profiling(1 if on else 0))


def profile_ms(which):
    n = C.c_int64(0)
    ms = lib().float_profile_ms(which, C.byref(n))
    return ms, n.value


def rebuildable(cls):
    init = cls.__init__

    def __init__(self, *a, **k):
        if "_ctor" not in self.__dict__:
            self._ctor = (a, k)
        init(self, *a, **k)

    def offload(self):
        self.close()

    def to_target(self):
        if not self.__dict__.get("_h"):
            a, k = self._ctor
            type(self).__init__(self, *a, **k)
        return self

    cls.__init__ = __init__
    cls.offload = offload
    cls.to_target = to_target
    cls.resident = property(lambda self: bool(self.__dict__.get("_h")))
    return cls


def probe_peaks(device=None):
    v = [C.c_float(0) for _ in range(4)]
    n = C.c_int32(0)
    with torch.cuda.device(device if device is not None else torch.cuda.current_device()):
        torch.cuda.synchronize()
        check(lib().float_probe_peaks(C.byref(v[0]), C.byref(v[1]), C.byref(v[2]), C.byref(v[3]), C.byref(n)))
    return {"hbm_read_GBps": round(v[0].value, 1), "hbm_copy_GBps": round(v[1].value, 1), "mfma_f16_16x16x32_TFLOPs": round(v[2].value, 1),
            "mfma_f16_32x32x16_TFLOPs": round(v[3].value, 1), "compute_units": n.value}
```

### include/float_hip.h

```cpp
#ifndef FLOAT_HIP_H
#define FLOAT_HIP_H

#include <stddef.h>
#include <stdint.h>

#ifdef __cplusplus
extern "C" {
#endif

#define FLOAT_HIP_ABI_VERSION 6

enum {
  FLOAT_OK = 0,
  FLOAT_E_INVALID = 1,
  FLOAT_E_MISSING = 2,
  FLOAT_E_HIP = 3,
  FLOAT_E_NOMEM = 4
};

enum { FLOAT_DT_BF16 = 0, FLOAT_DT_FP16 = 1, FLOAT_DT_FP32 = 2 };

typedef struct {
  const char* name;
  const float* data;
  int32_t ndim;
  int64_t shape[6];
} float_tensor_t;

typedef struct {
  int32_t dim_w, dim_a, dim_e, dim_h;
  int32_t depth, heads;
  int32_t mlp_hidden;
  int32_t n_prev, n_cur;
  int32_t attn_window;
  int32_t dtype;
  int32_t use_graph;
  int32_t max_batch;
} float_fmt_cfg_t;

typedef struct float_fmt float_fmt_t;

int float_fmt_create(const float_fmt_cfg_t* cfg, const float_tensor_t* tensors, int32_t n_tensors,
                     float_fmt_t** out);
void float_fmt_destroy(float_fmt_t* h);

enum { FLOAT_ODE_EULER = 0, FLOAT_ODE_MIDPOINT = 1, FLOAT_ODE_RK4 = 2, FLOAT_ODE_HEUN2 = 3, FLOAT_ODE_HEUN3 = 4 };
int float_fmt_set_method(float_fmt_t* h, int32_t method);

int float_fmt_saturation(float_fmt_t* h, uint64_t* total, int32_t reset, void* stream);

int float_fmt_eval(float_fmt_t* h, float t, const float* x, const float* wa, const float* wr,
                   const float* we, int32_t we_len, const float* prev_x, const float* prev_wa,
                   const float* prev_we, float a_cfg, float r_cfg, float e_cfg, int32_t include_r_cfg,
                   float* out, void* stream);

int float_fmt_sample_chunk(float_fmt_t* h, const float* x0, const float* wa, const float* wr,
                           const float* we, int32_t we_len, const float* prev_x, const float* prev_wa,
                           const float* prev_we, int32_t nfe, float a_cfg, float r_cfg, float e_cfg,
                           int32_t include_r_cfg, float* out, void* stream);

int float_fmt_sample(float_fmt_t* h, const float* wr, const float* wa, int32_t T, const float* we,
                     int32_t we_len, const float* noise, int32_t nfe, float a_cfg, float r_cfg,
                     float e_cfg, int32_t include_r_cfg, float* r_d, void* stream);

int float_fmt_sample_batch(float_fmt_t* h, int32_t n_clips, const float* wr, const float* wa, int32_t T,
                           const float* we, int32_t we_len, const float* noise, int32_t nfe, float a_cfg,
                           float r_cfg, float e_cfg, int32_t include_r_cfg, float* r_d, void* stream);

int float_fmt_sample_begin(float_fmt_t* h, const float* wr, const float* wa, int32_t T, const float* we,
                           int32_t we_len, const float* noise, int32_t nfe, float a_cfg, float r_cfg,
                           float e_cfg, int32_t include_r_cfg, float* r_d);
int float_fmt_sample_next(float_fmt_t* h, void* stream, int32_t* window_done, int32_t* windows_left);

int float_fmt_sample_begin_range(float_fmt_t* h, const float* wr, const float* wa, int32_t T, const float* we,
                                 int32_t we_len, const float* noise, int32_t nfe, float a_cfg, float r_cfg,
                                 float e_cfg, int32_t include_r_cfg, float* r_d, int32_t first_window,
                                 int32_t end_window, const float* hist_x, const float* hist_wa, const float* hist_we);

int float_fmt_debug(float_fmt_t* h, int32_t what, const float* in, float* out, void* stream);

typedef struct {
  int32_t size;
  int32_t style_dim;
  int32_t dtype;
  int32_t max_frames;
} float_dec_cfg_t;

typedef struct float_dec float_dec_t;

int float_dec_create(const float_dec_cfg_t* cfg, const float_tensor_t* tensors, int32_t n_tensors,
                     float_dec_t** out);
void float_dec_destroy(float_dec_t* h);

int float_dec_set_feats(float_dec_t* h, const float* const* feats, int32_t n_feats, void* stream);

int float_dec_frames(float_dec_t* h, const float* s_r, const float* r_d, int32_t n_frames,
                     float* out_hwc, void* stream);

int float_dec_frames_host(float_dec_t* h, const float* s_r, const float* r_d, int32_t n_frames,
                          float* out_hwc, float* host_hwc, void* stream, void* copy_stream);

int float_dec_frames_u8(float_dec_t* h, const float* s_r, const float* r_d, int32_t n_frames,
                        uint8_t* out_hwc, void* stream);
int float_dec_frames_host_u8(float_dec_t* h, const float* s_r, const float* r_d, int32_t n_frames,
                             uint8_t* out_hwc, uint8_t* host_hwc, void* stream, void* copy_stream);

int float_dec_feat_shape(float_dec_t* h, int32_t i, int32_t* channels, int32_t* resolution);

int float_dec_frames_raw(float_dec_t* h, const float* s_r, const float* r_d, int32_t n_frames,
                         float* out_chw, void* stream);

#define FLOAT_DEC_SAT_SITES 40
int float_dec_saturation(float_dec_t* h, uint64_t* total, uint64_t* per_site, int32_t reset, void* stream);

typedef struct {
  int32_t dtype;
  int32_t cin, cout;
  int32_t res;
  int32_t upsample;
  int32_t n_frames;
  int32_t style_dim;
  int32_t flags;
} float_dec_unit_t;
int float_dec_debug_styled_conv(const float_dec_unit_t* u, const float_tensor_t* tensors, int32_t n_tensors, const float* x,
                                const float* style, float* out, uint64_t* saturated, void* stream);
int float_dec_debug_flow_level(const float_dec_unit_t* u, const float_tensor_t* tensors, int32_t n_tensors, const float* x,
                               const float* feat, const float* style, const float* prev_flow, const float* prev_rgb,
                               float* out_flow, float* out_blend, float* out_rgb, void* stream);

int float_dec_direction(float_dec_t* h, const float* lam, float* r_s, void* stream);

int float_dec_set_feats16(float_dec_t* h, const void* const* feats16, int32_t n_feats, int32_t dtype,
                          void* stream);

typedef struct {
  int32_t size;
  int32_t dim;
  int32_t dim_motion;
  int32_t dtype;
} float_enc_cfg_t;

typedef struct float_enc float_enc_t;

int float_enc_create(const float_enc_cfg_t* cfg, const float_tensor_t* tensors, int32_t n_tensors,
                     float_enc_t** out);
void float_enc_destroy(float_enc_t* h);

int float_enc_forward(float_enc_t* h, const float* img, float* s_r, float* lam, float* r_s,
                      float* const* feats, int32_t n_feats, void* stream);

int float_enc_saturation(float_enc_t* h, uint64_t* total, int32_t reset, void* stream);
int float_enc_feats16(float_enc_t* h, const void** feats16, int32_t* channels, int32_t max_feats,
                      int32_t* n_out);
int float_enc_export_feats16(float_enc_t* h, void* const* dst, int32_t n_feats, void* stream);

typedef struct {
  int32_t n_conv;
  int32_t conv_dim[8], conv_kernel[8], conv_stride[8];
  int32_t hidden, layers, heads, intermediate;
  int32_t pos_k, pos_groups;
  int32_t dim_w;
  int32_t only_last;
  int32_t dtype;
  float ln_eps;
  int32_t feat_norm_layer;
  int32_t stable_ln;
  int32_t conv_bias;
  int32_t num_labels;
} float_aud_cfg_t;

typedef struct float_aud float_aud_t;

int float_aud_create(const float_aud_cfg_t* cfg, const float_tensor_t* tensors, int32_t n_tensors,
                     float_aud_t** out);
void float_aud_destroy(float_aud_t* h);

int float_aud_reserve(float_aud_t* h, int32_t n_samples, int32_t seq_len, void* stream);
int float_aud_saturation(float_aud_t* h, uint64_t* total, int32_t reset, void* stream);

int float_aud_inference(float_aud_t* h, const float* a, int32_t n_samples, int32_t seq_len, float* wa,
                        void* stream);

int float_aud_classify(float_aud_t* h, const float* a, int32_t n_samples, float* scores, void* stream);

int float_hip_abi_version(void);
const char* float_last_error(void);
int float_stream_create_cu_range(int32_t cu_begin, int32_t cu_end, void** stream_out);
int float_stream_destroy(void* stream);
int float_set_profiling(int32_t on);
double float_profile_ms(int32_t which, int64_t* n_launches);
int float_probe_peaks(float* hbm_read_gbps, float* hbm_copy_gbps, float* mfma16_tflops, float* mfma32_tflops, int32_t* n_cu);

int float_cmp_segments(const float* a, const float* b, int32_t n_seg, int64_t seg_len, float thr, double* stats, void* work,
                       size_t work_bytes, void* stream);
size_t float_cmp_work_bytes(int32_t n_seg, int64_t seg_len);

#ifdef __cplusplus
}
#endif
#endif
```

Baseline: 2336 frames/s.

## Deduplicate adaLN modulation rows across CFG branches via a row map

Builds a host-side map that finds which token rows across the CFG batch share identical conditioning (same reference/audio/emotion masks and token index), then computes the adaLN modulation GEMM only for the distinct rows. LayerNorm-modulate kernels, gate-residual epilogues and the persistent mega kernel look up their modulation row through the map. This shrinks the per-step modulation GEMM and its output buffer, at the cost of an extra indirect load per row in several kernels.

```diff
diff --git a/comfyui-float_optimized_amd/csrc/fmt_api.hip b/comfyui-float_optimized_amd/csrc/fmt_api.hip
--- a/comfyui-float_optimized_amd/csrc/fmt_api.hip
+++ b/comfyui-float_optimized_amd/csrc/fmt_api.hip
@@ -3,6 +3,7 @@
 
 #include "fmt_gemm.hpp"
 #include "fmt_kernels.hpp"
+#include "fmt_modrows.hpp"
 #include "fmt_rb_kernels.hpp"
 #include "fmt_big_kernels.hpp"
 
@@ -48,6 +49,11 @@
   float* modall = nullptr;
   int Mmod = 0;
   size_t mod_zs = 0;
+  struct RowMap {
+    int* dev = nullptr;
+    int rows1 = 0, dist1 = 0;
+  } rowmap[3][2];
+  int last_rows = 0, last_dist = 0;
   struct GraphKey {
     int nfe, bc, we_len, method, nclip;
     int prio;
@@ -564,7 +570,7 @@
 }
 
 template <class T>
-int launch_lnmod(float_fmt* h, int M, const float* shift, const float* scale, hipStream_t s, PendingRed* pend = nullptr,
+int launch_lnmod(float_fmt* h, int M, const float* shift, const float* scale, const int* modrow, hipStream_t s, PendingRed* pend = nullptr,
                  const Lin* next = nullptr, u16* out = nullptr, int perm = 0, int touch_bit = 1, int rb_shape = -1) {
   const int nv = h->D / 256;
   const int rpw = h->tune.ln_rows;
@@ -579,10 +585,10 @@
                        : make_touch(h->tune, *next, M, 0, (grid.x / 8) * 64, 6);
 #define LN_LAUNCH(NV, KS)                                                                                                          \
   do {                                                                                                                             \
-    if (pf.W && wt) hipLaunchKernelGGL((fmt_lnmod_kernel<T, NV, KS, true, true>), grid, block, 0, s, h->xres, M, shift, scale, h->Ntot, out ? out : h->h16, red, pf, h->ntok, perm, h->sat); \
-    else if (pf.W) hipLaunchKernelGGL((fmt_lnmod_kernel<T, NV, KS, true, false>), grid, block, 0, s, h->xres, M, shift, scale, h->Ntot, out ? out : h->h16, red, pf, h->ntok, perm, h->sat); \
-    else if (wt) hipLaunchKernelGGL((fmt_lnmod_kernel<T, NV, KS, false, true>), grid, block, 0, s, h->xres, M, shift, scale, h->Ntot, out ? out : h->h16, red, pf, h->ntok, perm, h->sat); \
-    else hipLaunchKernelGGL((fmt_lnmod_kernel<T, NV, KS, false, false>), grid, block, 0, s, h->xres, M, shift, scale, h->Ntot, out ? out : h->h16, red, pf, h->ntok, perm, h->sat);   \
+    if (pf.W && wt) hipLaunchKernelGGL((fmt_lnmod_kernel<T, NV, KS, true, true>), grid, block, 0, s, h->xres, M, shift, scale, h->Ntot, modrow, out ? out : h->h16, red, pf, h->ntok, perm, h->sat); \
+    else if (pf.W) hipLaunchKernelGGL((fmt_lnmod_kernel<T, NV, KS, true, false>), grid, block, 0, s, h->xres, M, shift, scale, h->Ntot, modrow, out ? out : h->h16, red, pf, h->ntok, perm, h->sat); \
+    else if (wt) hipLaunchKernelGGL((fmt_lnmod_kernel<T, NV, KS, false, true>), grid, block, 0, s, h->xres, M, shift, scale, h->Ntot, modrow, out ? out : h->h16, red, pf, h->ntok, perm, h->sat); \
+    else hipLaunchKernelGGL((fmt_lnmod_kernel<T, NV, KS, false, false>), grid, block, 0, s, h->xres, M, shift, scale, h->Ntot, modrow, out ? out : h->h16, red, pf, h->ntok, perm, h->sat);   \
   } while (0)
 #define LN_CASE(NV)                     \
   case NV:                              \
@@ -664,14 +670,14 @@
 }
 
 template <class T>
-int run_mod_all(float_fmt* h, int M, int e0, int n, hipStream_t s) {
+int run_mod_all(float_fmt* h, int M, const int* src, int e0, int n, hipStream_t s) {
   const int D = h->D;
   const FmtTune& tn = h->tune;
   FH_REQUIRE(n >= 1 && n <= kScSteps, "modulation batch of %d evaluations (max %d)", n, kScSteps);
   const int prio = (s == h->cap_stream && s) ? h->cap_prio : stream_priority(s);
   const bool big = !T::is32 && tn.wide && prio == 0 && big_shape_ok(tn, n * M, h->adaln_all.N, h->adaln_all.K, h->n_cu);
   hipLaunchKernelGGL((fmt_silu_c_kernel<T>), dim3((M * D / 8 + 255) / 256, n), dim3(256), 0, s, h->sc16, h->temb + (size_t)e0 * D,
-                     h->ccond, M, D, (size_t)h->Mpad * D, big ? M : 0, h->sat);
+                     h->ccond, src, M, D, (size_t)h->Mpad * D, big ? M : 0, h->sat);
   h->mod_zs = big ? (size_t)M * h->Ntot : (size_t)h->Mmod * h->Ntot;
   if constexpr (!T::is32) {
     if (big) return launch_big4<T>(h->sc16, h->adaln_all, h->modall, n * M, h->Ntot, h->n_cu, false, s);
@@ -883,16 +889,16 @@
 }
 
 template <class T>
-int run_mega(float_fmt* h, int bc, const float* modbuf, bool euler, float dt, float a, float r, float e, hipStream_t s, float* vout_to) {
+int run_mega(float_fmt* h, int bc, const float* modbuf, const int* modrow, bool euler, float dt, float a, float r, float e, hipStream_t s, float* vout_to) {
   float_fmt::MegaPlan& P = h->mega[bc];
-  MegaDyn d{modbuf, dt, a, r, e, euler ? 1 : 0, vout_to ? vout_to : h->vout};
+  MegaDyn d{modbuf, modrow, dt, a, r, e, euler ? 1 : 0, vout_to ? vout_to : h->vout};
   fh_launch_prof(0, (fmt_mega_kernel<T>), dim3(kMegaWgs), dim3(512), kMegaSmem, s, P.dev, P.nstage, d, P.ctx, mega_sync_of(h));
   FH_CHECK_HIP(hipGetLastError());
   return FLOAT_OK;
 }
 
 template <class T>
-int run_blocks(float_fmt* h, int nclip, int bc, const float* modbuf, bool euler, float dt, float a, float r, float e, hipStream_t s,
+int run_blocks(float_fmt* h, int nclip, int bc, const float* modbuf, const int* modrow, bool euler, float dt, float a, float r, float e, hipStream_t s,
                float* vout_to = nullptr) {
   const float_fmt_cfg_t& c = h->cfg;
   const FmtTune& tn = h->tune;
@@ -900,7 +906,7 @@
   int rc;
   if constexpr (!T::is32) {
     if (bc <= 4 && mega_shape_ok<T>(h, nclip, bc)) {
-      if (h->mega[bc].dev) return run_mega<T>(h, bc, modbuf, euler, dt, a, r, e, s, vout_to);
+      if (h->mega[bc].dev) return run_mega<T>(h, bc, modbuf, modrow, euler, dt, a, r, e, s, vout_to);
     }
   }
   {
@@ -922,7 +928,7 @@
   for (int b = 0; b < c.depth; ++b) {
     const float* mod = modbuf + (size_t)b * 6 * D;
     const Blk& B = h->blk[b];
-    if ((rc = launch_lnmod<T>(h, M, mod, mod + D, s, &pend, &B.qkv, nullptr, 0, 128, rb_qkv.shape))) return rc;
+    if ((rc = launch_lnmod<T>(h, M, mod, mod + D, modrow, s, &pend, &B.qkv, nullptr, 0, 128, rb_qkv.shape))) return rc;
     {
       GemmArgs g = base_args(h->h16, B.qkv, M);
       g.sat = h->sat;
@@ -962,10 +968,11 @@
       g.ldo = D;
       g.gate = mod + 2 * D;
       g.ldg = h->Ntot;
+      g.modrow = modrow;
       if (tn.touch & 16) g.touch = make_touch(tn, B.fc1, M, 0, gemm_lanes_per_xcd(tn, M, g.N, g.K), 2);
       if ((rc = run_gemm<T, EPI_GATE_RES>(tn, g, s, false, &tn.plan_layer[RB_PROJ]))) return rc;
     }
-    if ((rc = launch_lnmod<T>(h, M, mod + 3 * D, mod + 4 * D, s, &pend, &B.fc1, nullptr, 0, 64, rb_fc1.shape))) return rc;
+    if ((rc = launch_lnmod<T>(h, M, mod + 3 * D, mod + 4 * D, modrow, s, &pend, &B.fc1, nullptr, 0, 64, rb_fc1.shape))) return rc;
     {
       GemmArgs g = base_args(h->h16, B.fc1, M);
       g.sat = h->sat;
@@ -1004,6 +1011,7 @@
       g.ldo = D;
       g.gate = mod + 5 * D;
       g.ldg = h->Ntot;
+      g.modrow = modrow;
       if ((rc = run_gemm<T, EPI_GATE_RES>(tn, g, s))) return rc;
     }
   }
@@ -1012,7 +1020,7 @@
     const bool tokblk = (!tn.no_tokblk || nclip > 1) && (bc == 1 || bc == 3 || bc == 4) && h->final_lin.K % 256 == 0;
     FH_REQUIRE(tokblk || nclip == 1, "batched sampling needs the token-blocked head GEMM");
     const int nblk = (ntok + 15) / 16, seqs = nclip * bc;
-    if ((rc = launch_lnmod<T>(h, M, mod, mod + D, s, &pend, nullptr, tokblk ? h->hfin16 : nullptr, tokblk ? seqs * 16 : 0))) return rc;
+    if ((rc = launch_lnmod<T>(h, M, mod, mod + D, modrow, s, &pend, nullptr, tokblk ? h->hfin16 : nullptr, tokblk ? seqs * 16 : 0))) return rc;
     GemmArgs g = base_args(tokblk ? h->hfin16 : h->h16, h->final_lin, tokblk ? nblk * seqs * 16 : M);
     g.sat = h->sat;
     g.tokblk = tokblk ? 1 : 0;
@@ -1077,12 +1085,25 @@
   int bc;
   unsigned wr_mask, wa_mask, we_mask;
   int nclip = 1;
+  int Mdist = 0;
+  const int *modrow = nullptr, *modsrc = nullptr;
 };
 
 CfgMode cfg_mode(float a, float r, float e, int include_r) {
   if (a == 1.0f && r == 1.0f && e == 1.0f) return {1, 1u, 1u, 1u, 1};
   if (!include_r) return {3, 0b111u, 0b110u, 0b010u, 1};
   return {4, 0b1110u, 0b1100u, 0b0100u, 1};
+}
+
+int rowmap_slot(int bc) { return bc == 1 ? 0 : (bc == 3 ? 1 : 2); }
+void bind_rows(float_fmt* h, CfgMode* m, int we_len) {
+  const float_fmt::RowMap& R = h->rowmap[rowmap_slot(m->bc)][we_len > 1 ? 1 : 0];
+  const int M = m->nclip * m->bc * h->ntok;
+  m->Mdist = R.dev ? m->nclip * R.dist1 : M;
+  m->modrow = R.dev;
+  m->modsrc = R.dev ? R.dev + (size_t)h->Bmax * R.rows1 : nullptr;
+  h->last_rows = M;
+  h->last_dist = m->Mdist;
 }
 
 template <class T>
@@ -1147,17 +1168,17 @@
   const Tableau& tb = tableau(h->method);
   const float_fmt_cfg_t& c = h->cfg;
   const size_t kstride = (size_t)h->Bmax * kMaxTok * c.dim_w;
-  const int n = m.nclip * c.n_cur * c.dim_w, rows = m.nclip * m.bc * h->ntok;
+  const int n = m.nclip * c.n_cur * c.dim_w;
   const int nev = n_evals(h->method, nfe), batch = h->tune.hoist ? kScSteps : 1;
   const bool euler = h->method == FLOAT_ODE_EULER;
   int rc;
   for (int ev = 0; ev < nev; ++ev) {
     const int i = ev / tb.s, j = ev - i * tb.s, z = ev % batch;
     const float dt = ts[i + 1] - ts[i];
-    if (z == 0 && (rc = run_mod_all<T>(h, rows, ev, std::min(batch, nev - ev), s))) return rc;
+    if (z == 0 && (rc = run_mod_all<T>(h, m.Mdist, m.modsrc, ev, std::min(batch, nev - ev), s))) return rc;
     const float* mod = h->modall + (size_t)z * h->mod_zs;
     if (euler) {
-      if ((rc = run_blocks<T>(h, m.nclip, m.bc, mod, true, dt, a, r, e, s))) return rc;
+      if ((rc = run_blocks<T>(h, m.nclip, m.bc, mod, m.modrow, true, dt, a, r, e, s))) return rc;
       continue;
     }
     if (j > 0) {
@@ -1165,7 +1186,7 @@
                          dt * tb.a[j][0], dt * tb.a[j][1], dt * tb.a[j][2], 0.f, 0, h->xin16, h->Kx / 32, c.n_prev, c.n_cur,
                          c.dim_w, m.nclip, h->sat);
     }
-    if ((rc = run_blocks<T>(h, m.nclip, m.bc, mod, false, 0.f, a, r, e, s, h->kbuf + (size_t)j * kstride))) return rc;
+    if ((rc = run_blocks<T>(h, m.nclip, m.bc, mod, m.modrow, false, 0.f, a, r, e, s, h->kbuf + (size_t)j * kstride))) return rc;
     if (j == tb.s - 1) {
       hipLaunchKernelGGL((fmt_rk_combine_kernel<T>), dim3((n + 255) / 256), dim3(256), 0, s, h->xcur, h->kbuf, kstride, tb.s,
                          dt * tb.b[0], dt * tb.b[1], dt * tb.b[2], dt * tb.b[3], 1, h->xin16, h->Kx / 32, c.n_prev, c.n_cur,
@@ -1231,6 +1252,7 @@
                 float a, float r, float e, int include_r, hipStream_t s, int nclip = 1) {
   CfgMode m = cfg_mode(a, r, e, include_r);
   m.nclip = nclip;
+  bind_rows(h, &m, we_len);
   FH_REQUIRE(!h->tune.no_tokblk || m.bc * h->ntok <= 240,
              "%d-way CFG of %d tokens is %d rows; the all-rows CFG epilogue GEMM holds at most 240 (15 row tiles)", m.bc, h->ntok,
              m.bc * h->ntok);
@@ -1255,13 +1277,14 @@
   tsp.t = t;
   int rc = prepare_time<T>(h, tsp, 1, s);
   if (rc) return rc;
-  const CfgMode m = cfg_mode(a, r, e, include_r);
+  CfgMode m = cfg_mode(a, r, e, include_r);
+  bind_rows(h, &m, we_len);
   FH_REQUIRE(!h->tune.no_tokblk || m.bc * h->ntok <= 240,
              "%d-way CFG of %d tokens is %d rows; the all-rows CFG epilogue GEMM holds at most 240 (15 row tiles)", m.bc, h->ntok,
              m.bc * h->ntok);
   if ((rc = stage_window<T>(h, m, x, wa, wr, we, we_len, prev_x, prev_wa, prev_we, s))) return rc;
-  if ((rc = run_mod_all<T>(h, m.bc * h->ntok, 0, 1, s))) return rc;
-  if ((rc = run_blocks<T>(h, 1, m.bc, h->modall, false, 0.f, a, r, e, s))) return rc;
+  if ((rc = run_mod_all<T>(h, m.Mdist, m.modsrc, 0, 1, s))) return rc;
+  if ((rc = run_blocks<T>(h, 1, m.bc, h->modall, m.modrow, false, 0.f, a, r, e, s))) return rc;
   return dev_copy(out, h->vout, (size_t)h->ntok * h->cfg.dim_w, s);
 }
 
@@ -1471,7 +1494,30 @@
   A(&h->tsin16, (size_t)kMaxSteps * 256);
   A(&h->th16, (size_t)kMaxSteps * D);
   A(&h->ccond, (size_t)Mp * D);
-  h->Mmod = 16 * ((h->Bmax * 4 * h->ntok + 15) / 16);
+  int max_dist = 0;
+  for (int include_r = 0; include_r <= 2 && !rc; ++include_r) {
+    const CfgMode m = include_r == 2 ? cfg_mode(1.f, 1.f, 1.f, 0) : cfg_mode(2.f, 1.f, 1.f, include_r);
+    for (int dyn = 0; dyn <= 1 && !rc; ++dyn) {
+      float_fmt::RowMap& R = h->rowmap[rowmap_slot(m.bc)][dyn];
+      R.rows1 = m.bc * h->ntok;
+      R.dist1 = R.rows1;
+      if (h->tune.modrows) {
+        const FmtRowMap map = fmt_row_map(m.bc, m.wr_mask, m.wa_mask, m.we_mask, h->Bmax, h->ntok, cfg->n_prev, dyn ? cfg->n_cur : 1);
+        if (!map.identity()) {
+          R.dist1 = map.ndist / h->Bmax;
+          std::vector<int> tab(map.modrow);
+          tab.insert(tab.end(), map.src.begin(), map.src.end());
+          rc = h->pool.alloc(&R.dev, tab.size(), false);
+          if (!rc && hipMemcpy(R.dev, tab.data(), tab.size() * sizeof(int), hipMemcpyHostToDevice) != hipSuccess) {
+            fh_set_error("hipMemcpy of the FMT row maps failed");
+            rc = FLOAT_E_HIP;
+          }
+        }
+      }
+      max_dist = std::max(max_dist, h->Bmax * R.dist1);
+    }
+  }
+  h->Mmod = 16 * ((max_dist + 15) / 16);
   if (!rc) rc = h->pool.alloc(&h->modall, (size_t)kScSteps * h->Mmod * h->Ntot, false);
   A(&h->kbuf, (size_t)4 * h->Bmax * kMaxTok * cfg->dim_w);
   A(&h->xres, (size_t)Mp * D);
@@ -1598,6 +1644,25 @@
     FH_CHECK_HIP(hipStreamSynchronize((hipStream_t)stream));
   }
   if (int rc = mega_poll(h)) return rc;
+  return FLOAT_OK;
+}
+
+int float_fmt_modrow_map(int32_t bc, int32_t nclip, int32_t n_prev, int32_t n_cur, int32_t we_len, int32_t* modrow,
+                         int32_t* n_distinct) {
+  FH_REQUIRE(bc == 1 || bc == 3 || bc == 4, "float_fmt_modrow_map: a CFG batch has 1, 3 or 4 rows per token (got %d)", bc);
+  FH_REQUIRE(nclip >= 1 && n_prev >= 0 && n_cur >= 1 && (we_len == 1 || we_len == n_cur) && n_distinct,
+             "float_fmt_modrow_map: invalid shape (%d clips, %d + %d tokens, we_len %d)", nclip, n_prev, n_cur, we_len);
+  const CfgMode m = bc == 1 ? cfg_mode(1.f, 1.f, 1.f, 0) : cfg_mode(2.f, 1.f, 1.f, bc == 4);
+  const FmtRowMap map = fmt_row_map(m.bc, m.wr_mask, m.wa_mask, m.we_mask, nclip, n_prev + n_cur, n_prev, we_len);
+  if (modrow) std::copy(map.modrow.begin(), map.modrow.end(), modrow);
+  *n_distinct = map.ndist;
+  return FLOAT_OK;
+}
+
+int float_fmt_modrows_in_use(float_fmt_t* h, int32_t* rows, int32_t* n_distinct) {
+  FH_REQUIRE(h && rows && n_distinct, "null argument to float_fmt_modrows_in_use");
+  *rows = h->last_rows;
+  *n_distinct = h->last_dist;
   return FLOAT_OK;
 }
 
diff --git a/comfyui-float_optimized_amd/csrc/fmt_kernels.hpp b/comfyui-float_optimized_amd/csrc/fmt_kernels.hpp
--- a/comfyui-float_optimized_amd/csrc/fmt_kernels.hpp
+++ b/comfyui-float_optimized_amd/csrc/fmt_kernels.hpp
@@ -61,10 +61,11 @@
     const int r = threadIdx.x / (NT * 2), cg = threadIdx.x % (NT * 2);
     const int row = m0 + r, nb = n0 + cg * 8;
     if (r < ROWS && row < g.M) {
+      const int grow = g.modrow ? g.modrow[row] : row;
       const float* o = g.out_f32 + (size_t)row * g.ldo + nb;
-      const float* gt = g.gate + (size_t)row * g.ldg + nb;
       res_pf[0] = fh_load_f4<COH>(o);
       res_pf[1] = fh_load_f4<COH>(o + 4);
+      const float* gt = g.gate + (size_t)grow * g.ldg + nb;
       gate_pf[0] = fh_load_f4_stream(gt);
       gate_pf[1] = fh_load_f4_stream(gt + 4);
     }
@@ -209,7 +210,7 @@
         else T::template store8_wt<fh_site<COH>(8), WT>(o16 + fmt_pack_off(row, nb, g.ldo16), u);
       } else if constexpr (EPI == EPI_GATE_RES) {
         float* o = g.out_f32 + (size_t)row * g.ldo + nb;
-        const float* gt = g.gate + (size_t)row * g.ldg + nb;
+        const float* gt = g.gate + (size_t)(g.modrow ? g.modrow[row] : row) * g.ldg + nb;
 #pragma unroll
         for (int e = 0; e < 8; e += 4) {
           float4 x, gg;
@@ -602,8 +603,8 @@
 
 template <class T, int NV, int KS, bool TOUCH, bool WT_, bool COH>
 __device__ __forceinline__ void fmt_lnmod_body(float* __restrict__ x, int M, const float* __restrict__ shift,
-                                               const float* __restrict__ scale, int ldm, u16* __restrict__ out, const LnRed& red,
-                                               const TouchSpec& pf, int ntok, int perm, unsigned long long* sat, const unsigned bid,
+                                               const float* __restrict__ scale, int ldm, const int* __restrict__ modrow,
+                                               u16* __restrict__ out, const LnRed& red, const TouchSpec& pf, int ntok, int perm, unsigned long long* sat, const unsigned bid,
                                                const unsigned nblk, const int wpb) {
   constexpr int D = NV * 256;
   constexpr bool WT = WT_ || COH;
@@ -624,37 +625,43 @@
     return;
   }
   float* xr = x + (size_t)row * D;
-#ifdef FMT_DIAG_HOTMOD
-  const size_t mrow = 0;
-#else
-  const size_t mrow = (size_t)row;
-#endif
-  const float* sh = shift + mrow * ldm;
-  const float* sc = scale + mrow * ldm;
+  const int mslot = *(modrow ? modrow + __builtin_amdgcn_readfirstlane(row) : reinterpret_cast<const int*>(shift));
+  __builtin_amdgcn_sched_barrier(0);
   float4 v[NV], a[NV], b[NV];
+  float4 p[KS > 0 ? KS : 1][NV], gt[NV], bi[NV];
+  (void)p, (void)gt, (void)bi;
   float s = 0.f;
 #pragma unroll
   for (int i = 0; i < NV; ++i) {
     const int c = i * 256 + lane * 4;
     v[i] = fh_load_f4<COH>(xr + c);
-    a[i] = fh_load_f4_stream(sh + c);
-    b[i] = fh_load_f4_stream(sc + c);
-  }
-  if (KS == 0 && touch) fmt_touch(pf, bid & 7, tfirst, tstride, touched);
-  if constexpr (KS > 0) {
-    float4 p[KS][NV], gt[NV], bi[NV];
-#pragma unroll
-    for (int i = 0; i < NV; ++i) {
-      const int c = i * 256 + lane * 4;
+    if constexpr (KS > 0) {
 #pragma unroll
       for (int k = 0; k < KS; ++k) {
         const float* ps = red.slab + k * red.slab_stride + (size_t)row * D + c;
         if constexpr (COH) p[k][i] = fh_load_f4<true>(ps);
         else p[k][i] = fh_load_f4_stream(ps);
       }
-      gt[i] = fh_load_f4_stream(red.gate + mrow * ldm + c);
       bi[i] = *reinterpret_cast<const float4*>(red.bias + c);
     }
+  }
+  __builtin_amdgcn_sched_barrier(0);
+#ifdef FMT_DIAG_HOTMOD
+  const size_t mrow = 0;
+#else
+  const size_t mrow = modrow ? (size_t)mslot : (size_t)row;
+#endif
+  const float* sh = shift + mrow * ldm;
+  const float* sc = scale + mrow * ldm;
+#pragma unroll
+  for (int i = 0; i < NV; ++i) {
+    const int c = i * 256 + lane * 4;
+    a[i] = fh_load_f4_stream(sh + c);
+    b[i] = fh_load_f4_stream(sc + c);
+    if constexpr (KS > 0) gt[i] = fh_load_f4_stream(red.gate + mrow * ldm + c);
+  }
+  if (KS == 0 && touch) fmt_touch(pf, bid & 7, tfirst, tstride, touched);
+  if constexpr (KS > 0) {
     if (touch) fmt_touch(pf, bid & 7, tfirst, tstride, touched);
 #pragma unroll
     for (int i = 0; i < NV; ++i) {
@@ -702,9 +709,10 @@
 
 template <class T, int NV, int KS, bool TOUCH, bool WT>
 __global__ __launch_bounds__(256) void fmt_lnmod_kernel(float* __restrict__ x, int M, const float* __restrict__ shift,
-                                                        const float* __restrict__ scale, int ldm, u16* __restrict__ out,
-                                                        LnRed red, TouchSpec pf, int ntok, int perm, unsigned long long* sat) {
-  fmt_lnmod_body<T, NV, KS, TOUCH, WT, false>(x, M, shift, scale, ldm, out, red, pf, ntok, perm, sat, blockIdx.x, gridDim.x,
+                                                        const float* __restrict__ scale, int ldm, const int* __restrict__ modrow,
+                                                        u16* __restrict__ out, LnRed red, TouchSpec pf, int ntok, int perm,
+                                                        unsigned long long* sat) {
+  fmt_lnmod_body<T, NV, KS, TOUCH, WT, false>(x, M, shift, scale, ldm, modrow, out, red, pf, ntok, perm, sat, blockIdx.x, gridDim.x,
                                               (int)(blockDim.x >> 6));
 }
 
@@ -1026,6 +1034,7 @@
 };
 struct MegaDyn {
   const float* mod;
+  const int* modrow;
   float dt, a, r, e;
   int euler;
   float* vout;
@@ -1094,10 +1103,10 @@
           if (threadIdx.x < 64) {
             const LnRed red{c.slab, c.slab_stride, st.red_bias, d.mod + st.red_gate_off};
             if (st.ks == 0)
-              fmt_lnmod_body<T, 4, 0, true, true, true>(c.xres, c.M, d.mod + st.shift_off, d.mod + st.scale_off, c.ldm, st.ln_out, red,
+              fmt_lnmod_body<T, 4, 0, true, true, true>(c.xres, c.M, d.mod + st.shift_off, d.mod + st.scale_off, c.ldm, d.modrow, st.ln_out, red,
                                                         st.pf, c.ntok, st.perm, c.sat, bid, st.nblk, 1);
             else
-              fmt_lnmod_body<T, 4, 4, true, true, true>(c.xres, c.M, d.mod + st.shift_off, d.mod + st.scale_off, c.ldm, st.ln_out, red,
+              fmt_lnmod_body<T, 4, 4, true, true, true>(c.xres, c.M, d.mod + st.shift_off, d.mod + st.scale_off, c.ldm, d.modrow, st.ln_out, red,
                                                         st.pf, c.ntok, st.perm, c.sat, bid, st.nblk, 1);
           }
           break;
@@ -1112,6 +1121,7 @@
         case MS_PROJ: {
           GemmArgs g = st.g;
           g.gate = d.mod + st.gate_off;
+          g.modrow = d.modrow;
           fmt_gemm_body<T, 3, 1, 8, EPI_GATE_RES, true>(g, bid, st.nblk);
           break;
         }
@@ -1219,16 +1229,18 @@
 
 template <class T>
 __global__ void fmt_silu_c_kernel(u16* __restrict__ out, const float* __restrict__ temb, const float* __restrict__ ccond,
-                                  int M, int D, size_t step_stride, int dense_rows, unsigned long long* sat) {
+                                  const int* __restrict__ src, int M, int D, size_t step_stride, int dense_rows,
+                                  unsigned long long* sat) {
   const int idx = (blockIdx.x * blockDim.x + threadIdx.x) * 8;
   if (idx >= M * D) return;
-  const int c = idx % D, row = idx / D + (int)blockIdx.y * dense_rows;
+  const int c = idx % D, r = idx / D, row = r + (int)blockIdx.y * dense_rows;
+  ccond += (size_t)(src ? src[r] : r) * D + c;
   typename T::elem* const o = reinterpret_cast<typename T::elem*>(out) + (dense_rows ? (size_t)0 : (size_t)blockIdx.y * step_stride);
   temb += (size_t)blockIdx.y * D;
   typename T::pack8 u;
 #pragma unroll
   for (int h = 0; h < 2; ++h) {
-    const float4 a = *reinterpret_cast<const float4*>(ccond + idx + 4 * h);
+    const float4 a = *reinterpret_cast<const float4*>(ccond + 4 * h);
     const float4 t = *reinterpret_cast<const float4*>(temb + c + 4 * h);
     T::set(u, 4 * h + 0, fh_silu(a.x + t.x));
     T::set(u, 4 * h + 1, fh_silu(a.y + t.y));
diff --git a/comfyui-float_optimized_amd/csrc/fmt_modrows.hpp b/comfyui-float_optimized_amd/csrc/fmt_modrows.hpp
--- /dev/null
+++ b/comfyui-float_optimized_amd/csrc/fmt_modrows.hpp
@@ -0,0 +1,36 @@
+#pragma once
+#include <map>
+#include <tuple>
+#include <vector>
+
+struct FmtRowMap {
+  std::vector<int> modrow;
+  std::vector<int> src;
+  int ndist = 0;
+  bool identity() const { return ndist == (int)modrow.size(); }
+};
+
+inline FmtRowMap fmt_row_map(int bc, unsigned wr_mask, unsigned wa_mask, unsigned we_mask, int nclip, int ntok, int n_prev,
+                             int we_len) {
+  FmtRowMap m;
+  m.modrow.resize((size_t)nclip * bc * ntok);
+  constexpr int kNull = -1;
+  for (int q = 0; q < nclip; ++q) {
+    std::map<std::tuple<int, int, int>, int> seen;
+    for (int b = 0; b < bc; ++b) {
+      const bool on_r = (wr_mask >> b) & 1, on_a = (wa_mask >> b) & 1, on_e = (we_mask >> b) & 1;
+      for (int i = 0; i < ntok; ++i) {
+        const int a = i < n_prev ? i : (on_a ? i : kNull);
+        const int e = !on_e ? kNull : (we_len == 1 ? 0 : i);
+        const int row = (q * bc + b) * ntok + i;
+        auto it = seen.find({on_r ? 1 : 0, a, e});
+        if (it == seen.end()) {
+          it = seen.emplace(std::make_tuple(on_r ? 1 : 0, a, e), m.ndist++).first;
+          m.src.push_back(row);
+        }
+        m.modrow[row] = it->second;
+      }
+    }
+  }
+  return m;
+}
diff --git a/comfyui-float_optimized_amd/csrc/fmt_pack.hpp b/comfyui-float_optimized_amd/csrc/fmt_pack.hpp
--- a/comfyui-float_optimized_amd/csrc/fmt_pack.hpp
+++ b/comfyui-float_optimized_amd/csrc/fmt_pack.hpp
@@ -59,6 +59,7 @@
   int ldo16;
   const float* gate;
   int ldg;
+  const int* modrow;
   const float* pos;
   int bc, ntok, n_prev;
   int nclip;
diff --git a/comfyui-float_optimized_amd/csrc/tuning.hpp b/comfyui-float_optimized_amd/csrc/tuning.hpp
--- a/comfyui-float_optimized_amd/csrc/tuning.hpp
+++ b/comfyui-float_optimized_amd/csrc/tuning.hpp
@@ -57,6 +57,7 @@
   int proj_split = 0;
   int touch = 230;
   bool hoist = true;
+  bool modrows = true;
   int zgroup = 0;
   int ln_rows = 1;
   int attn_qpw = 8, attn_lpq = 16;
@@ -88,6 +89,7 @@
     t.proj_split = env_atoi("FLOAT_FMT_PROJ_SPLIT", t.proj_split);
     t.touch = env_atoi("FLOAT_FMT_TOUCH", t.touch);
     t.hoist = env_atoi("FLOAT_FMT_HOIST", 1) != 0;
+    t.modrows = env_atoi("FLOAT_FMT_MODROWS", 1) != 0;
     t.zgroup = std::max(0, env_atoi("FLOAT_FMT_ZGROUP", 0));
     t.ln_rows = std::max(1, std::min(4, env_atoi("FLOAT_FMT_LN_ROWS", 1)));
     int attn[2] = {t.attn_qpw, t.attn_lpq};
diff --git a/comfyui-float_optimized_amd/fmt.py b/comfyui-float_optimized_amd/fmt.py
--- a/comfyui-float_optimized_amd/fmt.py
+++ b/comfyui-float_optimized_amd/fmt.py
@@ -52,6 +52,11 @@
             native.check(native.lib().float_fmt_debug(self._h, 1, native.dev_ptr(qkv), native.dev_ptr(out),
                                                       native.stream_ptr(self.device)))
         return out
+
+    def modrows_in_use(self):
+        rows, dist = C.c_int32(0), C.c_int32(0)
+        native.check(native.lib().float_fmt_modrows_in_use(self._h, C.byref(rows), C.byref(dist)))
+        return rows.value, dist.value
 
     def saturation(self, reset=False):
         with torch.cuda.device(self.device):
diff --git a/comfyui-float_optimized_amd/native.py b/comfyui-float_optimized_amd/native.py
--- a/comfyui-float_optimized_amd/native.py
+++ b/comfyui-float_optimized_amd/native.py
@@ -68,6 +68,8 @@
     "float_fmt_destroy": (None, [C.c_void_p]),
     "float_fmt_set_method": (C.c_int, [C.c_void_p, C.c_int32]),
     "float_fmt_debug": (C.c_int, [C.c_void_p, C.c_int32, C.c_void_p, C.c_void_p, C.c_void_p]),
+    "float_fmt_modrow_map": (C.c_int, [C.c_int32] * 5 + [C.POINTER(C.c_int32)] * 2),
+    "float_fmt_modrows_in_use": (C.c_int, [C.c_void_p, C.POINTER(C.c_int32), C.POINTER(C.c_int32)]),
     "float_fmt_eval": (C.c_int, [C.c_void_p, C.c_float] + [C.c_void_p] * 4 + [C.c_int32] + [C.c_void_p] * 3 +
                        [C.c_float] * 3 + [C.c_int32, C.c_void_p, C.c_void_p]),
     "float_fmt_sample_chunk": (C.c_int, [C.c_void_p] + [C.c_void_p] * 4 + [C.c_int32] + [C.c_void_p] * 3 +
@@ -196,6 +198,13 @@
     return int(tot.value)
 
 
+def fmt_modrow_map(bc, nclip, n_prev, n_cur, we_len=1):
+    rows = (C.c_int32 * (nclip * bc * (n_prev + n_cur)))()
+    n = C.c_int32(0)
+    check(lib().float_fmt_modrow_map(bc, nclip, n_prev, n_cur, we_len, rows, C.byref(n)))
+    return list(rows), n.value
+
+
 CMP_STATS = ("sum_sq_diff", "sum_sq_ref", "max_abs", "beyond_thr", "non_finite")
 _cmp_work = {}
 
diff --git a/include/float_hip.h b/include/float_hip.h
--- a/include/float_hip.h
+++ b/include/float_hip.h
@@ -78,6 +78,10 @@
                                  int32_t end_window, const float* hist_x, const float* hist_wa, const float* hist_we);
 
 int float_fmt_debug(float_fmt_t* h, int32_t what, const float* in, float* out, void* stream);
+
+int float_fmt_modrow_map(int32_t bc, int32_t nclip, int32_t n_prev, int32_t n_cur, int32_t we_len, int32_t* modrow,
+                         int32_t* n_distinct);
+int float_fmt_modrows_in_use(float_fmt_t* h, int32_t* rows, int32_t* n_distinct);
 
 typedef struct {
   int32_t size;
```

Result: slower. 2310 frames/s (-1.1%).
